# cheolwanpark/tiny-raytracer

Hardware: AMD Instinct MI355X
Metric: Mray/s (primary+secondary) (higher is better)
Workload: dtype f32; 1 GPU; cornell 2048x2048, depth 50, 256 spp per step (of 4096), streamed, reference-order BVH, seed 1; rays=160658711950, samples=22548578304, image_rows_per_gpu=2048, tuning=default, parallelism=single GPU, world_size=1, launched_by=plain

## Files before the change

### bindings/rust/tinyrt-sys/src/lib.rs

```rust
#![allow(non_camel_case_types)]

use std::os::raw::{c_char, c_int, c_void};

pub const TRT_ABI_VERSION: u32 = 4;

pub const TRT_OK: c_int = 0;
pub const TRT_ERR_INVALID_ARG: c_int = -1;
pub const TRT_ERR_DUPLICATE: c_int = -2;
pub const TRT_ERR_NOT_FOUND: c_int = -3;
pub const TRT_ERR_HIP: c_int = -4;
pub const TRT_ERR_NO_DEVICE: c_int = -5;
pub const TRT_ERR_OOM: c_int = -6;

pub const TRT_LAMBERTIAN: u32 = 0;
pub const TRT_METAL: u32 = 1;
pub const TRT_DIELECTRIC: u32 = 2;
pub const TRT_LIGHT: u32 = 3;

pub const TRT_BACKEND_MEGAKERNEL: u32 = 0;
pub const TRT_BACKEND_WAVEFRONT: u32 = 1;
pub const TRT_BACKEND_AUTO: u32 = 2;
pub const TRT_BACKEND_STREAMED: u32 = 3;

#[repr(C)]
// ... 420 lines not shown
    pub fn trt_render_multi(s: *mut trt_scene, cam: *const trt_camera, p: *const trt_render_params, devices: *const c_int,
                            ndev: u32, accum: *mut f32, stats: *mut trt_stats) -> c_int;
    pub fn trt_render_multi_device(s: *mut trt_scene, cam: *const trt_camera, p: *const trt_render_params,
                                   devices: *const c_int, ndev: u32, d_accum: *mut f32, stats: *mut trt_stats) -> c_int;
    pub fn trt_band_rows_local(height: u32, ndev: u32, rank: u32, rows_local: *mut u32) -> c_int;
    pub fn trt_band_copy_plan(width: u32, height: u32, ndev: u32, rank: u32, out: *mut trt_band_copy) -> c_int;
    pub fn trt_streamed_launch_plan(s: *const trt_scene, cam: *const trt_camera, p: *const trt_render_params,
                                    out: *mut trt_launch_plan) -> c_int;
    pub fn trt_render_device(s: *mut trt_scene, cam: *const trt_camera, p: *const trt_render_params, d_accum: *mut f32,
                             d_counters: *mut u64, stream: *mut c_void) -> c_int;
    pub fn trt_render_moments(s: *mut trt_scene, cam: *const trt_camera, p: *const trt_render_params, accum: *mut f32,
                              moment2: *mut f32, stats: *mut trt_stats) -> c_int;
    pub fn trt_render_moments_device(s: *mut trt_scene, cam: *const trt_camera, p: *const trt_render_params, d_accum: *mut f32,
                                     d_moment2: *mut f32, d_counters: *mut u64, stream: *mut c_void) -> c_int;
    pub fn trt_variance(accum: *const f32, moment2: *const f32, npixels: u32, samples_per_pixel: u32, variance: *mut f32) -> c_int;
    pub fn trt_variance_device(d_accum: *const f32, d_moment2: *const f32, npixels: u32, samples_per_pixel: u32,
                               d_variance: *mut f32, stream: *mut c_void) -> c_int;
    pub fn trt_render_pixels(s: *mut trt_scene, cam: *const trt_camera, p: *const trt_render_params, pixels: *const u32, n: u32,
                             accum: *mut f32, moment2: *mut f32, stats: *mut trt_stats) -> c_int;
    pub fn trt_render_pixels_device(s: *mut trt_scene, cam: *const trt_camera, p: *const trt_render_params, d_pixels: *const u32, n: u32,
                                    d_count: *const u32, d_accum: *mut f32, d_moment2: *mut f32, d_counters: *mut u64,
                                    stream: *mut c_void) -> c_int;
    pub fn trt_pixels_launch_plan(s: *const trt_scene, n: u32, compute_units: u32, out: *mut trt_query_plan) -> c_int;
    pub fn trt_select_pixels(accum: *const f32, moment2: *const f32, npixels: u32, samples_per_pixel: u32, samples_done: u32,
                             candidates: *const u32, n_candidates: u32, rel_tol: f32, abs_tol: f32, selected: *mut u32,
                             count: *mut u32) -> c_int;
    pub fn trt_select_pixels_device(d_accum: *const f32, d_moment2: *const f32, npixels: u32, samples_per_pixel: u32, samples_done: u32,
                                    d_candidates: *const u32, n_candidates: u32, rel_tol: f32, abs_tol: f32, d_selected: *mut u32,
                                    d_count: *mut u32, d_scratch: *mut c_void, scratch_bytes: u64, stream: *mut c_void) -> c_int;
    pub fn trt_select_scratch_bytes(n_candidates: u32) -> u64;
    pub fn trt_radiance_params_default(out: *mut trt_radiance_params);
    pub fn trt_radiance(s: *mut trt_scene, rays: *const trt_ray, n: u32, p: *const trt_radiance_params, radiance: *mut f32,
                        moment2: *mut f32, stats: *mut trt_stats) -> c_int;
    pub fn trt_radiance_device(s: *mut trt_scene, d_rays: *const trt_ray, n: u32, p: *const trt_radiance_params, d_radiance: *mut f32,
                               d_moment2: *mut f32, d_counters: *mut u64, stream: *mut c_void) -> c_int;
    pub fn trt_radiance_launch_plan(s: *const trt_scene, n: u32, compute_units: u32, out: *mut trt_query_plan) -> c_int;
    pub fn trt_gather_params_default(out: *mut trt_gather_params);
    pub fn trt_gather(s: *mut trt_scene, items: *const trt_ray, n: u32, p: *const trt_gather_params, radiance: *mut f32,
                      moment2: *mut f32, stats: *mut trt_stats) -> c_int;
    pub fn trt_gather_device(s: *mut trt_scene, d_items: *const trt_ray, n: u32, p: *const trt_gather_params, d_radiance: *mut f32,
                             d_moment2: *mut f32, d_counters: *mut u64, stream: *mut c_void) -> c_int;
    pub fn trt_gather_launch_plan(s: *const trt_scene, n: u32, compute_units: u32, out: *mut trt_query_plan) -> c_int;
    pub fn trt_ambient_params_default(out: *mut trt_ambient_params);
    pub fn trt_ambient(s: *mut trt_scene, items: *const trt_ray, n: u32, p: *const trt_ambient_params, visibility: *mut f32,
                       bent: *mut f32, stats: *mut trt_stats) -> c_int;
    pub fn trt_ambient_device(s: *mut trt_scene, d_items: *const trt_ray, n: u32, p: *const trt_ambient_params, d_visibility: *mut f32,
                              d_bent: *mut f32, d_counters: *mut u64, stream: *mut c_void) -> c_int;
    pub fn trt_ambient_launch_plan(s: *const trt_scene, n: u32, compute_units: u32, out: *mut trt_query_plan) -> c_int;
    pub fn trt_scene_emitters(s: *const trt_scene, out: *mut trt_emitter, cap: u32, count: *mut u32) -> c_int;
    pub fn trt_emitter_init_quad(out: *mut trt_emitter, corner: trt_vec3, u: trt_vec3, v: trt_vec3, color: trt_vec3);
    pub fn trt_emitter_init_sphere(out: *mut trt_emitter, centre: trt_vec3, radius: f32, color: trt_vec3);
    pub fn trt_direct_params_default(out: *mut trt_direct_params);
    pub fn trt_direct(s: *mut trt_scene, items: *const trt_ray, n: u32, emitters: *const trt_emitter, n_emitters: u32,
                      p: *const trt_direct_params, radiance: *mut f32, moment2: *mut f32, stats: *mut trt_stats) -> c_int;
    pub fn trt_direct_device(s: *mut trt_scene, d_items: *const trt_ray, n: u32, d_emitters: *const trt_emitter, n_emitters: u32,
                             p: *const trt_direct_params, d_radiance: *mut f32, d_moment2: *mut f32, d_counters: *mut u64,
                             stream: *mut c_void) -> c_int;
    pub fn trt_direct_launch_plan(s: *const trt_scene, n: u32, compute_units: u32, out: *mut trt_query_plan) -> c_int;
    pub fn trt_nee_params_default(out: *mut trt_nee_params);
    pub fn trt_nee(s: *mut trt_scene, items: *const trt_ray, n: u32, emitters: *const trt_emitter, n_emitters: u32,
                   p: *const trt_nee_params, radiance: *mut f32, moment2: *mut f32, stats: *mut trt_stats) -> c_int;
    pub fn trt_nee_device(s: *mut trt_scene, d_items: *const trt_ray, n: u32, d_emitters: *const trt_emitter, n_emitters: u32,
                          p: *const trt_nee_params, d_radiance: *mut f32, d_moment2: *mut f32, d_counters: *mut u64,
                          stream: *mut c_void) -> c_int;
    pub fn trt_nee_launch_plan(s: *const trt_scene, n: u32, compute_units: u32, out: *mut trt_query_plan) -> c_int;
    pub fn trt_nee_mis_params_default(out: *mut trt_nee_mis_params);
    pub fn trt_nee_mis(s: *mut trt_scene, items: *const trt_ray, n: u32, emitters: *const trt_emitter, n_emitters: u32,
                       p: *const trt_nee_mis_params, radiance: *mut f32, moment2: *mut f32, stats: *mut trt_stats) -> c_int;
    pub fn trt_nee_mis_device(s: *mut trt_scene, d_items: *const trt_ray, n: u32, d_emitters: *const trt_emitter, n_emitters: u32,
                              p: *const trt_nee_mis_params, d_radiance: *mut f32, d_moment2: *mut f32, d_counters: *mut u64,
                              stream: *mut c_void) -> c_int;
    pub fn trt_nee_mis_launch_plan(s: *const trt_scene, n: u32, compute_units: u32, out: *mut trt_query_plan) -> c_int;
    pub fn trt_direct_mis_params_default(out: *mut trt_direct_mis_params);
    pub fn trt_direct_mis(s: *mut trt_scene, items: *const trt_ray, n: u32, emitters: *const trt_emitter, n_emitters: u32,
                          p: *const trt_direct_mis_params, radiance: *mut f32, moment2: *mut f32, stats: *mut trt_stats) -> c_int;
    pub fn trt_direct_mis_device(s: *mut trt_scene, d_items: *const trt_ray, n: u32, d_emitters: *const trt_emitter, n_emitters: u32,
                                 p: *const trt_direct_mis_params, d_radiance: *mut f32, d_moment2: *mut f32, d_counters: *mut u64,
                                 stream: *mut c_void) -> c_int;
    pub fn trt_direct_mis_launch_plan(s: *const trt_scene, n: u32, compute_units: u32, out: *mut trt_query_plan) -> c_int;
    pub fn trt_emitter_pick_build(emitters: *const trt_emitter, n_emitters: u32, weights: *const f32, out: *mut trt_emitter_pick,
                                  total: *mut f32) -> c_int;
    pub fn trt_direct_pick(s: *mut trt_scene, items: *const trt_ray, n: u32, emitters: *const trt_emitter, pick: *const trt_emitter_pick,
                           n_emitters: u32, p: *const trt_direct_params, radiance: *mut f32, moment2: *mut f32, stats: *mut trt_stats) -> c_int;
    pub fn trt_direct_pick_device(s: *mut trt_scene, d_items: *const trt_ray, n: u32, d_emitters: *const trt_emitter,
                                  d_pick: *const trt_emitter_pick, n_emitters: u32, p: *const trt_direct_params, d_radiance: *mut f32,
                                  d_moment2: *mut f32, d_counters: *mut u64, stream: *mut c_void) -> c_int;
    pub fn trt_direct_pick_launch_plan(s: *const trt_scene, n: u32, compute_units: u32, out: *mut trt_query_plan) -> c_int;
    pub fn trt_direct_mis_pick(s: *mut trt_scene, items: *const trt_ray, n: u32, emitters: *const trt_emitter, pick: *const trt_emitter_pick,
                               n_emitters: u32, p: *const trt_direct_mis_params, total_power: f32, radiance: *mut f32, moment2: *mut f32,
                               stats: *mut trt_stats) -> c_int;
    pub fn trt_direct_mis_pick_device(s: *mut trt_scene, d_items: *const trt_ray, n: u32, d_emitters: *const trt_emitter,
                                      d_pick: *const trt_emitter_pick, n_emitters: u32, p: *const trt_direct_mis_params, total_power: f32,
                                      d_radiance: *mut f32, d_moment2: *mut f32, d_counters: *mut u64, stream: *mut c_void) -> c_int;
    pub fn trt_direct_mis_pick_launch_plan(s: *const trt_scene, n: u32, compute_units: u32, out: *mut trt_query_plan) -> c_int;
    pub fn trt_nee_pick(s: *mut trt_scene, items: *const trt_ray, n: u32, emitters: *const trt_emitter, pick: *const trt_emitter_pick,
                        n_emitters: u32, p: *const trt_nee_params, radiance: *mut f32, moment2: *mut f32, stats: *mut trt_stats) -> c_int;
    pub fn trt_nee_pick_device(s: *mut trt_scene, d_items: *const trt_ray, n: u32, d_emitters: *const trt_emitter,
                               d_pick: *const trt_emitter_pick, n_emitters: u32, p: *const trt_nee_params, d_radiance: *mut f32,
                               d_moment2: *mut f32, d_counters: *mut u64, stream: *mut c_void) -> c_int;
    pub fn trt_nee_pick_launch_plan(s: *const trt_scene, n: u32, compute_units: u32, out: *mut trt_query_plan) -> c_int;
    pub fn trt_nee_mis_pick(s: *mut trt_scene, items: *const trt_ray, n: u32, emitters: *const trt_emitter, pick: *const trt_emitter_pick,
                            n_emitters: u32, p: *const trt_nee_mis_params, total_power: f32, radiance: *mut f32, moment2: *mut f32,
                            stats: *mut trt_stats) -> c_int;
    pub fn trt_nee_mis_pick_device(s: *mut trt_scene, d_items: *const trt_ray, n: u32, d_emitters: *const trt_emitter,
                                   d_pick: *const trt_emitter_pick, n_emitters: u32, p: *const trt_nee_mis_params, total_power: f32,
                                   d_radiance: *mut f32, d_moment2: *mut f32, d_counters: *mut u64, stream: *mut c_void) -> c_int;
    pub fn trt_nee_mis_pick_launch_plan(s: *const trt_scene, n: u32, compute_units: u32, out: *mut trt_query_plan) -> c_int;
    pub fn trt_probe_params_default(out: *mut trt_probe_params);
    pub fn trt_probe(s: *mut trt_scene, items: *const trt_ray, n: u32, p: *const trt_probe_params, sh: *mut f32,
                     stats: *mut trt_stats) -> c_int;
    pub fn trt_probe_device(s: *mut trt_scene, d_items: *const trt_ray, n: u32, p: *const trt_probe_params, d_sh: *mut f32,
                            d_counters: *mut u64, stream: *mut c_void) -> c_int;
    pub fn trt_probe_launch_plan(s: *const trt_scene, n: u32, bands: u32, compute_units: u32, out: *mut trt_query_plan) -> c_int;
    pub fn trt_passes_params_default(out: *mut trt_passes_params);
    pub fn trt_passes(s: *mut trt_scene, items: *const trt_ray, n: u32, p: *const trt_passes_params, passes: *mut f32, spent: *mut f32,
                      stats: *mut trt_stats) -> c_int;
    pub fn trt_passes_device(s: *mut trt_scene, d_items: *const trt_ray, n: u32, p: *const trt_passes_params, d_passes: *mut f32,
                             d_spent: *mut f32, d_counters: *mut u64, stream: *mut c_void) -> c_int;
    pub fn trt_passes_launch_plan(s: *const trt_scene, n: u32, depth_bins: u32, compute_units: u32, out: *mut trt_query_plan) -> c_int;
    pub fn trt_sample_batch(s: *mut trt_scene, input: *const trt_sample_point, n: u32, out: *mut trt_sampled_color,
                            max_bounces: u32, background: trt_vec3, seed: u32, stats: *mut trt_stats) -> c_int;
    pub fn trt_intersect(s: *mut trt_scene, rays: *const trt_ray, t_max: *const f32, n: u32, hits: *mut trt_hit) -> c_int;
    pub fn trt_occluded(s: *mut trt_scene, rays: *const trt_ray, t_max: *const f32, n: u32, occluded: *mut u8) -> c_int;
    pub fn trt_intersect_device(s: *mut trt_scene, d_rays: *const trt_ray, d_t_max: *const f32, n: u32, d_hits: *mut trt_hit,
                                stream: *mut c_void) -> c_int;
    pub fn trt_occluded_device(s: *mut trt_scene, d_rays: *const trt_ray, d_t_max: *const f32, n: u32, d_occluded: *mut u8,
                               stream: *mut c_void) -> c_int;
    pub fn trt_query_launch_plan(s: *const trt_scene, n: u32, compute_units: u32, out: *mut trt_query_plan) -> c_int;
    pub fn trt_primary_rays(cam: *const trt_camera, p: *const trt_render_params, s: u32, rays: *mut trt_ray) -> c_int;
    pub fn trt_primary_rays_device(cam: *const trt_camera, p: *const trt_render_params, s: u32, d_rays: *mut trt_ray,
                                   stream: *mut c_void) -> c_int;
    pub fn trt_render_aov(s: *mut trt_scene, cam: *const trt_camera, p: *const trt_render_params, buffers: *const trt_aov_buffers) -> c_int;
    pub fn trt_render_aov_device(s: *mut trt_scene, cam: *const trt_camera, p: *const trt_render_params,
                                 d_buffers: *const trt_aov_buffers, stream: *mut c_void) -> c_int;
    pub fn trt_aov_launch_plan(s: *const trt_scene, n_pixels: u32, compute_units: u32, out: *mut trt_query_plan) -> c_int;
    pub fn trt_denoise_params_default(out: *mut trt_denoise_params);
    pub fn trt_denoise_scratch_bytes(width: u32, height: u32, params: *const trt_denoise_params) -> u64;
    pub fn trt_denoise(input: *const trt_denoise_inputs, width: u32, height: u32, params: *const trt_denoise_params, out: *mut f32) -> c_int;
    pub fn trt_denoise_device(d_in: *const trt_denoise_inputs, width: u32, height: u32, params: *const trt_denoise_params,
                              d_out: *mut f32, d_scratch: *mut c_void, scratch_bytes: u64, stream: *mut c_void) -> c_int;
    pub fn trt_denoise_color_default(out: *mut trt_denoise_color);
    pub fn trt_denoise_ex(input: *const trt_denoise_inputs, color: *const trt_denoise_color, width: u32, height: u32,
                          params: *const trt_denoise_params, out: *mut f32) -> c_int;
    pub fn trt_denoise_ex_device(d_in: *const trt_denoise_inputs, color: *const trt_denoise_color, width: u32, height: u32,
                                 params: *const trt_denoise_params, d_out: *mut f32, d_scratch: *mut c_void, scratch_bytes: u64,
                                 stream: *mut c_void) -> c_int;
    pub fn trt_tonemap_u8(accum: *const f32, npixels: u32, gamma: f32, rgb: *mut u8) -> c_int;
    pub fn trt_tonemap_u8_device(d_accum: *const f32, npixels: u32, gamma: f32, d_rgb: *mut u8, stream: *mut c_void) -> c_int;
    pub fn trt_streamed_chunk_spp(width: u32, rows: u32) -> u32;
    pub fn trt_kernel_timing_begin() -> c_int;
    pub fn trt_kernel_timing_end(total_ms: *mut f64, launches: *mut u32) -> c_int;

    pub fn trt_dominant_kernel(s: *const trt_scene, cam: *const trt_camera, p: *const trt_render_params) -> *const c_char;

    pub fn trt_last_error() -> *const c_char;
    pub fn trt_device_count() -> c_int;
    pub fn trt_set_device(ordinal: c_int) -> c_int;
    pub fn trt_abi_version() -> u32;
}
```

### include/tinyrt.h

```cpp
#ifndef TINYRT_H
#define TINYRT_H

#include <stddef.h>
#include <stdint.h>

#ifdef __cplusplus
extern "C" {
#endif

#define TRT_ABI_VERSION 4

enum trt_status {
    TRT_OK = 0,
    TRT_ERR_INVALID_ARG = -1,
    TRT_ERR_DUPLICATE = -2,
    TRT_ERR_NOT_FOUND = -3,
    TRT_ERR_HIP = -4,
    TRT_ERR_NO_DEVICE = -5,
    TRT_ERR_OOM = -6
};

typedef struct { float x, y, z; } trt_vec3;
typedef struct { trt_vec3 origin, direction; } trt_ray;
typedef struct { uint32_t x, y; trt_ray ray; } trt_sample_point;
// ... 267 lines not shown
typedef struct {
    uint32_t kind;
    uint32_t geometry;
    trt_vec3 a, b, c;
    trt_vec3 normal;
    trt_vec3 color;
    float area;
    uint32_t reserved[2];
} trt_emitter;
int trt_scene_emitters(const trt_scene *s, trt_emitter *out, uint32_t cap, uint32_t *count);
void trt_emitter_init_quad(trt_emitter *out, trt_vec3 corner, trt_vec3 u, trt_vec3 v, trt_vec3 color);
void trt_emitter_init_sphere(trt_emitter *out, trt_vec3 centre, float radius, trt_vec3 color);
typedef struct {
    trt_radiance_params path;
    float shadow_end;
    uint32_t reserved[7];
} trt_direct_params;
void trt_direct_params_default(trt_direct_params *out);
int trt_direct(trt_scene *s, const trt_ray *items, uint32_t n, const trt_emitter *emitters, uint32_t n_emitters,
               const trt_direct_params *p, float *radiance, float *moment2, trt_stats *stats);
int trt_direct_device(trt_scene *s, const trt_ray *d_items, uint32_t n, const trt_emitter *d_emitters, uint32_t n_emitters,
                      const trt_direct_params *p, float *d_radiance, float *d_moment2, uint64_t *d_counters, void *stream);
int trt_direct_launch_plan(const trt_scene *s, uint32_t n, uint32_t compute_units, trt_query_plan *out);

typedef struct {
    trt_gather_params gather;
    float shadow_end;
    uint32_t source_is_diffuse;
    uint32_t reserved[6];
} trt_nee_params;
void trt_nee_params_default(trt_nee_params *out);
int trt_nee(trt_scene *s, const trt_ray *items, uint32_t n, const trt_emitter *emitters, uint32_t n_emitters, const trt_nee_params *p,
            float *radiance, float *moment2, trt_stats *stats);
int trt_nee_device(trt_scene *s, const trt_ray *d_items, uint32_t n, const trt_emitter *d_emitters, uint32_t n_emitters,
                   const trt_nee_params *p, float *d_radiance, float *d_moment2, uint64_t *d_counters, void *stream);
int trt_nee_launch_plan(const trt_scene *s, uint32_t n, uint32_t compute_units, trt_query_plan *out);

enum trt_mis_heuristic { TRT_MIS_BALANCE = 0, TRT_MIS_POWER = 1 };
typedef struct {
    trt_nee_params nee;
    uint32_t heuristic;
    uint32_t reserved[7];
} trt_nee_mis_params;
void trt_nee_mis_params_default(trt_nee_mis_params *out);
int trt_nee_mis(trt_scene *s, const trt_ray *items, uint32_t n, const trt_emitter *emitters, uint32_t n_emitters,
                const trt_nee_mis_params *p, float *radiance, float *moment2, trt_stats *stats);
int trt_nee_mis_device(trt_scene *s, const trt_ray *d_items, uint32_t n, const trt_emitter *d_emitters, uint32_t n_emitters,
                       const trt_nee_mis_params *p, float *d_radiance, float *d_moment2, uint64_t *d_counters, void *stream);
int trt_nee_mis_launch_plan(const trt_scene *s, uint32_t n, uint32_t compute_units, trt_query_plan *out);

typedef struct {
    trt_direct_params direct;
    uint32_t heuristic;
    uint32_t reserved[7];
} trt_direct_mis_params;
void trt_direct_mis_params_default(trt_direct_mis_params *out);
int trt_direct_mis(trt_scene *s, const trt_ray *items, uint32_t n, const trt_emitter *emitters, uint32_t n_emitters,
                   const trt_direct_mis_params *p, float *radiance, float *moment2, trt_stats *stats);
int trt_direct_mis_device(trt_scene *s, const trt_ray *d_items, uint32_t n, const trt_emitter *d_emitters, uint32_t n_emitters,
                          const trt_direct_mis_params *p, float *d_radiance, float *d_moment2, uint64_t *d_counters, void *stream);
int trt_direct_mis_launch_plan(const trt_scene *s, uint32_t n, uint32_t compute_units, trt_query_plan *out);

typedef struct {
    float q;
    uint32_t alias;
    float prob;
    uint32_t reserved;
} trt_emitter_pick;
int trt_emitter_pick_build(const trt_emitter *emitters, uint32_t n_emitters, const float *weights, trt_emitter_pick *out, float *total);
int trt_direct_pick(trt_scene *s, const trt_ray *items, uint32_t n, const trt_emitter *emitters, const trt_emitter_pick *pick,
                    uint32_t n_emitters, const trt_direct_params *p, float *radiance, float *moment2, trt_stats *stats);
int trt_direct_pick_device(trt_scene *s, const trt_ray *d_items, uint32_t n, const trt_emitter *d_emitters, const trt_emitter_pick *d_pick,
                           uint32_t n_emitters, const trt_direct_params *p, float *d_radiance, float *d_moment2, uint64_t *d_counters,
                           void *stream);
int trt_direct_pick_launch_plan(const trt_scene *s, uint32_t n, uint32_t compute_units, trt_query_plan *out);
int trt_direct_mis_pick(trt_scene *s, const trt_ray *items, uint32_t n, const trt_emitter *emitters, const trt_emitter_pick *pick,
                        uint32_t n_emitters, const trt_direct_mis_params *p, float total_power, float *radiance, float *moment2,
                        trt_stats *stats);
int trt_direct_mis_pick_device(trt_scene *s, const trt_ray *d_items, uint32_t n, const trt_emitter *d_emitters,
                               const trt_emitter_pick *d_pick, uint32_t n_emitters, const trt_direct_mis_params *p, float total_power,
                               float *d_radiance, float *d_moment2, uint64_t *d_counters, void *stream);
int trt_direct_mis_pick_launch_plan(const trt_scene *s, uint32_t n, uint32_t compute_units, trt_query_plan *out);

int trt_nee_pick(trt_scene *s, const trt_ray *items, uint32_t n, const trt_emitter *emitters, const trt_emitter_pick *pick,
                 uint32_t n_emitters, const trt_nee_params *p, float *radiance, float *moment2, trt_stats *stats);
int trt_nee_pick_device(trt_scene *s, const trt_ray *d_items, uint32_t n, const trt_emitter *d_emitters, const trt_emitter_pick *d_pick,
                        uint32_t n_emitters, const trt_nee_params *p, float *d_radiance, float *d_moment2, uint64_t *d_counters,
                        void *stream);
int trt_nee_pick_launch_plan(const trt_scene *s, uint32_t n, uint32_t compute_units, trt_query_plan *out);
int trt_nee_mis_pick(trt_scene *s, const trt_ray *items, uint32_t n, const trt_emitter *emitters, const trt_emitter_pick *pick,
                     uint32_t n_emitters, const trt_nee_mis_params *p, float total_power, float *radiance, float *moment2,
                     trt_stats *stats);
int trt_nee_mis_pick_device(trt_scene *s, const trt_ray *d_items, uint32_t n, const trt_emitter *d_emitters,
                            const trt_emitter_pick *d_pick, uint32_t n_emitters, const trt_nee_mis_params *p, float total_power,
                            float *d_radiance, float *d_moment2, uint64_t *d_counters, void *stream);
int trt_nee_mis_pick_launch_plan(const trt_scene *s, uint32_t n, uint32_t compute_units, trt_query_plan *out);

typedef struct {
    uint32_t iterations;
    uint32_t normal_power_log2;
    float sigma_albedo;
    float sigma_depth;
    uint32_t reserved[4];
} trt_denoise_params;
void trt_denoise_params_default(trt_denoise_params *out);
typedef struct {
    const float *color;
    const float *albedo;
    const float *normal;
    const float *depth;
} trt_denoise_inputs;
uint64_t trt_denoise_scratch_bytes(uint32_t width, uint32_t height, const trt_denoise_params *params);
int trt_denoise(const trt_denoise_inputs *in, uint32_t width, uint32_t height, const trt_denoise_params *params, float *out);
int trt_denoise_device(const trt_denoise_inputs *d_in, uint32_t width, uint32_t height, const trt_denoise_params *params,
                       float *d_out, void *d_scratch, uint64_t scratch_bytes, void *stream);

typedef struct {
    const float *variance;
    float sigma_color;
    uint32_t reserved[5];
} trt_denoise_color;
void trt_denoise_color_default(trt_denoise_color *out);
int trt_denoise_ex(const trt_denoise_inputs *in, const trt_denoise_color *color, uint32_t width, uint32_t height,
                   const trt_denoise_params *params, float *out);
int trt_denoise_ex_device(const trt_denoise_inputs *d_in, const trt_denoise_color *color, uint32_t width, uint32_t height,
                          const trt_denoise_params *params, float *d_out, void *d_scratch, uint64_t scratch_bytes, void *stream);

int trt_tonemap_u8(const float *accum, uint32_t npixels, float gamma, uint8_t *rgb);

int trt_tonemap_u8_device(const float *d_accum, uint32_t npixels, float gamma, uint8_t *d_rgb, void *stream);

typedef struct {
    uint32_t scene_mode;
    uint32_t threads_per_workgroup, waves_per_simd, workgroups_per_cu;
    uint32_t lds_bytes, scene_lds_bytes;
    uint32_t leaf_slots, lds_leaf_stack, ray_pool;
    uint32_t walk;
    uint32_t specialised;
    uint32_t has_kernel;
    uint32_t kernel_waves_per_simd, kernel_threads, kernel_walk , kernel_ray_pool, kernel_counting;
    uint32_t chunk_spp;
    uint32_t dual_walk;
    uint64_t workspace_bytes;
} trt_launch_plan;
int trt_streamed_launch_plan(const trt_scene *s, const trt_camera *cam, const trt_render_params *p, trt_launch_plan *out);

uint32_t trt_streamed_chunk_spp(uint32_t width, uint32_t rows);

int trt_kernel_timing_begin(void);
int trt_kernel_timing_end(double *total_ms, uint32_t *launches);

const char *trt_dominant_kernel(const trt_scene *s, const trt_camera *cam, const trt_render_params *p);

const char *trt_last_error(void);
int trt_device_count(void);
int trt_set_device(int ordinal);
uint32_t trt_abi_version(void);

#ifdef __cplusplus
}
#endif
#endif
```

### tiny-raytracer_amd/_lib.py

```python
import ctypes as C
import os
import subprocess

_HERE = os.path.dirname(os.path.abspath(__file__))
LIB_PATH = os.environ.get("TRT_LIB_PATH") or os.path.join(_HERE, "libtinyrt.so")
CSRC = os.path.join(_HERE, "csrc")

TRT_OK = 0
ABI_VERSION = 4
ERR_INVALID_ARG, ERR_DUPLICATE, ERR_NOT_FOUND, ERR_HIP, ERR_NO_DEVICE, ERR_OOM = -1, -2, -3, -4, -5, -6
LAMBERTIAN, METAL, DIELECTRIC, LIGHT = 0, 1, 2, 3
BACKEND_MEGAKERNEL, BACKEND_WAVEFRONT, BACKEND_AUTO, BACKEND_STREAMED = 0, 1, 2, 3


class Vec3(C.Structure):
    _fields_ = [("x", C.c_float), ("y", C.c_float), ("z", C.c_float)]

    def __init__(self, x=0.0, y=0.0, z=0.0):
        super().__init__(float(x), float(y), float(z))

    def tolist(self):
        return [self.x, self.y, self.z]


# ... 178 lines not shown

SIGNATURES = {
    "trt_world_create": (C.c_int, [C.POINTER(C.c_void_p)]),
    "trt_world_destroy": (None, [C.c_void_p]),
    "trt_world_add_material": (C.c_int, [C.c_void_p, C.c_char_p, C.POINTER(Material)]),
    "trt_world_get_material": (C.c_int, [C.c_void_p, C.c_char_p, C.POINTER(C.c_uint32)]),
    "trt_world_add_sphere": (C.c_int, [C.c_void_p, Vec3, C.c_float, C.c_uint32]),
    "trt_world_add_spheres": (C.c_int, [C.c_void_p, C.c_uint32, C.c_void_p, C.c_void_p]),
    "trt_world_add_quad": (C.c_int, [C.c_void_p, Vec3, Vec3, Vec3, C.c_uint32]),
    "trt_world_num_geometries": (C.c_int, [C.c_void_p]),
    "trt_world_num_materials": (C.c_int, [C.c_void_p]),
    "trt_scene_create": (C.c_int, [C.c_void_p, C.POINTER(C.c_void_p)]),
    "trt_scene_options_default": (None, [C.POINTER(SceneOptions)]),
    "trt_scene_create_ex": (C.c_int, [C.c_void_p, C.POINTER(SceneOptions), C.POINTER(C.c_void_p)]),
    "trt_scene_create_on_device": (C.c_int, [C.c_void_p, C.POINTER(SceneOptions), C.POINTER(C.c_void_p)]),
    "trt_tuning_default": (None, [C.POINTER(Tuning)]),
    "trt_scene_destroy": (None, [C.c_void_p]),
    "trt_scene_trim": (C.c_int, [C.c_void_p]),
    "trt_scene_get_info": (C.c_int, [C.c_void_p, C.POINTER(SceneInfo)]),
    "trt_scene_get_nodes": (C.c_int, [C.c_void_p, C.c_void_p, C.c_void_p, C.c_void_p, C.c_uint32]),
    "trt_scene_get_cull_nodes": (C.c_int, [C.c_void_p, C.c_void_p, C.c_void_p, C.c_void_p, C.c_uint32]),
    "trt_scene_get_compact_nodes": (C.c_int, [C.c_void_p, C.c_void_p, C.c_uint32]),
    "trt_scene_get_packed": (C.c_int, [C.c_void_p, C.c_void_p, C.c_uint32]),
    "trt_camera_init": (C.c_int, [C.POINTER(CameraPOD), C.c_float, C.c_float, Vec3, Vec3, Vec3, C.c_float,
                                  C.c_uint32, C.c_uint32]),
    "trt_render": (C.c_int, [C.c_void_p, C.POINTER(CameraPOD), C.POINTER(RenderParams), C.c_void_p, C.POINTER(Stats)]),
    "trt_render_multi": (C.c_int, [C.c_void_p, C.POINTER(CameraPOD), C.POINTER(RenderParams), C.POINTER(C.c_int), C.c_uint32,
                                   C.c_void_p, C.POINTER(Stats)]),
    "trt_render_multi_device": (C.c_int, [C.c_void_p, C.POINTER(CameraPOD), C.POINTER(RenderParams), C.POINTER(C.c_int),
                                          C.c_uint32, C.c_void_p, C.POINTER(Stats)]),
    "trt_band_rows_local": (C.c_int, [C.c_uint32, C.c_uint32, C.c_uint32, C.POINTER(C.c_uint32)]),
    "trt_band_copy_plan": (C.c_int, [C.c_uint32, C.c_uint32, C.c_uint32, C.c_uint32, C.POINTER(BandCopy)]),
    "trt_streamed_launch_plan": (C.c_int, [C.c_void_p, C.POINTER(CameraPOD), C.POINTER(RenderParams), C.POINTER(LaunchPlan)]),
    "trt_kernel_timing_begin": (C.c_int, []),
    "trt_kernel_timing_end": (C.c_int, [C.POINTER(C.c_double), C.POINTER(C.c_uint32)]),
    "trt_render_device": (C.c_int, [C.c_void_p, C.POINTER(CameraPOD), C.POINTER(RenderParams), C.c_void_p, C.c_void_p,
                                    C.c_void_p]),
    "trt_render_moments": (C.c_int, [C.c_void_p, C.POINTER(CameraPOD), C.POINTER(RenderParams), C.c_void_p, C.c_void_p, C.POINTER(Stats)]),
    "trt_render_moments_device": (C.c_int, [C.c_void_p, C.POINTER(CameraPOD), C.POINTER(RenderParams), C.c_void_p, C.c_void_p, C.c_void_p,
                                            C.c_void_p]),
    "trt_variance": (C.c_int, [C.c_void_p, C.c_void_p, C.c_uint32, C.c_uint32, C.c_void_p]),
    "trt_variance_device": (C.c_int, [C.c_void_p, C.c_void_p, C.c_uint32, C.c_uint32, C.c_void_p, C.c_void_p]),
    "trt_render_pixels": (C.c_int, [C.c_void_p, C.POINTER(CameraPOD), C.POINTER(RenderParams), C.c_void_p, C.c_uint32, C.c_void_p, C.c_void_p,
                                    C.POINTER(Stats)]),
    "trt_render_pixels_device": (C.c_int, [C.c_void_p, C.POINTER(CameraPOD), C.POINTER(RenderParams), C.c_void_p, C.c_uint32, C.c_void_p,
                                           C.c_void_p, C.c_void_p, C.c_void_p, C.c_void_p]),
    "trt_pixels_launch_plan": (C.c_int, [C.c_void_p, C.c_uint32, C.c_uint32, C.POINTER(QueryPlan)]),
    "trt_select_pixels": (C.c_int, [C.c_void_p, C.c_void_p, C.c_uint32, C.c_uint32, C.c_uint32, C.c_void_p, C.c_uint32, C.c_float, C.c_float,
                                    C.c_void_p, C.POINTER(C.c_uint32)]),
    "trt_select_pixels_device": (C.c_int, [C.c_void_p, C.c_void_p, C.c_uint32, C.c_uint32, C.c_uint32, C.c_void_p, C.c_uint32, C.c_float,
                                           C.c_float, C.c_void_p, C.c_void_p, C.c_void_p, C.c_uint64, C.c_void_p]),
    "trt_select_scratch_bytes": (C.c_uint64, [C.c_uint32]),
    "trt_radiance_params_default": (None, [C.POINTER(RadianceParams)]),
    "trt_radiance": (C.c_int, [C.c_void_p, C.c_void_p, C.c_uint32, C.POINTER(RadianceParams), C.c_void_p, C.c_void_p, C.POINTER(Stats)]),
    "trt_radiance_device": (C.c_int, [C.c_void_p, C.c_void_p, C.c_uint32, C.POINTER(RadianceParams), C.c_void_p, C.c_void_p, C.c_void_p,
                                      C.c_void_p]),
    "trt_radiance_launch_plan": (C.c_int, [C.c_void_p, C.c_uint32, C.c_uint32, C.POINTER(QueryPlan)]),
    "trt_gather_params_default": (None, [C.POINTER(GatherParams)]),
    "trt_gather": (C.c_int, [C.c_void_p, C.c_void_p, C.c_uint32, C.POINTER(GatherParams), C.c_void_p, C.c_void_p, C.POINTER(Stats)]),
    "trt_gather_device": (C.c_int, [C.c_void_p, C.c_void_p, C.c_uint32, C.POINTER(GatherParams), C.c_void_p, C.c_void_p, C.c_void_p,
                                    C.c_void_p]),
    "trt_gather_launch_plan": (C.c_int, [C.c_void_p, C.c_uint32, C.c_uint32, C.POINTER(QueryPlan)]),
    "trt_ambient_params_default": (None, [C.POINTER(AmbientParams)]),
    "trt_ambient": (C.c_int, [C.c_void_p, C.c_void_p, C.c_uint32, C.POINTER(AmbientParams), C.c_void_p, C.c_void_p, C.POINTER(Stats)]),
    "trt_ambient_device": (C.c_int, [C.c_void_p, C.c_void_p, C.c_uint32, C.POINTER(AmbientParams), C.c_void_p, C.c_void_p, C.c_void_p,
                                     C.c_void_p]),
    "trt_ambient_launch_plan": (C.c_int, [C.c_void_p, C.c_uint32, C.c_uint32, C.POINTER(QueryPlan)]),
    "trt_scene_emitters": (C.c_int, [C.c_void_p, C.c_void_p, C.c_uint32, C.POINTER(C.c_uint32)]),
    "trt_emitter_init_quad": (None, [C.POINTER(Emitter), Vec3, Vec3, Vec3, Vec3]),
    "trt_emitter_init_sphere": (None, [C.POINTER(Emitter), Vec3, C.c_float, Vec3]),
    "trt_direct_params_default": (None, [C.POINTER(DirectParams)]),
    "trt_direct": (C.c_int, [C.c_void_p, C.c_void_p, C.c_uint32, C.c_void_p, C.c_uint32, C.POINTER(DirectParams), C.c_void_p, C.c_void_p,
                             C.POINTER(Stats)]),
    "trt_direct_device": (C.c_int, [C.c_void_p, C.c_void_p, C.c_uint32, C.c_void_p, C.c_uint32, C.POINTER(DirectParams), C.c_void_p, C.c_void_p,
                                    C.c_void_p, C.c_void_p]),
    "trt_direct_launch_plan": (C.c_int, [C.c_void_p, C.c_uint32, C.c_uint32, C.POINTER(QueryPlan)]),
    "trt_nee_params_default": (None, [C.POINTER(NeeParams)]),
    "trt_nee": (C.c_int, [C.c_void_p, C.c_void_p, C.c_uint32, C.c_void_p, C.c_uint32, C.POINTER(NeeParams), C.c_void_p, C.c_void_p,
                          C.POINTER(Stats)]),
    "trt_nee_device": (C.c_int, [C.c_void_p, C.c_void_p, C.c_uint32, C.c_void_p, C.c_uint32, C.POINTER(NeeParams), C.c_void_p, C.c_void_p,
                                 C.c_void_p, C.c_void_p]),
    "trt_nee_launch_plan": (C.c_int, [C.c_void_p, C.c_uint32, C.c_uint32, C.POINTER(QueryPlan)]),
    "trt_nee_mis_params_default": (None, [C.POINTER(NeeMisParams)]),
    "trt_nee_mis": (C.c_int, [C.c_void_p, C.c_void_p, C.c_uint32, C.c_void_p, C.c_uint32, C.POINTER(NeeMisParams), C.c_void_p, C.c_void_p,
                              C.POINTER(Stats)]),
    "trt_nee_mis_device": (C.c_int, [C.c_void_p, C.c_void_p, C.c_uint32, C.c_void_p, C.c_uint32, C.POINTER(NeeMisParams), C.c_void_p, C.c_void_p,
                                     C.c_void_p, C.c_void_p]),
    "trt_nee_mis_launch_plan": (C.c_int, [C.c_void_p, C.c_uint32, C.c_uint32, C.POINTER(QueryPlan)]),
    "trt_direct_mis_params_default": (None, [C.POINTER(DirectMisParams)]),
    "trt_direct_mis": (C.c_int, [C.c_void_p, C.c_void_p, C.c_uint32, C.c_void_p, C.c_uint32, C.POINTER(DirectMisParams), C.c_void_p, C.c_void_p,
                                 C.POINTER(Stats)]),
    "trt_direct_mis_device": (C.c_int, [C.c_void_p, C.c_void_p, C.c_uint32, C.c_void_p, C.c_uint32, C.POINTER(DirectMisParams), C.c_void_p,
                                        C.c_void_p, C.c_void_p, C.c_void_p]),
    "trt_direct_mis_launch_plan": (C.c_int, [C.c_void_p, C.c_uint32, C.c_uint32, C.POINTER(QueryPlan)]),
    "trt_emitter_pick_build": (C.c_int, [C.c_void_p, C.c_uint32, C.c_void_p, C.c_void_p, C.POINTER(C.c_float)]),
    "trt_direct_pick": (C.c_int, [C.c_void_p, C.c_void_p, C.c_uint32, C.c_void_p, C.c_void_p, C.c_uint32, C.POINTER(DirectParams), C.c_void_p,
                                  C.c_void_p, C.POINTER(Stats)]),
    "trt_direct_pick_device": (C.c_int, [C.c_void_p, C.c_void_p, C.c_uint32, C.c_void_p, C.c_void_p, C.c_uint32, C.POINTER(DirectParams),
                                         C.c_void_p, C.c_void_p, C.c_void_p, C.c_void_p]),
    "trt_direct_pick_launch_plan": (C.c_int, [C.c_void_p, C.c_uint32, C.c_uint32, C.POINTER(QueryPlan)]),
    "trt_direct_mis_pick": (C.c_int, [C.c_void_p, C.c_void_p, C.c_uint32, C.c_void_p, C.c_void_p, C.c_uint32, C.POINTER(DirectMisParams),
                                      C.c_float, C.c_void_p, C.c_void_p, C.POINTER(Stats)]),
    "trt_direct_mis_pick_device": (C.c_int, [C.c_void_p, C.c_void_p, C.c_uint32, C.c_void_p, C.c_void_p, C.c_uint32, C.POINTER(DirectMisParams),
                                             C.c_float, C.c_void_p, C.c_void_p, C.c_void_p, C.c_void_p]),
    "trt_direct_mis_pick_launch_plan": (C.c_int, [C.c_void_p, C.c_uint32, C.c_uint32, C.POINTER(QueryPlan)]),
    "trt_nee_pick": (C.c_int, [C.c_void_p, C.c_void_p, C.c_uint32, C.c_void_p, C.c_void_p, C.c_uint32, C.POINTER(NeeParams), C.c_void_p,
                               C.c_void_p, C.POINTER(Stats)]),
    "trt_nee_pick_device": (C.c_int, [C.c_void_p, C.c_void_p, C.c_uint32, C.c_void_p, C.c_void_p, C.c_uint32, C.POINTER(NeeParams),
                                      C.c_void_p, C.c_void_p, C.c_void_p, C.c_void_p]),
    "trt_nee_pick_launch_plan": (C.c_int, [C.c_void_p, C.c_uint32, C.c_uint32, C.POINTER(QueryPlan)]),
    "trt_nee_mis_pick": (C.c_int, [C.c_void_p, C.c_void_p, C.c_uint32, C.c_void_p, C.c_void_p, C.c_uint32, C.POINTER(NeeMisParams),
                                   C.c_float, C.c_void_p, C.c_void_p, C.POINTER(Stats)]),
    "trt_nee_mis_pick_device": (C.c_int, [C.c_void_p, C.c_void_p, C.c_uint32, C.c_void_p, C.c_void_p, C.c_uint32, C.POINTER(NeeMisParams),
                                          C.c_float, C.c_void_p, C.c_void_p, C.c_void_p, C.c_void_p]),
    "trt_nee_mis_pick_launch_plan": (C.c_int, [C.c_void_p, C.c_uint32, C.c_uint32, C.POINTER(QueryPlan)]),
    "trt_probe_params_default": (None, [C.POINTER(ProbeParams)]),
    "trt_probe": (C.c_int, [C.c_void_p, C.c_void_p, C.c_uint32, C.POINTER(ProbeParams), C.c_void_p, C.POINTER(Stats)]),
    "trt_probe_device": (C.c_int, [C.c_void_p, C.c_void_p, C.c_uint32, C.POINTER(ProbeParams), C.c_void_p, C.c_void_p, C.c_void_p]),
    "trt_probe_launch_plan": (C.c_int, [C.c_void_p, C.c_uint32, C.c_uint32, C.c_uint32, C.POINTER(QueryPlan)]),
    "trt_passes_params_default": (None, [C.POINTER(PassesParams)]),
    "trt_passes": (C.c_int, [C.c_void_p, C.c_void_p, C.c_uint32, C.POINTER(PassesParams), C.c_void_p, C.c_void_p, C.POINTER(Stats)]),
    "trt_passes_device": (C.c_int, [C.c_void_p, C.c_void_p, C.c_uint32, C.POINTER(PassesParams), C.c_void_p, C.c_void_p, C.c_void_p,
                                    C.c_void_p]),
    "trt_passes_launch_plan": (C.c_int, [C.c_void_p, C.c_uint32, C.c_uint32, C.c_uint32, C.POINTER(QueryPlan)]),
    "trt_sample_batch": (C.c_int, [C.c_void_p, C.c_void_p, C.c_uint32, C.c_void_p, C.c_uint32, Vec3, C.c_uint32,
                                   C.POINTER(Stats)]),
    "trt_intersect": (C.c_int, [C.c_void_p, C.c_void_p, C.c_void_p, C.c_uint32, C.c_void_p]),
    "trt_occluded": (C.c_int, [C.c_void_p, C.c_void_p, C.c_void_p, C.c_uint32, C.c_void_p]),
    "trt_intersect_device": (C.c_int, [C.c_void_p, C.c_void_p, C.c_void_p, C.c_uint32, C.c_void_p, C.c_void_p]),
    "trt_occluded_device": (C.c_int, [C.c_void_p, C.c_void_p, C.c_void_p, C.c_uint32, C.c_void_p, C.c_void_p]),
    "trt_query_launch_plan": (C.c_int, [C.c_void_p, C.c_uint32, C.c_uint32, C.POINTER(QueryPlan)]),
    "trt_primary_rays": (C.c_int, [C.POINTER(CameraPOD), C.POINTER(RenderParams), C.c_uint32, C.c_void_p]),
    "trt_primary_rays_device": (C.c_int, [C.POINTER(CameraPOD), C.POINTER(RenderParams), C.c_uint32, C.c_void_p, C.c_void_p]),
    "trt_render_aov": (C.c_int, [C.c_void_p, C.POINTER(CameraPOD), C.POINTER(RenderParams), C.POINTER(AovBuffers)]),
    "trt_render_aov_device": (C.c_int, [C.c_void_p, C.POINTER(CameraPOD), C.POINTER(RenderParams), C.POINTER(AovBuffers), C.c_void_p]),
    "trt_aov_launch_plan": (C.c_int, [C.c_void_p, C.c_uint32, C.c_uint32, C.POINTER(QueryPlan)]),
    "trt_denoise_params_default": (None, [C.POINTER(DenoiseParams)]),
    "trt_denoise_scratch_bytes": (C.c_uint64, [C.c_uint32, C.c_uint32, C.POINTER(DenoiseParams)]),
    "trt_denoise": (C.c_int, [C.POINTER(DenoiseInputs), C.c_uint32, C.c_uint32, C.POINTER(DenoiseParams), C.c_void_p]),
    "trt_denoise_device": (C.c_int, [C.POINTER(DenoiseInputs), C.c_uint32, C.c_uint32, C.POINTER(DenoiseParams), C.c_void_p, C.c_void_p,
                                     C.c_uint64, C.c_void_p]),
    "trt_denoise_color_default": (None, [C.POINTER(DenoiseColor)]),
    "trt_denoise_ex": (C.c_int, [C.POINTER(DenoiseInputs), C.POINTER(DenoiseColor), C.c_uint32, C.c_uint32, C.POINTER(DenoiseParams), C.c_void_p]),
    "trt_denoise_ex_device": (C.c_int, [C.POINTER(DenoiseInputs), C.POINTER(DenoiseColor), C.c_uint32, C.c_uint32, C.POINTER(DenoiseParams),
                                        C.c_void_p, C.c_void_p, C.c_uint64, C.c_void_p]),
    "trt_streamed_chunk_spp": (C.c_uint32, [C.c_uint32, C.c_uint32]),
    "trt_tonemap_u8": (C.c_int, [C.c_void_p, C.c_uint32, C.c_float, C.c_void_p]),
    "trt_tonemap_u8_device": (C.c_int, [C.c_void_p, C.c_uint32, C.c_float, C.c_void_p, C.c_void_p]),
    "trt_dominant_kernel": (C.c_char_p, [C.c_void_p, C.POINTER(CameraPOD), C.POINTER(RenderParams)]),
    "trt_last_error": (C.c_char_p, []),
    "trt_device_count": (C.c_int, []),
    "trt_set_device": (C.c_int, [C.c_int]),
    "trt_abi_version": (C.c_uint32, []),
}


def build(force=False):
    if force and os.path.exists(LIB_PATH):
        os.remove(LIB_PATH)
    subprocess.run(["make", "-C", CSRC, "--no-print-directory"], check=True)
    return LIB_PATH


def _share_hip_runtime_with_torch():
    import importlib.util
    try:
        spec = importlib.util.find_spec("torch")
    except (ImportError, ValueError):
        spec = None
    if spec is None or not spec.submodule_search_locations:
        return None
    cand = os.path.join(list(spec.submodule_search_locations)[0], "lib", "libamdhip64.so")
    if os.path.exists(cand):
        C.CDLL(cand, mode=C.RTLD_GLOBAL)
        return cand
    return None


def load():
    _share_hip_runtime_with_torch()
    if not os.path.exists(LIB_PATH):
        raise ImportError(
            f"{LIB_PATH} is missing: build the HIP extension first (python -c 'import __graft_entry__ as g; g.build()' "
            "or make -C tiny-raytracer_amd/csrc). There is no fallback path.")
    lib = C.CDLL(LIB_PATH)
    for name, (res, args) in SIGNATURES.items():
        fn = getattr(lib, name)
        fn.restype = res
        fn.argtypes = args
    if lib.trt_abi_version() != ABI_VERSION:
        raise ImportError("libtinyrt.so ABI version mismatch")
    return lib


lib = load()


class TinyRTError(RuntimeError):
    def __init__(self, code, message):
        super().__init__(f"tinyrt error {code}: {message}")
        self.code = code


def check(rc):
    if rc != TRT_OK:
        raise TinyRTError(rc, lib.trt_last_error().decode("utf-8", "replace"))
```

### tiny-raytracer_amd/csrc/capi.hip

```cpp
#include <hip/hip_runtime.h>

#include <math.h>
#include <stdio.h>
#include <stdlib.h>
#include <string.h>

#include <algorithm>
#include <memory>
#include <mutex>
#include <new>
#include <string>
#include <thread>
#include <vector>

#include "axis_quads.h"
#include "nearest_first.h"
#include "flat_reuse.h"
#include "host_stage.h"
#include "kernels.h"
#include "scene.h"
#include "scene_adopt.h"
#include "scene_cache.h"
#include "scene_query.h"
#include "stream_plan.h"

using namespace trt;

struct trt_world {
    World w;
};

namespace trt {
namespace {
std::mutex g_timing_mu;
bool g_timing_on = false;
unsigned g_timing_epoch = 0;
struct TimingPair { hipEvent_t begin, end; int device; };
std::vector<TimingPair> g_timing_pairs;
struct TimingOpen { hipEvent_t ev = nullptr; hipStream_t stream = nullptr; int device = -1; unsigned epoch = 0; };
thread_local TimingOpen t_open;
}
void timing_mark(hipStream_t stream, bool begin) {
    unsigned epoch;
    {
        std::lock_guard<std::mutex> lock(g_timing_mu);
        if (!g_timing_on) return;
        epoch = g_timing_epoch;
    }
    int dev = -1;
    if (hipGetDevice(&dev) != hipSuccess) { (void)hipGetLastError(); return; }
    if (begin) {
        if (t_open.ev) { (void)hipEventDestroy(t_open.ev); t_open = TimingOpen{}; }
        hipEvent_t ev = nullptr;
        if (hipEventCreate(&ev) != hipSuccess) { (void)hipGetLastError(); return; }
        if (hipEventRecord(ev, stream) != hipSuccess) { (void)hipGetLastError(); (void)hipEventDestroy(ev); return; }
        t_open.ev = ev; t_open.stream = stream; t_open.device = dev; t_open.epoch = epoch;
        return;
    }
    if (!t_open.ev) return;
    TimingOpen o = t_open;
    t_open = TimingOpen{};
    hipEvent_t ev = nullptr;
    if (o.stream != stream || o.device != dev || o.epoch != epoch || hipEventCreate(&ev) != hipSuccess) {
        (void)hipGetLastError();
        (void)hipEventDestroy(o.ev);
        return;
    }
    if (hipEventRecord(ev, stream) != hipSuccess) { (void)hipGetLastError(); (void)hipEventDestroy(ev); (void)hipEventDestroy(o.ev); return; }
    std::lock_guard<std::mutex> lock(g_timing_mu);
    if (g_timing_on && g_timing_epoch == epoch) g_timing_pairs.push_back(TimingPair{o.ev, ev, dev});
    else { (void)hipEventDestroy(o.ev); (void)hipEventDestroy(ev); }
}
}

struct trt_scene {
    SceneHost host;
    FlatReuse flat_reuse{};
    std::vector<uint32_t> geo_index;
    SceneCache cache;
};

namespace {

thread_local std::string g_last_error;

int fail(int code, const std::string& msg) {
    g_last_error = msg;
    return code;
}
int fail_hip(hipError_t e, const char* what) {
    return fail(TRT_ERR_HIP, std::string(what) + ": " + hipGetErrorString(e));
}
#define TRT_HIP(call)                                        \
    do {                                                     \
        hipError_t e_ = (call);                              \
        if (e_ != hipSuccess) return fail_hip(e_, #call);    \
    } while (0)

struct Defaults {
    trt_tuning tuning;
    trt_scene_options scene;
    bool flat_reuse = true;
    bool axis_quads = true;
    bool nearest_first = true;
};
const Defaults& defaults() {
    static const Defaults d = [] {
        Defaults x;
        x.tuning = tuning_builtin();
        x.scene = scene_options_builtin();
        auto env = [](const char* name) -> const char* { const char* e = getenv(name); return (e && *e) ? e : nullptr; };
        auto u32 = [&](const char* name, uint32_t& field) { if (const char* e = env(name)) field = (uint32_t)strtoul(e, nullptr, 10); };
        trt_tuning& t = x.tuning;
        u32("TRT_STREAM_MINW", t.stream_waves_per_simd); u32("TRT_BIG_THREADS", t.stream_big_threads); u32("TRT_STREAM_BATCH_SPP", t.stream_batch_spp);
        u32("TRT_RADIANCE_GB", t.radiance_gb); u32("TRT_LEAF_SLOTS", t.leaf_slots); u32("TRT_LDS_LEAF_STACK", t.lds_leaf_stack);
        u32("TRT_RAY_POOL", t.ray_pool); u32("TRT_STRAGGLERS", t.stragglers); u32("TRT_LDS_STRAGGLERS", t.lds_stragglers);
        u32("TRT_DUAL_WALK", t.dual_walk); u32("TRT_RUNTIME_WALK", t.runtime_walk); u32("TRT_XCD_REMAP", t.xcd_remap);
        u32("TRT_MINW", t.mega_waves_per_simd); u32("TRT_MEGA_THREADS", t.mega_threads); u32("TRT_MINW8", t.mega_global_waves8);
        u32("TRT_WF_MINW", t.wf_waves_per_simd); u32("TRT_WF_SERVE_MIN", t.wf_serve_min);
        trt_scene_options& o = x.scene;
        if (const char* e = env("TRT_CULL_PRUNE")) {
            const float v = (float)atof(e);
            if (v > 0.0f && v <= 1.0f) o.cull_prune = v;
        }
        if (const char* e = env("TRT_FLAT_WALK")) o.flat_walk = atoi(e) ? 1 : 0;
        if (const char* e = env("TRT_FLAT_REUSE")) x.flat_reuse = atoi(e) != 0;
        if (const char* e = env("TRT_AXIS_QUADS")) x.axis_quads = atoi(e) != 0;
        if (const char* e = env("TRT_NEAREST_FIRST")) x.nearest_first = atoi(e) != 0;
        if (const char* e = env("TRT_COMPACT_NODES")) o.compact_nodes = atoi(e) ? 1 : 0;
        if (const char* e = env("TRT_SCRATCH_CAP_MB")) o.scratch_cap_bytes = (uint64_t)strtoull(e, nullptr, 10) << 20;
        return x;
    }();
    return d;
}

[[maybe_unused]] const bool g_defaults_read_at_load = (defaults(), true);

int require_device() {
    int n = 0;
    hipError_t e = hipGetDeviceCount(&n);
    if (e != hipSuccess || n <= 0) {
        (void)hipGetLastError();
        return fail(TRT_ERR_NO_DEVICE, "no HIP device visible: libtinyrt has no CPU path, it needs a gfx950 GPU");
    }
    return TRT_OK;
}

int scene_on_device(trt_scene* s, SceneDev& out) {
    out.L = s->host.layout;
    return s->cache.on_device(SceneCache::PACKED_SCENE, s->host.blob.data(), s->host.layout.blob_bytes, "scene upload", out.blob);
}

void to_camera_dev(const trt_camera& c, CameraDev& d) {
    const trt_vec3* src[6] = {&c.position, &c.viewport_upper_left, &c.horizontal, &c.vertical, &c.defocus_disk_u, &c.defocus_disk_v};
    float* dst[6] = {d.pos, d.upper_left, d.horizontal, d.vertical, d.du, d.dv};
    for (int i = 0; i < 6; i++) { dst[i][0] = src[i]->x; dst[i][1] = src[i]->y; dst[i][2] = src[i]->z; }
    d.width = c.width;
    d.height = c.height;
}

int to_render_args(const trt_camera* cam, const trt_render_params* p, RenderArgs& ra, uint32_t& rows, trt_tuning& tn) {
    if (cam->width < 2 || cam->height < 2) return fail(TRT_ERR_INVALID_ARG, "camera width and height must be at least 2 (pointgen.rs:41-42 divides by width-1, height-1)");
    if (p->samples_per_pixel == 0) return fail(TRT_ERR_INVALID_ARG, "samples_per_pixel must be positive");
    uint32_t s1 = p->sample_end == 0 ? p->samples_per_pixel : p->sample_end;
    if (p->sample_begin > s1 || s1 > p->samples_per_pixel) return fail(TRT_ERR_INVALID_ARG, "sample range must satisfy begin <= end <= samples_per_pixel");
    if (p->backend > TRT_BACKEND_STREAMED) return fail(TRT_ERR_INVALID_ARG, "unknown backend");
    ra.background[0] = p->background.x; ra.background[1] = p->background.y; ra.background[2] = p->background.z;
    ra.inv_spp = 1.0f / (float)p->samples_per_pixel;
    ra.max_bounces = p->max_bounces;
    ra.seed_key = rng_seed_key(p->seed);
    ra.sample_begin = p->sample_begin;
    ra.sample_end = s1;
    ra.accumulate = p->accumulate ? 1u : 0u;
    if (p->band_rows == 0) {
        ra.band_rows = 0; ra.band_stride = 1; ra.band_offset = 0;
        rows = cam->height;
    } else {
        if (p->band_stride == 0 || p->band_offset >= p->band_stride) return fail(TRT_ERR_INVALID_ARG, "band_offset must be below band_stride");
        rows = p->rows_local;
        if (rows > 0) {
            uint32_t last = rows - 1;
            uint64_t y = ((uint64_t)(last / p->band_rows) * p->band_stride + p->band_offset) * p->band_rows + last % p->band_rows;
            if (y >= cam->height) return fail(TRT_ERR_INVALID_ARG, "rows_local maps past the last image row");
        }
        ra.band_rows = p->band_rows; ra.band_stride = p->band_stride; ra.band_offset = p->band_offset;
    }
    ra.rows_local = rows;
    tn = p->tuning ? *p->tuning : defaults().tuning;
    if (tn.stream_batch_spp > 256u) tn.stream_batch_spp = 256u;
    if (tn.stragglers > 63u) tn.stragglers = 63u;
    if (tn.lds_stragglers > 63u) tn.lds_stragglers = 63u;
    if (tn.radiance_gb > 64u) tn.radiance_gb = 64u;
    ra.leaf_slots = tn.leaf_slots;
    ra.lds_leaf_stack = tn.lds_leaf_stack;
    ra.xcd_aware = tn.xcd_remap ? 1u : 0u;
    ra.stragglers = tn.stragglers;
    ra.ref_tree = p->collect_stats == 1 ? 1u : 0u;
    ra.flat_reuse = FlatReuse{0u, 0u, 0u};
    return TRT_OK;
}

int check_render_args(const trt_camera* cam, const trt_render_params* p, uint32_t& rows) {
    RenderArgs ra;
    trt_tuning tn;
    return to_render_args(cam, p, ra, rows, tn);
}

int enqueue_render(trt_scene* s, const trt_camera* cam, const trt_render_params* p, float* d_accum, uint64_t* d_counters,
                   hipStream_t stream, uint32_t* rows_out, float* d_moment2 = nullptr, MomentsLaunch launch_moments = nullptr) {
    RenderArgs ra;
    trt_tuning tn;
    uint32_t rows = 0;
    int rc = to_render_args(cam, p, ra, rows, tn);
    if (rc != TRT_OK) return rc;
    if (rows_out) *rows_out = rows;
    SceneDev sc;
    rc = scene_on_device(s, sc);
    if (rc != TRT_OK) return rc;
    CameraDev cd;
    to_camera_dev(*cam, cd);
    ra.flat_reuse = s->flat_reuse;
    const size_t bytes = (size_t)rows * cam->width * 3 * sizeof(float);
    if (rows == 0 || ra.sample_begin == ra.sample_end || ra.max_bounces == 0) {
        if (!ra.accumulate && bytes) TRT_HIP(hipMemsetAsync(d_accum, 0, bytes, stream));
        if (!ra.accumulate && bytes && d_moment2) TRT_HIP(hipMemsetAsync(d_moment2, 0, bytes, stream));
        return TRT_OK;
    }
    const bool wavefront = p->backend == TRT_BACKEND_WAVEFRONT;
    const bool streamed = p->backend == TRT_BACKEND_STREAMED || p->backend == TRT_BACKEND_AUTO;
    if (wavefront || streamed) {
        int dev = 0;
        TRT_HIP(hipGetDevice(&dev));
        Workspace* ws = nullptr;
        if (wavefront) {
            rc = s->cache.workspace_acquire(dev, wavefront_workspace_bytes(cam->width, rows), stream, &ws);
        } else {
            uint32_t samples = ra.sample_end - ra.sample_begin;
            const uint32_t full = streamed_chunk_spp(cam->width, rows, tn.radiance_gb);
            if (samples > full) samples = full;
            const uint32_t wanted = samples;
            const uint32_t short_samples = s->cache.short_samples(dev);
            if (short_samples != 0u && short_samples < samples) {
                const size_t idle = s->cache.idle_workspace_bytes(dev);
                size_t free_b = 0, total_b = 0;
                const bool known = hipMemGetInfo(&free_b, &total_b) == hipSuccess;
                (void)hipGetLastError();
                if (!known || free_b + idle < streamed_workspace_bytes(cam->width, rows, samples, tn.radiance_gb)) samples = short_samples;
            }
            bool trimmed = false;
            for (;;) {
                rc = s->cache.workspace_acquire(dev, streamed_workspace_bytes(cam->width, rows, samples, tn.radiance_gb), stream, &ws);
                if (rc != TRT_ERR_OOM) break;
                if (!trimmed) {
                    trimmed = true;
                    s->cache.trim(dev, 0);
                    continue;
                }
                if (samples <= 1u) break;
                samples = (samples + 1u) / 2u;
            }
            s->cache.set_short_samples(dev, (rc == TRT_OK && samples < wanted) ? samples : 0u);
        }
        if (rc != TRT_OK) return rc;
        hipError_t le;
        if (streamed && d_moment2) {
            le = launch_moments ? launch_moments(sc, cd, ra, tn, ws->ptr, ws->bytes, d_accum, d_moment2, reinterpret_cast<unsigned long long*>(d_counters),
                                                 p->collect_stats != 0, stream)
                                : hipErrorInvalidDeviceFunction;
        } else if (streamed) {
            le = launch_streamed(sc, cd, ra, tn, ws->ptr, ws->bytes, d_accum, reinterpret_cast<unsigned long long*>(d_counters), p->collect_stats != 0, stream);
        } else {
            le = launch_wavefront(sc, cd, ra, tn, ws->ptr, d_accum, reinterpret_cast<unsigned long long*>(d_counters), p->collect_stats != 0, stream);
        }
        rc = s->cache.workspace_release(dev, ws, stream);
        if (le != hipSuccess) return fail_hip(le, streamed ? "launch_streamed" : "launch_wavefront");
        return rc;
    }
    TRT_HIP(launch_megakernel(sc, cd, ra, tn, d_accum, reinterpret_cast<unsigned long long*>(d_counters), p->collect_stats != 0, stream));
    return TRT_OK;
}

void set_flat_reuse(trt_scene* s) {
    const SceneLayout& L = s->host.layout;
    const size_t end = 16u * ((size_t)L.off_leaf_list + 2u * (size_t)L.n_leaves);
    const bool have = L.flat_walk != 0u && L.n_leaves > 0u && s->host.blob.size() >= end;
    uint32_t m[3];
    flat_reuse_masks(have ? s->host.blob.data() + 16u * (size_t)L.off_leaf_list : nullptr, L.n_leaves, have && defaults().flat_reuse, m);
    const size_t qend = 16u * ((size_t)L.off_quad + 5u * (size_t)L.n_quads);
    const bool have_quads = have && L.n_quads > 0u && s->host.blob.size() >= qend;
    const uint32_t aq = axis_quads_flag(have_quads ? s->host.blob.data() + 16u * (size_t)L.off_quad : nullptr, L.n_quads, L.n_leaves, L.flat_walk != 0u,
                                        scene_mode(L) == 1, defaults().axis_quads);
    float planes[3];
    const uint32_t nf = nearest_first_flag(have ? s->host.blob.data() + 16u * (size_t)L.off_leaf_list : nullptr, L.n_leaves,
                                           have_quads ? s->host.blob.data() + 16u * (size_t)L.off_quad : nullptr, L.n_quads, L.n_spheres, aq,
                                           defaults().nearest_first, planes);
    s->flat_reuse = FlatReuse{m[0], m[1], m[2], aq, nf, planes[0], planes[1], planes[2]};
}

void set_geo_index(trt_scene* s) {
    const SceneLayout& L = s->host.layout;
    const std::vector<int32_t>& geo = s->host.reference.prim_geo;
    s->geo_index.assign((size_t)L.n_spheres + L.n_quads, 0xFFFFFFFFu);
    const size_t end = 16u * ((size_t)L.off_ref_nodes + 2u * (size_t)L.n_nodes);
    if (geo.size() < L.n_nodes || s->host.blob.size() < end) return;
    for (uint32_t i = 0; i < L.n_nodes; i++) {
        if (geo[i] < 0) continue;
        uint32_t link;
        memcpy(&link, s->host.blob.data() + 16u * ((size_t)L.off_ref_nodes + 2u * (size_t)i + 1u) + 12u, 4);
        const size_t slot = (size_t)(link & PRIM_INDEX_MASK) + ((link & PRIM_QUAD_BIT) ? L.n_spheres : 0u);
        if (!(link & NODE_INNER_BIT) && slot < s->geo_index.size()) s->geo_index[slot] = (uint32_t)geo[i];
    }
}

trt_scene* scene_from_host(SceneHost&& host, const trt_scene_options& opt) {
    std::unique_ptr<trt_scene> s(new trt_scene());
    s->host = std::move(host);
    set_flat_reuse(s.get());
    set_geo_index(s.get());
    s->cache.set_cap((size_t)opt.scratch_cap_bytes);
    return s.release();
}

}

namespace trt {
int query_fail(int code, const std::string& msg) { return fail(code, msg); }
int query_fail_hip(hipError_t e, const char* what) { return fail_hip(e, what); }
int query_require_device() { return require_device(); }
const SceneLayout& query_scene_layout(const trt_scene* s) { return s->host.layout; }
int query_scene_on_device(trt_scene* s, QueryScene& out) {
    int rc = scene_on_device(s, out.scene);
    if (rc != TRT_OK) return rc;
    out.flat_reuse = s->flat_reuse;
    return s->cache.on_device(SceneCache::GEO_INDEX, s->geo_index.data(), s->geo_index.size() * sizeof(uint32_t), "geometry index upload", out.geo_index);
}
int query_render_args(const trt_camera* cam, const trt_render_params* p, RenderArgs& ra, uint32_t& rows) {
    trt_render_params q = *p;
    q.backend = TRT_BACKEND_AUTO;
    q.tuning = nullptr;
    trt_tuning tn;
    return to_render_args(cam, &q, ra, rows, tn);
}
void query_camera_dev(const trt_camera& cam, CameraDev& out) { to_camera_dev(cam, out); }
}

namespace trt {
int scene_options_check(const trt_scene_options& opt) {
    if (!(opt.cull_prune > 0.0f && opt.cull_prune <= 1.0f)) return fail(TRT_ERR_INVALID_ARG, "cull_prune must be in (0, 1]");
    return TRT_OK;
}
trt_scene_options scene_options_or_defaults(const trt_scene_options* options) { return options ? *options : defaults().scene; }
int scene_fail(int code, const std::string& msg) { return fail(code, msg); }
const World& world_of(const trt_world* w) { return w->w; }
trt_scene* scene_adopt(SceneHost&& host, const trt_scene_options& opt, int device, void* d_blob) {
    try {
        trt_scene* s = scene_from_host(std::move(host), opt);
        if (d_blob) s->cache.adopt_packed_scene(device, d_blob);
        return s;
    } catch (const std::bad_alloc&) {
        fail(TRT_ERR_OOM, "out of memory");
        return nullptr;
    }
}
}

extern "C" {

uint32_t trt_abi_version(void) { return TRT_ABI_VERSION; }
const char* trt_last_error(void) { return g_last_error.c_str(); }

int trt_device_count(void) {
    int n = 0;
    if (hipGetDeviceCount(&n) != hipSuccess) { (void)hipGetLastError(); return 0; }
    return n;
}
int trt_set_device(int ordinal) {
    int rc = require_device();
    if (rc != TRT_OK) return rc;
    TRT_HIP(hipSetDevice(ordinal));
    return TRT_OK;
}

int trt_world_create(trt_world** out) {
    if (!out) return fail(TRT_ERR_INVALID_ARG, "out is null");
    trt_world* w = new (std::nothrow) trt_world();
    if (!w) return fail(TRT_ERR_OOM, "out of memory");
    *out = w;
    return TRT_OK;
}
void trt_world_destroy(trt_world* w) { delete w; }

int trt_world_add_material(trt_world* w, const char* name, const trt_material* m) {
    if (!w || !name || !m) return fail(TRT_ERR_INVALID_ARG, "null argument");
    if (m->kind > TRT_LIGHT) return fail(TRT_ERR_INVALID_ARG, "unknown material kind");
    try {
        std::string key(name);
        if (w->w.material_index.count(key)) return fail(TRT_ERR_DUPLICATE, key + " key is already in the material table");
        trt_material mm = *m;
        if (mm.kind == TRT_METAL) mm.param = fminf(fmaxf(mm.param, 0.0f), 1.0f);
        w->w.material_index.emplace(key, (uint32_t)w->w.materials.size());
        w->w.materials.push_back(mm);
    } catch (const std::bad_alloc&) {
        return fail(TRT_ERR_OOM, "out of memory");
    }
    return TRT_OK;
}
int trt_world_get_material(const trt_world* w, const char* name, uint32_t* index) {
    if (!w || !name || !index) return fail(TRT_ERR_INVALID_ARG, "null argument");
    auto it = w->w.material_index.find(name);
    if (it == w->w.material_index.end()) return fail(TRT_ERR_NOT_FOUND, std::string("no material named ") + name);
    *index = it->second;
    return TRT_OK;
}
int trt_world_add_sphere(trt_world* w, trt_vec3 center, float radius, uint32_t material) {
    if (!w) return fail(TRT_ERR_INVALID_ARG, "world is null");
    if (material >= w->w.materials.size()) return fail(TRT_ERR_INVALID_ARG, "material index out of range");
// ... 550 lines not shown
```

### tiny-raytracer_amd/csrc/kernels.h

```cpp
#pragma once

#include <hip/hip_runtime.h>
#include <stddef.h>
#include <stdint.h>

#include "scene.h"

namespace trt {

struct SceneDev {
    const float4* blob;
    SceneLayout L;
};

struct CameraDev {
    float pos[3], upper_left[3], horizontal[3], vertical[3], du[3], dv[3];
    uint32_t width, height;
};

struct FlatReuse {
    uint32_t x, y, z;
    uint32_t axis_quads = 0u;
    uint32_t nearest_first = 0u;
    float px = 0.0f, py = 0.0f, pz = 0.0f;
};

struct RenderArgs {
    float background[3];
    float inv_spp;
    uint32_t max_bounces;
    uint32_t seed_key;
    uint32_t sample_begin, sample_end;
    uint32_t accumulate;
    uint32_t band_rows, band_stride, band_offset;
    uint32_t rows_local;
    uint32_t xcd_aware;
    uint32_t lds_leaf_stack;
    uint32_t leaf_slots;
    uint32_t ref_tree;
    uint32_t stragglers;
    FlatReuse flat_reuse;
};

inline trt_tuning tuning_builtin() {
    trt_tuning t{};
    t.stream_waves_per_simd = 0;
    t.stream_big_threads = 0;
    t.stream_batch_spp = 8;
    t.radiance_gb = 16;
    t.leaf_slots = 0;
    t.lds_leaf_stack = 1;
    t.ray_pool = 1;
    t.stragglers = 8;
    t.lds_stragglers = 8;
    t.dual_walk = 0;
    t.runtime_walk = 0;
    t.xcd_remap = 0;
    t.mega_waves_per_simd = 0; t.mega_threads = 0; t.mega_global_waves8 = 0;
    t.wf_waves_per_simd = 0; t.wf_serve_min = 0;
    return t;
}

inline uint32_t rng_seed_key(uint32_t seed) {
    uint32_t x = seed + 0x9E3779B9u;
    x ^= x >> 16; x *= 0x7feb352du; x ^= x >> 15; x *= 0x846ca68bu; x ^= x >> 16;
    return x;
}

enum { CTR_SAMPLES = 0, CTR_RAYS, CTR_NODE, CTR_SPHERE, CTR_QUAD_PLANE, CTR_QUAD_INSIDE, CTR_SHADE, CTR_PEND = 7,
       CTR_W_ROUNDS = 8, CTR_W_STEPS, CTR_W_LEAF, CTR_W_GEN, CTR_SHADE_KIND = 12, CTR_COUNT = 16 };

inline int scene_mode(const SceneLayout& L) { return L.hot_bytes <= kLdsSceneMaxBytes ? 1 : 0; }
inline uint32_t scene_lds_bytes(const SceneLayout& L) { return scene_mode(L) == 1 ? L.hot_bytes : 0u; }
inline size_t q_align16(size_t b) { return (b + 15u) & ~(size_t)15u; }

void timing_mark(hipStream_t stream, bool begin);

hipError_t launch_megakernel(const SceneDev& sc, const CameraDev& cam, const RenderArgs& ra, const trt_tuning& tn, float* d_accum,
                             unsigned long long* d_counters, bool stats, hipStream_t stream);

struct WfState {
    float4* s0;
    float4* s1;
    float4* s2;
    float4* s3;
    uint2* rng;
};
size_t wavefront_workspace_bytes(uint32_t width, uint32_t rows);
hipError_t launch_wavefront(const SceneDev& sc, const CameraDev& cam, const RenderArgs& ra, const trt_tuning& tn, void* workspace, float* d_accum,
                            unsigned long long* d_counters, bool stats, hipStream_t stream);

uint32_t streamed_chunk_spp(uint32_t width, uint32_t rows, uint32_t radiance_gb);
size_t streamed_workspace_bytes(uint32_t width, uint32_t rows, uint32_t samples, uint32_t radiance_gb);
uint32_t streamed_chunk_that_fits(uint32_t width, uint32_t rows, size_t bytes);
struct StreamLaunchPlan {
    int mode, threads, waves_per_simd;
    uint32_t wg_per_cu, slots;
    bool lds_stack, flat, compact, pool, specialised;
    bool dual;
    int walk;
    size_t lds_bytes, scene_lds_bytes;
    int kernel_index;
    int kernel_minw, kernel_threads, kernel_walk;
    bool kernel_pool, kernel_stats;
    const char* kernel_name;
};
hipError_t launch_streamed(const SceneDev& sc, const CameraDev& cam, const RenderArgs& ra, const trt_tuning& tn, void* workspace, size_t workspace_bytes,
                           float* d_accum, unsigned long long* d_counters, bool stats, hipStream_t stream);
hipError_t launch_streamed_moments(const SceneDev& sc, const CameraDev& cam, const RenderArgs& ra, const trt_tuning& tn, void* workspace, size_t workspace_bytes,
                                   float* d_accum, float* d_moment2, unsigned long long* d_counters, bool stats, hipStream_t stream);
hipError_t launch_variance(const float* d_accum, const float* d_moment2, uint32_t npixels, uint32_t samples_per_pixel, float* d_variance, hipStream_t stream);

hipError_t launch_tonemap_u8(const float* d_accum, unsigned long long npixels, float gamma, uint8_t* d_rgb, hipStream_t stream);

hipError_t launch_sample_batch(const SceneDev& sc, const trt_sample_point* d_in, uint32_t n, trt_sampled_color* d_out,
                               const RenderArgs& ra, unsigned long long* d_counters, bool stats, hipStream_t stream);

}
```

### tiny-raytracer_amd/csrc/rt_path.h

```cpp
#pragma once

#include "axis_quads.h"
#include "nearest_first.h"
#include "kernels.h"
#include "rt_device.h"
#include "stream_plan.h"

namespace trt {

extern __shared__ float4 g_lds[];


template <int MODE>
struct SceneAcc {
    const float4* blob;
    SceneLayout L;
    TRT_DEV float4 f4(uint32_t idx) const { return MODE == MODE_LDS ? g_lds[idx] : blob[idx]; }
    TRT_DEV uint32_t u32(uint32_t idx) const {
        return MODE == MODE_LDS ? reinterpret_cast<const uint32_t*>(g_lds)[idx] : reinterpret_cast<const uint32_t*>(blob)[idx];
    }
    TRT_DEV void node(uint32_t i, float4& a, float4& b) const { a = f4(2u * i); b = f4(2u * i + 1u); }
    TRT_DEV void ref_node(uint32_t i, float4& a, float4& b) const { a = blob[L.off_ref_nodes + 2u * i]; b = blob[L.off_ref_nodes + 2u * i + 1u]; }
    TRT_DEV float4 sphere(uint32_t i) const { return f4(L.off_sphere + i); }
    TRT_DEV float4 quad(uint32_t plane, uint32_t i) const { return f4(L.off_quad + 5u * i + plane); }
// ... 308 lines not shown
    const uint32_t lim = lds_offset(limit), base = lds_offset(g_lds);
    unsigned long long saved, m0, m1;
    uint32_t cnt;
    asm volatile(
        "s_mov_b64 %[sv], exec\n"
        "1:\n"
        "v_cmp_gt_u32_e32 vcc, %[n], %[i]\n"
        "v_cmp_ne_u32_e64 %[m0], %[top], %[lim]\n"
        "s_and_b64 vcc, vcc, %[m0]\n"
        "s_and_b64 exec, exec, vcc\n"
        "s_cbranch_scc0 2f\n"
        "v_lshl_add_u32 v52, %[i], 5, %[base]\n"
        "ds_read_b128 v[48:51], v52\n"
        "ds_read_b128 v[52:55], v52 offset:16\n"
        "s_waitcnt lgkmcnt(1)\n"
        "v_sub_f32_e32 v48, v48, %[ox]\n"
        "v_sub_f32_e32 v51, v51, %[ox]\n"
        "v_sub_f32_e32 v49, v49, %[oy]\n"
        "v_sub_f32_e32 v50, v50, %[oz]\n"
        "v_mul_f32_e32 v48, v48, %[ix]\n"
        "v_mul_f32_e32 v51, v51, %[ix]\n"
        "v_mul_f32_e32 v49, v49, %[iy]\n"
        "v_mul_f32_e32 v50, v50, %[iz]\n"
        "s_waitcnt lgkmcnt(0)\n"
        "v_sub_f32_e32 v52, v52, %[oy]\n"
        "v_sub_f32_e32 v53, v53, %[oz]\n"
        "v_mul_f32_e32 v52, v52, %[iy]\n"
        "v_mul_f32_e32 v53, v53, %[iz]\n"
        "v_med3_f32 v56, v48, v51, %[tmin]\n"
        "v_med3_f32 v48, v48, v51, %[tb]\n"
        "v_min_f32_e32 v57, v49, v52\n"
        "v_max_f32_e32 v49, v49, v52\n"
        "v_min_f32_e32 v51, v50, v53\n"
        "v_max_f32_e32 v50, v50, v53\n"
        "v_max3_f32 v56, v56, v57, v51\n"
        "v_min3_f32 v48, v48, v49, v50\n"
        "v_cmp_nle_f32_e32 vcc, v48, v56\n"
        "v_cmp_gt_i32_e64 %[m0], 0, v55\n"
        "s_and_b64 %[m1], vcc, %[m0]\n"
        "v_cndmask_b32_e64 %[i], v54, |v55|, %[m1]\n"
        "s_andn2_b64 %[m1], vcc, %[m0]\n"
        "s_and_saveexec_b64 %[m0], %[m1]\n"
        "ds_write2_b32 %[top], v55, v56 offset1:1\n"
        "v_add_u32_e32 %[top], 0x200, %[top]\n"
        "s_mov_b64 exec, %[m0]\n"
        "s_bcnt1_i32_b64 %[cnt], exec\n"
        "s_cmp_gt_u32 %[cnt], %[few]\n"
        "s_cbranch_scc1 1b\n"
        "2:\n"
        "s_mov_b64 exec, %[sv]\n"
        : [i] "+v"(tr.i), [top] "+v"(top), [sv] "=&s"(saved), [m0] "=&s"(m0), [m1] "=&s"(m1), [cnt] "=&s"(cnt)
        : [n] "s"(n), [few] "s"(few), [base] "s"(base), [lim] "v"(lim), [ox] "v"(o.x), [oy] "v"(o.y), [oz] "v"(o.z), [ix] "v"(tr.inv.x),
          [iy] "v"(tr.inv.y), [iz] "v"(tr.inv.z), [tb] "v"(tr.t_best), [tmin] "s"(kTMin)
        : "vcc", "scc", "memory", "v48", "v49", "v50", "v51", "v52", "v53", "v54", "v55", "v56", "v57");
    return stk + ((top - stk_off) >> 3);
}

template <int MODE, bool STATS, bool ANY = false>
TRT_DEV bool walk_fast_lds(const SceneAcc<MODE>& sc, const Ray& ray, Trav& tr, Counters<STATS>& ctr, float2* stk, uint32_t slots,
                           uint32_t stragglers = 0u, uint32_t entered = 64u) {
    const uint32_t n = sc.L.n_cull_nodes;
    float2* const limit = stk + 64u * slots;
    const uint32_t few = stragglers < entered ? stragglers : entered - 1u;
    for (;;) {
        float2* top = stk;
        if constexpr (kAsmBoxLoop && !STATS && MODE == MODE_LDS) {
            top = box_loop_lds(tr, ray.o, stk, limit, n, few);
        } else
        while (tr.i < n && top != limit) {
            float4 na, nb;
            sc.node(tr.i, na, nb);
            if constexpr (STATS) { ctr.node++; if (first_active_lane()) ctr.w_steps++; }
            float start;
            const bool pass = slab_fast_entry(na, nb, ray.o, tr.inv, kTMin, tr.t_best, start);
            const uint32_t link = __float_as_uint(nb.w);
            const bool inner = (link & NODE_INNER_BIT) != 0u;
            tr.i = (pass && inner) ? (link & ~NODE_INNER_BIT) : __float_as_uint(nb.z);
            if (pass && !inner) {
                *top = make_float2(nb.w, start);
                top += 64;
            }
            if ((uint32_t)__builtin_popcountll(__builtin_amdgcn_ballot_w64(true)) <= few) break;
        }
        TRT_CLK(ctr, 1);
        if (top == stk && tr.i >= n) return true;
        if (top != stk) leaf_phase<MODE, STATS>(stk, top, tr, ctr, [&](uint32_t leaf) { trav_leaf<MODE, STATS>(sc, ray, tr, leaf, ctr); });
        TRT_CLK(ctr, 2);
        if constexpr (ANY) { if (tr.prim_best != PRIM_NONE) tr.i = n; }
        if (tr.i >= n) return true;
        if ((uint32_t)__builtin_popcountll(__builtin_amdgcn_ballot_w64(true)) <= few) { trav_park(stk, tr); return false; }
    }
}

#define TRT_FLAT_BOX(LOX, LOY, LOZ, HIX, HIY, HIZ)                                                                                        \
    "s_bitcmp1_b32 %[rx], %[i]\n s_cbranch_scc1 10f\n"                                                                                  \
    "v_sub_f32_e32 %[t0], " LOX ", %[ox]\n v_sub_f32_e32 %[t1], " HIX ", %[ox]\n v_mul_f32_e32 %[t0], %[ix], %[t0]\n"                  \
    "v_mul_f32_e32 %[t1], %[ix], %[t1]\n v_med3_f32 %[xe], %[t0], %[t1], %[tmin]\n v_med3_f32 %[xx], %[t0], %[t1], %[tb]\n"              \
    "10:\n s_bitcmp1_b32 %[ry], %[i]\n s_cbranch_scc1 11f\n"                                                                            \
    "v_sub_f32_e32 %[t0], " LOY ", %[oy]\n v_sub_f32_e32 %[t1], " HIY ", %[oy]\n v_mul_f32_e32 %[t0], %[iy], %[t0]\n"                  \
    "v_mul_f32_e32 %[t1], %[iy], %[t1]\n v_min_f32_e32 %[ye], %[t0], %[t1]\n v_max_f32_e32 %[yx], %[t0], %[t1]\n"                        \
    "11:\n s_bitcmp1_b32 %[rz], %[i]\n s_cbranch_scc1 12f\n"                                                                            \
    "v_sub_f32_e32 %[t0], " LOZ ", %[oz]\n v_sub_f32_e32 %[t1], " HIZ ", %[oz]\n v_mul_f32_e32 %[t0], %[iz], %[t0]\n"                  \
    "v_mul_f32_e32 %[t1], %[iz], %[t1]\n v_min_f32_e32 %[ze], %[t0], %[t1]\n v_max_f32_e32 %[zx], %[t0], %[t1]\n"                        \
    "12:\n v_max3_f32 %[st], %[xe], %[ye], %[ze]\n v_min3_f32 %[t0], %[xx], %[yx], %[zx]\n v_cmp_nle_f32_e32 vcc, %[t0], %[st]\n"

TRT_DEV float2* box_loop_flat(const Trav& tr, const V3& o, const float4* __restrict__ leaf_list, uint32_t& i, uint32_t n, float2* stk, float2* limit,
                              FlatReuse reuse) {
    const uint32_t stk_off = lds_offset(stk);
    uint32_t top = stk_off;
    const uint32_t lim = lds_offset(limit);
    const uint32_t first = ~(1u << (i & 31u));
    const uint32_t rx = reuse.x & first, ry = reuse.y & first, rz = reuse.z & first;
    unsigned long long m;
    uint32_t off;
    float t0, t1, xe, xx, ye, yx, ze, zx, st, lk;
    asm volatile(
        "s_lshl_b32 %[off], %[i], 5\n"
        "s_load_dwordx16 s[36:51], %[list], %[off]\n"
        "1:\n"
        "s_waitcnt lgkmcnt(0)\n"
        TRT_FLAT_BOX("s36", "s37", "s38", "s39", "s40", "s41")
        "s_and_saveexec_b64 %[m], vcc\n"
        "v_mov_b32_e32 %[lk], s43\n"
        "ds_write2_b32 %[top], %[lk], %[st] offset1:1\n"
        "v_add_u32_e32 %[top], 0x200, %[top]\n"
        "s_mov_b64 exec, %[m]\n"
        "s_add_u32 %[i], %[i], 1\n"
        "s_cmp_ge_u32 %[i], %[n]\n"
        "s_cbranch_scc1 2f\n"
        TRT_FLAT_BOX("s44", "s45", "s46", "s47", "s48", "s49")
        "v_mov_b32_e32 %[lk], s51\n"
        "s_add_u32 %[off], %[off], 64\n"
        "s_load_dwordx16 s[36:51], %[list], %[off]\n"
        "s_and_saveexec_b64 %[m], vcc\n"
        "ds_write2_b32 %[top], %[lk], %[st] offset1:1\n"
        "v_add_u32_e32 %[top], 0x200, %[top]\n"
        "s_mov_b64 exec, %[m]\n"
        "s_add_u32 %[i], %[i], 1\n"
        "v_cmp_gt_u32_e32 vcc, %[top], %[lim]\n"
        "s_cmp_lg_u64 vcc, 0\n"
        "s_cbranch_scc1 2f\n"
        "s_cmp_lt_u32 %[i], %[n]\n"
        "s_cbranch_scc1 1b\n"
        "2:\n"
        "s_waitcnt lgkmcnt(0)\n"
        : [i] "+s"(i), [top] "+v"(top), [m] "=&s"(m), [off] "=&s"(off), [t0] "=&v"(t0), [t1] "=&v"(t1), [xe] "=&v"(xe), [xx] "=&v"(xx),
          [ye] "=&v"(ye), [yx] "=&v"(yx), [ze] "=&v"(ze), [zx] "=&v"(zx), [st] "=&v"(st), [lk] "=&v"(lk)
        : [n] "s"(n), [list] "s"(leaf_list), [lim] "v"(lim), [ox] "v"(o.x), [oy] "v"(o.y), [oz] "v"(o.z), [ix] "v"(tr.inv.x), [iy] "v"(tr.inv.y),
          [iz] "v"(tr.inv.z), [tb] "v"(tr.t_best), [tmin] "s"(kTMin), [rx] "s"(rx), [ry] "s"(ry), [rz] "s"(rz)
        : "vcc", "scc", "memory", "s36", "s37", "s38", "s39", "s40", "s41", "s42", "s43", "s44", "s45", "s46", "s47", "s48", "s49", "s50", "s51");
    return stk + ((top - stk_off) >> 3);
}

struct FlatIntervals {
    float xe, xx, ye, yx, ze, zx;
};
TRT_DEV bool flat_box(FlatIntervals& c, float4 na, float4 nb, V3 o, V3 inv, uint32_t axes, float start, float end, float& start_out) {
    if (axes & 1u) { const float x0 = (na.x - o.x) * inv.x, x1 = (na.w - o.x) * inv.x; c.xe = __builtin_fminf(x0, x1); c.xx = __builtin_fmaxf(x0, x1); }
    if (axes & 2u) { const float y0 = (na.y - o.y) * inv.y, y1 = (nb.x - o.y) * inv.y; c.ye = __builtin_fminf(y0, y1); c.yx = __builtin_fmaxf(y0, y1); }
    if (axes & 4u) { const float z0 = (na.z - o.z) * inv.z, z1 = (nb.y - o.z) * inv.z; c.ze = __builtin_fminf(z0, z1); c.zx = __builtin_fmaxf(z0, z1); }
    const float tn = __builtin_fmaxf(__builtin_fmaxf(c.xe, c.ye), c.ze);
    const float tf = __builtin_fminf(__builtin_fminf(c.xx, c.yx), c.zx);
    start = __builtin_fmaxf(start, tn);
    end = __builtin_fminf(end, tf);
    start_out = start;
    return !(end <= start);
}
TRT_DEV uint32_t flat_axes(const FlatReuse& r, uint32_t i) {
    const uint32_t b = 1u << (i & 31u);
    return ((r.x & b) ? 0u : 1u) | ((r.y & b) ? 0u : 2u) | ((r.z & b) ? 0u : 4u);
}

template <int MODE, bool STATS, bool ANY = false>
TRT_DEV void walk_flat(const SceneAcc<MODE>& sc, const float4* __restrict__ leaf_list, const Ray& ray, Trav& tr, Counters<STATS>& ctr,
                       float2* stk, uint32_t slots, FlatReuse reuse) {
    const uint32_t n = sc.L.n_leaves;
    uint32_t i = 0;
    const bool nearest = !STATS && !ANY && reuse.nearest_first != 0u;
    const float margin = nearest ? nf_margin(reuse.px, reuse.py, reuse.pz, ray.o.x, ray.o.y, ray.o.z, tr.inv.x, tr.inv.y, tr.inv.z) : 0.0f;
    auto phase = [&](const float2* top) {
        if constexpr (!STATS && !ANY) {
            if (nearest) { leaf_phase_nearest<MODE>(sc, ray, stk, top, tr, margin); return; }
        }
        leaf_phase<MODE, STATS>(stk, top, tr, ctr, [&](uint32_t leaf) { trav_leaf<MODE, STATS, !STATS>(sc, ray, tr, leaf, ctr, reuse.axis_quads); });
    };
    if constexpr (kAsmBoxLoop && !STATS) {
        float2* const lim = stk + 64u * (slots - 2u);
        do {
            float2* const top = box_loop_flat(tr, ray.o, leaf_list, i, n, stk, lim, reuse);
            TRT_CLK(ctr, 1);
            phase(top);
            TRT_CLK(ctr, 2);
            if constexpr (ANY) { if (__builtin_amdgcn_ballot_w64(tr.prim_best == PRIM_NONE) == 0ull) return; }
        } while (i < n);
        return;
    }
    const float4* __restrict__ pair = leaf_list;
    float4 a0 = pair[0], b0 = pair[1], a1 = pair[2], b1 = pair[3];
    float2* const limit = stk + 64u * (slots - 2u);
    FlatIntervals iv;
    do {
        float2* top = stk;
        bool first = true;
        for (; i < n;) {
            pair += 4;
            const float4 na0 = pair[0], nb0 = pair[1], na1 = pair[2], nb1 = pair[3];
            if constexpr (STATS) { ctr.node++; if (first_active_lane()) ctr.w_steps++; }
            float start;
            if (flat_box(iv, a0, b0, ray.o, tr.inv, first ? 7u : flat_axes(reuse, i), kTMin, tr.t_best, start)) {
                *top = make_float2(b0.w, start);
                top += 64;
            }
            first = false;
            if (i + 1u < n) {
                if constexpr (STATS) { ctr.node++; if (first_active_lane()) ctr.w_steps++; }
                if (flat_box(iv, a1, b1, ray.o, tr.inv, flat_axes(reuse, i + 1u), kTMin, tr.t_best, start)) {
                    *top = make_float2(b1.w, start);
                    top += 64;
                }
            }
            i += 2u;
            a0 = na0; b0 = nb0; a1 = na1; b1 = nb1;
            if (__builtin_amdgcn_ballot_w64(top > limit) != 0ull) break;
        }
        TRT_CLK(ctr, 1);
        if constexpr (STATS) ctr.pend += (uint32_t)(top - stk) >> 6;
        phase(top);
        TRT_CLK(ctr, 2);
        if constexpr (ANY) { if (__builtin_amdgcn_ballot_w64(tr.prim_best == PRIM_NONE) == 0ull) return; }
    } while (i < n);
}

constexpr uint32_t kCompactLeafBit = 0x80000000u;
typedef _Float16 half2_t __attribute__((ext_vector_type(2)));

template <int MODE, bool STATS>
TRT_DEV void compact_leaf_test(const SceneAcc<MODE>& sc, const float4* __restrict__ leaf_list, const Ray& ray, Trav& tr, uint32_t leaf, Counters<STATS>& ctr) {
    leaf &= ~kCompactLeafBit;
    const float4 na = leaf_list[2u * leaf], nb = leaf_list[2u * leaf + 1u];
    if constexpr (STATS) ctr.node++;
    if (slab_fast(na, nb, ray.o, tr.inv, kTMin, tr.t_best)) trav_leaf<MODE, STATS>(sc, ray, tr, __float_as_uint(nb.w), ctr);
}

TRT_DEV float2* box_loop_compact(Trav& tr, const V3& o, const uint4* __restrict__ nodes16, float2* stk, float2* limit, uint32_t end, uint32_t few) {
    const uint32_t stk_off = lds_offset(stk);
    uint32_t top = stk_off;
    const uint32_t lim = lds_offset(limit);
    unsigned long long saved, m0, m1;
    uint32_t cnt;
    asm volatile(
        "s_mov_b64 %[sv], exec\n"
        "v_mul_f32_e64 v57, -%[ox], %[ix]\n"
        "v_mul_f32_e64 v58, -%[oy], %[iy]\n"
        "v_mul_f32_e64 v59, -%[oz], %[iz]\n"
        "1:\n"
        "v_cmp_gt_u32_e32 vcc, %[n], %[i]\n"
        "v_cmp_ne_u32_e64 %[m0], %[top], %[lim]\n"
        "s_and_b64 vcc, vcc, %[m0]\n"
        "s_and_b64 exec, exec, vcc\n"
        "s_cbranch_scc0 2f\n"
        "global_load_dwordx4 v[48:51], %[i], %[nodes]\n"
        "s_waitcnt vmcnt(0)\n"
        "v_fma_mix_f32 v52, v48, %[ix], v57 op_sel:[0,0,0] op_sel_hi:[1,0,0]\n"
        "v_fma_mix_f32 v53, v48, %[iy], v58 op_sel:[1,0,0] op_sel_hi:[1,0,0]\n"
        "v_fma_mix_f32 v54, v49, %[iz], v59 op_sel:[0,0,0] op_sel_hi:[1,0,0]\n"
        "v_fma_mix_f32 v49, v49, %[ix], v57 op_sel:[1,0,0] op_sel_hi:[1,0,0]\n"
        "v_fma_mix_f32 v48, v50, %[iy], v58 op_sel:[0,0,0] op_sel_hi:[1,0,0]\n"
        "v_fma_mix_f32 v50, v50, %[iz], v59 op_sel:[1,0,0] op_sel_hi:[1,0,0]\n"
        "v_med3_f32 v55, v52, v49, %[tmin]\n"
        "v_med3_f32 v52, v52, v49, %[tb]\n"
        "v_min_f32_e32 v56, v53, v48\n"
        "v_max_f32_e32 v48, v53, v48\n"
        "v_min_f32_e32 v49, v54, v50\n"
        "v_max_f32_e32 v54, v54, v50\n"
        "v_max3_f32 v55, v55, v56, v49\n"
        "v_min3_f32 v52, v52, v48, v54\n"
        "v_cmp_nle_f32_e32 vcc, v52, v55\n"
        "v_cmp_gt_i32_e64 %[m0], 0, v51\n"
        "s_or_b64 %[m1], vcc, %[m0]\n"
        "v_add_u32_e32 v56, 16, %[i]\n"
        "v_cndmask_b32_e64 %[i], v51, v56, %[m1]\n"
        "s_and_b64 %[m1], vcc, %[m0]\n"
        "s_and_saveexec_b64 %[m0], %[m1]\n"
        "ds_write2_b32 %[top], v51, v55 offset1:1\n"
        "v_add_u32_e32 %[top], 0x200, %[top]\n"
        "s_mov_b64 exec, %[m0]\n"
        "s_bcnt1_i32_b64 %[cnt], exec\n"
        "s_cmp_gt_u32 %[cnt], %[few]\n"
        "s_cbranch_scc1 1b\n"
        "2:\n"
        "s_mov_b64 exec, %[sv]\n"
        : [i] "+v"(tr.i), [top] "+v"(top), [sv] "=&s"(saved), [m0] "=&s"(m0), [m1] "=&s"(m1), [cnt] "=&s"(cnt)
        : [n] "s"(end), [few] "s"(few), [nodes] "s"(nodes16), [lim] "v"(lim), [ox] "v"(o.x), [oy] "v"(o.y), [oz] "v"(o.z), [ix] "v"(tr.inv.x),
          [iy] "v"(tr.inv.y), [iz] "v"(tr.inv.z), [tb] "v"(tr.t_best), [tmin] "s"(kTMin)
        : "vcc", "scc", "memory", "v48", "v49", "v50", "v51", "v52", "v53", "v54", "v55", "v56", "v57", "v58", "v59");
    return stk + ((top - stk_off) >> 3);
}

template <int MODE, bool STATS, bool ANY = false>
TRT_DEV bool walk_compact(const SceneAcc<MODE>& sc, const uint4* __restrict__ nodes16, const float4* __restrict__ leaf_list,
                          const Ray& ray, Trav& tr, Counters<STATS>& ctr, float2* stk, uint32_t slots, uint32_t stragglers = 0u,
                          uint32_t entered = 64u) {
    const uint32_t n = sc.L.n_cull_nodes << 4;
    float2* const limit = stk + 64u * slots;
    const uint32_t few = stragglers < entered ? stragglers : entered - 1u;
    for (;;) {
        float2* top = stk;
        if constexpr (kAsmBoxLoop && !STATS) {
            top = box_loop_compact(tr, ray.o, nodes16, stk, limit, n, few);
        } else
        while (tr.i < n && top != limit) {
            const uint4 q = nodes16[tr.i >> 4];
            if constexpr (STATS) { ctr.node++; if (first_active_lane()) ctr.w_steps++; }
            const half2_t a = __builtin_bit_cast(half2_t, q.x), b = __builtin_bit_cast(half2_t, q.y), c = __builtin_bit_cast(half2_t, q.z);
            float start;
            const bool pass = slab_fast6_entry(v3((float)a.x, (float)a.y, (float)b.x), v3((float)b.y, (float)c.x, (float)c.y), ray.o, tr.inv,
                                               kTMin, tr.t_best, start);
            const bool is_leaf = (q.w & kCompactLeafBit) != 0u;
            const uint32_t next = tr.i + 16u;
            if (pass && is_leaf) {
                *top = make_float2(__uint_as_float(q.w & ~kCompactLeafBit), start);
                top += 64;
            }
            tr.i = (pass || is_leaf) ? next : q.w;
            if ((uint32_t)__builtin_popcountll(__builtin_amdgcn_ballot_w64(true)) <= few) break;
        }
        TRT_CLK(ctr, 1);
        if (top == stk && tr.i >= n) return true;
        if (top != stk) leaf_phase<MODE, STATS>(stk, top, tr, ctr, [&](uint32_t leaf) { compact_leaf_test<MODE, STATS>(sc, leaf_list, ray, tr, leaf, ctr); });
        TRT_CLK(ctr, 2);
        if constexpr (ANY) { if (tr.prim_best != PRIM_NONE) tr.i = n; }
        if (tr.i >= n) return true;
        if ((uint32_t)__builtin_popcountll(__builtin_amdgcn_ballot_w64(true)) <= few) { trav_park(stk, tr); return false; }
    }
}

#define TRT_COMPACT_STEP(D0, D1, D2, D3, I, TOP)                                                                                              \
                          \
        "v_fma_mix_f32 v52, " D0 ", %[ix" I "], %[nx" I "] op_sel:[0,0,0] op_sel_hi:[1,0,0]\n"                                        \
        "v_fma_mix_f32 v53, " D0 ", %[iy" I "], %[ny" I "] op_sel:[1,0,0] op_sel_hi:[1,0,0]\n"                                        \
        "v_fma_mix_f32 v54, " D1 ", %[iz" I "], %[nz" I "] op_sel:[0,0,0] op_sel_hi:[1,0,0]\n"                                        \
        "v_fma_mix_f32 " D1 ", " D1 ", %[ix" I "], %[nx" I "] op_sel:[1,0,0] op_sel_hi:[1,0,0]\n"                                     \
// ... 348 lines not shown
```

### tiny-raytracer_amd/csrc/scene.h

```cpp
#pragma once

#include <stdint.h>

#include <string>
#include <unordered_map>
#include <vector>

#include "../../include/tinyrt.h"

namespace trt {

struct F4 { float x, y, z, w; };

enum : uint32_t { PRIM_NONE = 0xFFFFFFFFu, PRIM_QUAD_BIT = 0x40000000u, PRIM_INDEX_MASK = 0x3FFFFFFFu,
                  NODE_INNER_BIT = 0x80000000u };

struct Geometry {
    uint32_t kind;
    uint32_t material;
    trt_vec3 a, b, c;
};

struct World {
    std::vector<Geometry> geometries;
    std::vector<trt_material> materials;
    std::unordered_map<std::string, uint32_t> material_index;
};

struct SceneLayout {
    uint32_t n_nodes;
    uint32_t n_cull_nodes;
    uint32_t reserved0;
    uint32_t n_spheres, n_quads, n_materials;
    uint32_t off_sphere, off_quad, off_material;
    uint32_t off_sphere_mat, off_material_kind;
    uint32_t off_ref_nodes;
    uint32_t hot_bytes, blob_bytes;
    uint32_t all_finite;
    uint32_t n_leaves;
    uint32_t off_leaf_list;
    uint32_t flat_walk;
    uint32_t off_compact;
    float compact_origin_limit[3];
    uint32_t lazy_color;
};
constexpr uint32_t kLdsSceneMaxBytes = 64u * 1024u;
constexpr uint32_t kLeafListPad = 4;
constexpr uint32_t kFlatWalkMaxLeaves = 32;

struct NodeDump {
    std::vector<float> bbox6;
    std::vector<int32_t> prim_geo;
    std::vector<int32_t> skip;
};

struct SceneHost {
    SceneLayout layout;
    std::vector<uint8_t> blob;
    uint32_t max_depth = 0;
    NodeDump reference, culling;
};

bool compile_scene(const World& w, const trt_scene_options& opt, SceneHost& out, std::string& msg);
bool scene_layout(const World& w, const trt_scene_options& opt, uint32_t ns, uint32_t nq, uint32_t nn, uint32_t nc, bool all_finite,
                  SceneLayout& L, std::string& msg);
uint32_t reference_max_depth(uint32_t n);
trt_scene_options scene_options_builtin();

void camera_init(trt_camera& out, float focus_distance, float defocus_angle_deg, trt_vec3 position, trt_vec3 look_at,
                 trt_vec3 up, float vertical_fov_deg, uint32_t width, uint32_t height);

void emitter_init_quad(trt_emitter& out, trt_vec3 corner, trt_vec3 u, trt_vec3 v, trt_vec3 color);
void emitter_init_sphere(trt_emitter& out, trt_vec3 centre, float radius, trt_vec3 color);

void tonemap_u8(const float* accum, uint32_t npixels, float gamma, uint8_t* rgb);

}
```

### tiny-raytracer_amd/csrc/scene_cache.h

```cpp
#pragma once

#include <hip/hip_runtime.h>

#include <algorithm>
#include <condition_variable>
#include <mutex>
#include <new>
#include <string>
#include <unordered_map>
#include <vector>

#include "scene_query.h"

namespace trt {

class DeviceRestore {
  public:
    DeviceRestore() : e_(hipGetDevice(&prev_)) {}
    DeviceRestore(const DeviceRestore&) = delete;
    ~DeviceRestore() { if (e_ == hipSuccess) (void)hipSetDevice(prev_); }
    hipError_t error() const { return e_; }
    int device() const { return prev_; }
  private:
    int prev_ = 0;
    hipError_t e_;
};

struct Workspace {
    void* ptr = nullptr;
    size_t bytes = 0;
    hipEvent_t done = nullptr;
    hipStream_t last_stream = nullptr;
    bool recorded = false;
    bool busy = false;
};
struct RenderCtx {
    hipStream_t stream = nullptr;
    hipEvent_t ev0 = nullptr, ev1 = nullptr;
    unsigned long long* d_ctr = nullptr;
    float* d_accum = nullptr;
    size_t accum_bytes = 0;
    bool busy = false;
};
constexpr size_t kMaxWorkspacesPerDevice = 8;

class SceneCache {
  public:
    enum Upload { PACKED_SCENE, GEO_INDEX };
    ~SceneCache() {
        DeviceRestore restore;
        for (auto& kv : dev_) {
            if (hipSetDevice(kv.first) != hipSuccess) continue;
            DeviceCache& dc = kv.second;
            for (Workspace* w : dc.ws) {
                if (w->recorded) (void)hipEventSynchronize(w->done);
                if (w->ptr) (void)hipFree(w->ptr);
                if (w->done) (void)hipEventDestroy(w->done);
                delete w;
            }
            for (RenderCtx* c : dc.ctx) context_destroy(c);
            for (Cached& u : dc.up) if (u.ptr) (void)hipFree(u.ptr);
        }
    }
    void set_cap(size_t bytes) { cap_ = bytes; }
    template <class T>
    int on_device(Upload which, const void* host, size_t bytes, const char* label, T*& out) {
        int dev = 0;
        hipError_t e = hipGetDevice(&dev);
        if (e != hipSuccess) return query_fail_hip(e, "hipGetDevice");
        std::unique_lock<std::mutex> lock(mu_);
        Cached& u = dev_[dev].up[which];
        while (u.ptr == nullptr && u.busy) cv_.wait(lock);
        if (u.ptr == nullptr) {
            u.busy = true;
            lock.unlock();
            void* d = nullptr;
            e = hipMalloc(&d, bytes ? bytes : sizeof(uint32_t));
            if (e == hipSuccess && bytes) {
                e = hipMemcpy(d, host, bytes, hipMemcpyHostToDevice);
                if (e != hipSuccess) { (void)hipFree(d); d = nullptr; }
            }
            lock.lock();
            u.busy = false;
            u.ptr = d;
            cv_.notify_all();
            if (e != hipSuccess) return query_fail_hip(e, label);
        }
        out = static_cast<T*>(u.ptr);
        return TRT_OK;
    }
    void adopt_packed_scene(int dev, void* d_blob) { std::lock_guard<std::mutex> lock(mu_); dev_[dev].up[PACKED_SCENE].ptr = d_blob; }
    int workspace_acquire(int dev, size_t need, hipStream_t stream, Workspace** out) {
        std::unique_lock<std::mutex> lock(mu_);
        DeviceCache& dc = dev_[dev];
        bool may_grow = true;
        for (;;) {
            Workspace* pick = nullptr;
            Workspace* regrow = nullptr;
            for (Workspace* w : dc.ws) {
                if (w->busy || !ws_finished(w)) continue;
                if (w->bytes >= need) { if (!pick || w->bytes < pick->bytes) pick = w; }
                else if (!regrow) regrow = w;
            }
            enum { USE, REGROW, CREATE, QUEUE, DRAIN } what = USE;
            bool same_stream = false;
            if (!pick && stream != hipStreamPerThread) {
                for (Workspace* w : dc.ws) if (!w->busy && w->recorded && w->last_stream == stream && w->bytes >= need && (!pick || w->bytes < pick->bytes)) pick = w;
                same_stream = pick != nullptr;
            }
            if (same_stream) what = QUEUE;
            if (!pick && regrow) { pick = regrow; what = REGROW; }
            if (!pick && may_grow && dc.ws.size() < kMaxWorkspacesPerDevice) {
                pick = new (std::nothrow) Workspace();
                if (!pick) return query_fail(TRT_ERR_OOM, "out of memory");
                dc.ws.push_back(pick);
                what = CREATE;
            }
            if (!pick) {
                for (Workspace* w : dc.ws) if (!w->busy && w->bytes >= need) { pick = w; what = QUEUE; break; }
            }
            if (!pick) {
                bool any_busy = false;
                for (Workspace* w : dc.ws) any_busy = any_busy || w->busy;
                if (any_busy) { cv_.wait(lock); continue; }
                if (dc.ws.empty()) return query_fail(TRT_ERR_OOM, "no device memory for a render workspace");
                pick = dc.ws.front();
                what = DRAIN;
            }
            pick->busy = true;
            lock.unlock();
            hipError_t e = hipSuccess;
            const char* where = "";
            if (what == CREATE) {
                e = hipEventCreateWithFlags(&pick->done, hipEventDisableTiming); where = "hipEventCreate(workspace)";
                if (e == hipSuccess) { e = hipMalloc(&pick->ptr, need); where = "hipMalloc(workspace)"; if (e == hipSuccess) pick->bytes = need; else pick->ptr = nullptr; }
            } else if (what == DRAIN || what == REGROW) {
                if (what == DRAIN) { e = hipEventSynchronize(pick->done); where = "hipEventSynchronize(workspace)"; }
                if (e == hipSuccess && pick->ptr) { e = hipFree(pick->ptr); where = "hipFree(workspace)"; pick->ptr = nullptr; pick->bytes = 0; }
                if (e == hipSuccess) { e = hipMalloc(&pick->ptr, need); where = "hipMalloc(workspace)"; if (e == hipSuccess) pick->bytes = need; else pick->ptr = nullptr; }
                if (e == hipSuccess) pick->recorded = false;
            } else if (what == QUEUE) {
                e = hipStreamWaitEvent(stream, pick->done, 0); where = "hipStreamWaitEvent(workspace)";
            }
            if (e == hipSuccess) { *out = pick; return TRT_OK; }
            (void)hipGetLastError();
            lock.lock();
            if (what == CREATE) {
                dc.ws.erase(std::find(dc.ws.begin(), dc.ws.end(), pick));
                if (pick->done) (void)hipEventDestroy(pick->done);
                delete pick;
                cv_.notify_all();
                if (e == hipErrorOutOfMemory) {
                    bool fits = false;
                    for (Workspace* w : dc.ws) fits = fits || w->busy || w->bytes >= need;
                    if (fits) { may_grow = false; continue; }
                    return query_fail(TRT_ERR_OOM, std::string(where) + ": " + hipGetErrorString(e));
                }
                return query_fail_hip(e, where);
            }
            pick->busy = false;
            cv_.notify_all();
            if (e == hipErrorOutOfMemory) return query_fail(TRT_ERR_OOM, std::string(where) + ": " + hipGetErrorString(e));
            return query_fail_hip(e, where);
        }
    }
    int workspace_release(int dev, Workspace* w, hipStream_t stream) {
        hipError_t e = hipEventRecord(w->done, stream);
        bool recorded = e == hipSuccess;
        if (!recorded) {
            (void)hipGetLastError();
            (void)hipStreamSynchronize(stream);
            (void)hipGetLastError();
        }
        {
            std::unique_lock<std::mutex> lock(mu_);
            w->recorded = recorded;
            w->last_stream = stream;
            w->busy = false;
            trim_locked(lock, dev_[dev], cap_);
        }
        cv_.notify_all();
        if (e != hipSuccess) return query_fail_hip(e, "hipEventRecord(workspace)");
        return TRT_OK;
    }

    int context_acquire(int dev, size_t accum_bytes, RenderCtx** out) {
        RenderCtx* c = nullptr;
        bool fresh = false;
        {
            std::lock_guard<std::mutex> lock(mu_);
            DeviceCache& dc = dev_[dev];
            RenderCtx* fits = nullptr;
            RenderCtx* any = nullptr;
            for (RenderCtx* k : dc.ctx) {
                if (k->busy) continue;
                if (k->accum_bytes >= accum_bytes && (!fits || k->accum_bytes < fits->accum_bytes)) fits = k;
                if (!any || k->accum_bytes > any->accum_bytes) any = k;
            }
            c = fits ? fits : any;
            if (!c) {
                c = new (std::nothrow) RenderCtx();
                if (!c) return query_fail(TRT_ERR_OOM, "out of memory");
                dc.ctx.push_back(c);
                fresh = true;
            }
            c->busy = true;
        }
        hipError_t e = hipSuccess;
        const char* where = "";
        if (fresh) {
            e = hipStreamCreateWithFlags(&c->stream, hipStreamNonBlocking); where = "hipStreamCreate";
            if (e == hipSuccess) { e = hipEventCreate(&c->ev0); where = "hipEventCreate"; }
            if (e == hipSuccess) { e = hipEventCreate(&c->ev1); where = "hipEventCreate"; }
            if (e == hipSuccess) { e = hipMalloc(reinterpret_cast<void**>(&c->d_ctr), CTR_COUNT * sizeof(unsigned long long)); where = "hipMalloc(counters)"; }
        }
        if (e == hipSuccess && c->accum_bytes < accum_bytes) {
            if (c->d_accum) { e = hipFree(c->d_accum); where = "hipFree(frame)"; c->d_accum = nullptr; c->accum_bytes = 0; }
            if (e == hipSuccess) { e = hipMalloc(reinterpret_cast<void**>(&c->d_accum), accum_bytes); where = "hipMalloc(frame)"; if (e == hipSuccess) c->accum_bytes = accum_bytes; else c->d_accum = nullptr; }
        }
        if (e == hipSuccess) { *out = c; return TRT_OK; }
        (void)hipGetLastError();
        const int rc = query_fail_hip(e, where);
        std::lock_guard<std::mutex> lock(mu_);
        if (fresh) {
            DeviceCache& dc = dev_[dev];
            dc.ctx.erase(std::find(dc.ctx.begin(), dc.ctx.end(), c));
            context_destroy(c);
        } else {
            c->busy = false;
        }
        return rc;
    }
    void context_release(int dev, RenderCtx* c) {
        std::unique_lock<std::mutex> lock(mu_);
        c->busy = false;
        trim_locked(lock, dev_[dev], cap_);
    }
    void trim(int dev, size_t cap) { std::unique_lock<std::mutex> lock(mu_); trim_locked(lock, dev_[dev], cap); }
    void trim_all() {
        DeviceRestore restore;
        std::vector<int> devices;
        {
            std::lock_guard<std::mutex> lock(mu_);
            for (auto& kv : dev_) devices.push_back(kv.first);
        }
        for (int d : devices) if (hipSetDevice(d) == hipSuccess) trim(d, 0);
    }
    size_t idle_workspace_bytes(int dev) {
        std::lock_guard<std::mutex> lock(mu_);
        size_t idle = 0;
        for (Workspace* w : dev_[dev].ws) if (!w->busy) idle += w->bytes;
        return idle;
    }
    uint32_t short_samples(int dev) { std::lock_guard<std::mutex> lock(mu_); return dev_[dev].short_samples; }
    void set_short_samples(int dev, uint32_t samples) { std::lock_guard<std::mutex> lock(mu_); dev_[dev].short_samples = samples; }
  private:
    struct Cached { void* ptr = nullptr; bool busy = false; };
    struct DeviceCache {
        Cached up[2];
        std::vector<Workspace*> ws;
        std::vector<RenderCtx*> ctx;
        uint32_t short_samples = 0;
    };
    static bool ws_finished(Workspace* w) {
        if (!w->recorded) return true;
        const bool done = hipEventQuery(w->done) == hipSuccess;
        (void)hipGetLastError();
        return done;
    }
    static void context_destroy(RenderCtx* c) {
        if (c->d_accum) (void)hipFree(c->d_accum);
        if (c->d_ctr) (void)hipFree(c->d_ctr);
        if (c->ev0) (void)hipEventDestroy(c->ev0);
        if (c->ev1) (void)hipEventDestroy(c->ev1);
        if (c->stream) { (void)hipStreamSynchronize(c->stream); (void)hipStreamDestroy(c->stream); }
        (void)hipGetLastError();
        delete c;
    }
    void trim_locked(std::unique_lock<std::mutex>& lock, DeviceCache& dc, size_t cap) {
        for (;;) {
            size_t total = 0;
            for (Workspace* w : dc.ws) if (!w->busy) total += w->bytes;
            for (RenderCtx* c : dc.ctx) if (!c->busy) total += c->accum_bytes;
            if (total <= cap) return;
            Workspace* bw = nullptr;
            RenderCtx* bc = nullptr;
            for (Workspace* w : dc.ws) if (!w->busy && w->bytes && ws_finished(w) && (!bw || w->bytes > bw->bytes)) bw = w;
            for (RenderCtx* c : dc.ctx) if (!c->busy && c->accum_bytes && (!bc || c->accum_bytes > bc->accum_bytes)) bc = c;
            if (!bw && !bc) return;
            void* victim;
            if (bw && (!bc || bw->bytes >= bc->accum_bytes)) { bw->busy = true; victim = bw->ptr; bw->ptr = nullptr; bw->bytes = 0; bw->recorded = false; bc = nullptr; }
            else { bc->busy = true; victim = bc->d_accum; bc->d_accum = nullptr; bc->accum_bytes = 0; bw = nullptr; }
            lock.unlock();
            (void)hipFree(victim);
            (void)hipGetLastError();
            lock.lock();
            if (bw) bw->busy = false; else bc->busy = false;
            cv_.notify_all();
        }
    }
    std::mutex mu_;
    std::condition_variable cv_;
    std::unordered_map<int, DeviceCache> dev_;
    size_t cap_ = (size_t)32 << 30;
};

inline void counters_to_stats(const unsigned long long* c, trt_stats* st) {
    st->samples = c[CTR_SAMPLES]; st->rays = c[CTR_RAYS]; st->node_tests = c[CTR_NODE]; st->sphere_tests = c[CTR_SPHERE];
    st->quad_plane_tests = c[CTR_QUAD_PLANE]; st->quad_inside_tests = c[CTR_QUAD_INSIDE]; st->shades = c[CTR_SHADE];
    for (int i = 0; i < 4; i++) st->wave_trips[i] = c[CTR_W_ROUNDS + i];
    st->gather_per_band = 0;
}

class CtxRun {
  public:
    explicit CtxRun(SceneCache& cache, int dev = -1) : cache_(cache), dev_(dev) { if (dev < 0) step(hipGetDevice(&dev_), "hipGetDevice"); }
    CtxRun(const CtxRun&) = delete;
    ~CtxRun() {
        if (!c_) return;
        if (!drained_) (void)hipStreamSynchronize(c_->stream);
        for (int k = 0; k < n_owned_; k++) (void)hipFree(owned_[k]);
        if (!ok()) (void)hipGetLastError();
        cache_.context_release(dev_, c_);
    }
    bool ok() const { return rc_ == TRT_OK; }
    void acquire(size_t frame_bytes) { if (ok()) rc_ = cache_.context_acquire(dev_, frame_bytes, &c_); }
    hipStream_t stream() const { return c_ ? c_->stream : nullptr; }
    float* frame() const { return c_ ? c_->d_accum : nullptr; }
    unsigned long long* counters() const { return c_ ? c_->d_ctr : nullptr; }
    template <class T>
    void alloc(T** p, size_t bytes, const char* what, int code) {
        if (!ok()) return;
        const hipError_t e = n_owned_ < 2 ? hipMalloc(reinterpret_cast<void**>(p), bytes) : hipErrorInvalidValue;
        if (e != hipSuccess) { (void)hipGetLastError(); *p = nullptr; rc_ = query_fail(code, std::string(what) + ": " + hipGetErrorString(e)); return; }
        owned_[n_owned_++] = *p;
    }
    void zero_counters() { if (ok()) step(hipMemsetAsync(c_->d_ctr, 0, CTR_COUNT * sizeof(unsigned long long), c_->stream), "hipMemsetAsync(counters)"); }
    void step(hipError_t e, const char* what) { if (ok() && e != hipSuccess) rc_ = query_fail_hip(e, what); }
    void step(int status) { if (ok()) rc_ = status; }
    void time_begin() { if (ok()) step(hipEventRecord(c_->ev0, c_->stream), "hipEventRecord(ev0)"); }
    void time_end() { if (ok()) step(hipEventRecord(c_->ev1, c_->stream), "hipEventRecord(ev1)"); }
    int finish(unsigned long long (&h_ctr)[CTR_COUNT], float* ms) {
        if (ok()) step(hipMemcpyAsync(h_ctr, c_->d_ctr, sizeof(h_ctr), hipMemcpyDeviceToHost, c_->stream), "hipMemcpyAsync(counters)");
        if (ok()) { step(hipStreamSynchronize(c_->stream), "hipStreamSynchronize"); drained_ = ok(); }
        if (ok()) step(hipEventElapsedTime(ms, c_->ev0, c_->ev1), "hipEventElapsedTime");
        return rc_;
    }
    int finish(trt_stats* stats) {
        float ms = 0.0f;
        if (finish(h_ctr_, &ms) == TRT_OK && stats) { counters_to_stats(h_ctr_, stats); stats->kernel_ms = ms; }
        return rc_;
    }
  private:
    SceneCache& cache_;
    int dev_ = 0;
    RenderCtx* c_ = nullptr;
    int rc_ = TRT_OK, n_owned_ = 0;
    bool drained_ = false;
    void* owned_[2] = {nullptr, nullptr};
    unsigned long long h_ctr_[CTR_COUNT] = {0};
};

}
```

### tiny-raytracer_amd/csrc/streamed.hip

```cpp
#include <string>

#include "host_stage.h"
#include "kernels.h"
#include "rt_path.h"
#include "stream_plan.h"
#include "wave_run.h"

namespace trt {

template <int MODE, bool STATS, int MINW = 1, int THREADS = 256, int WALK = WALK_RUNTIME, bool LAZY = false>
__global__ __launch_bounds__(THREADS, MINW) void stream_sample_kernel(SceneDev scd, CameraDev cam, RenderArgs ra,
                                                                             float* __restrict__ colors,
                                                                             uint32_t* __restrict__ batch_counter,
                                                                             unsigned long long* __restrict__ counters,
                                                                             uint32_t tiles_x, uint32_t n_tiles, uint32_t n_batches, uint32_t batch_spp,
                                                                             const float4* __restrict__ leaf_list,
                                                                             const uint4* __restrict__ nodes16) {
    stage_scene_to_lds<MODE>(scd);
    const FlatReuse flat_reuse = axis_quads_to_lds<MODE, STATS, WALK>(scd, ra.flat_reuse);
    const SceneAcc<MODE> sc{scd.blob, scd.L};
    const uint32_t lane = threadIdx.x & 63u;
    const V3 background = v3(ra.background[0], ra.background[1], ra.background[2]);
    const uint32_t n_spp = ra.sample_end - ra.sample_begin;
    float2* const leaf_stack = (WALK != WALK_REGS && (WALK != WALK_RUNTIME || ra.lds_leaf_stack))
        ? reinterpret_cast<float2*>(lds_behind_scene(sc)) + (threadIdx.x >> 6) * (64u * ra.leaf_slots) + lane
        : nullptr;

    uint32_t tile_x0 = 0, tile_row0 = 0, tile_slot0 = 0, ds0 = 0, items_per_batch = 0, cursor = 0;
    bool exhausted = false;

    Path p;
    p.remain = 0u;
    bool has_path = false, stocked = false;
    uint32_t out_idx = 0, stock_idx = 0;
    Ray stock_ray;
    Rng stock_rng;
    uint32_t n_samples = 0, n_rays = 0;
    Counters<STATS> ctr;
    constexpr bool kResumable = !STATS && (WALK == WALK_COMPACT || WALK == WALK_LDS_STACK);
    bool walking = false;

    TRT_CLK_START(ctr);
    for (;;) {
        if (!exhausted && __builtin_amdgcn_ballot_w64(!has_path && !stocked) != 0ull) {
            if (cursor >= items_per_batch) {
                uint32_t b = 0;
                if (lane == 0u) b = atomicAdd(batch_counter, 1u);
                b = __builtin_amdgcn_readfirstlane(b);
                if (b >= n_batches) {
                    exhausted = true;
                } else {
                    const uint32_t tile = b % n_tiles;
                    ds0 = (b / n_tiles) * batch_spp;
                    tile_x0 = (tile % tiles_x) * 8u;
                    tile_row0 = (tile / tiles_x) * 8u;
                    tile_slot0 = tile * n_spp * 64u;
                    items_per_batch = 64u * (n_spp - ds0 < batch_spp ? n_spp - ds0 : batch_spp);
                    cursor = 0;
                }
            }
            if (!exhausted) {
                const uint64_t want = __builtin_amdgcn_ballot_w64(!stocked);
                const uint32_t item = cursor + wave_rank(want);
                cursor += (uint32_t)__builtin_popcountll(want);
                if (!stocked && item < items_per_batch) {
                    const uint32_t l = item & 63u, ds = ds0 + (item >> 6);
                    const uint32_t x = tile_x0 + (l & 7u), row = tile_row0 + (l >> 3);
                    if (x < cam.width && row < ra.rows_local) {
                        if constexpr (STATS) { if (first_active_lane()) ctr.w_gen++; }
                        const uint32_t y = image_row(ra, row);
                        stock_rng = rng_seed(ra.seed_key, y * cam.width + x, ra.sample_begin + ds);
                        stock_ray = primary_ray(cam, x, y, stock_rng);
                        stock_idx = tile_slot0 + ds * 64u + l;
                        stocked = true;
                    }
                }
            }
        }
        if (!has_path && stocked) {
            p.ray = stock_ray;
            p.rng = stock_rng;
            p.color = v3(0.0f, 0.0f, 0.0f);
            p.atten = v3(1.0f, 1.0f, 1.0f);
            p.remain = ra.max_bounces;
            out_idx = stock_idx;
            has_path = true;
            stocked = false;
            n_samples++;
        }
        if (__builtin_amdgcn_ballot_w64(has_path) == 0ull) {
            if (exhausted) break;
            continue;
        }
        TRT_CLK(ctr, 0);
        if (has_path) {
            if constexpr (STATS) { if (first_active_lane()) ctr.w_rounds++; }
            if constexpr (kResumable) {
                Trav tr = trav_begin<MODE, WALK == WALK_COMPACT>(sc, p.ray, false);
                if (walking) trav_unpark(leaf_stack, tr); else n_rays++;
                const uint32_t entered = (uint32_t)__builtin_popcountll(__builtin_amdgcn_ballot_w64(true));
                walking = !closest_hit_resume<MODE, STATS, WALK>(sc, p.ray, tr, ctr, ra.leaf_slots, leaf_stack, leaf_list, nodes16, ra.stragglers, entered);
                if (!walking) {
                    if (shade_hit<MODE, STATS, LAZY>(sc, p, tr.prim_best, tr.t_best, background, ctr)) {
                        radiance_store(colors, out_idx, p.color);
                        has_path = false;
                    }
                }
            } else {
                n_rays++;
                float t;
                const uint32_t prim = closest_hit<MODE, STATS, WALK>(sc, p.ray, STATS && ra.ref_tree != 0u, t, ctr, ra.leaf_slots, leaf_stack, leaf_list, nodes16, flat_reuse);
                if (shade_hit<MODE, STATS, LAZY>(sc, p, prim, t, background, ctr)) {
                    radiance_store(colors, out_idx, p.color);
                    has_path = false;
                }
            }
        }
        TRT_CLK(ctr, 3);
    }
    flush_counters<STATS>(counters, n_samples, n_rays, ctr);
}


struct StreamKernargs {
    SceneDev scd; CameraDev cam; RenderArgs ra;
    float* colors; uint32_t* batch_counter; unsigned long long* counters;
    uint32_t tiles_x, n_tiles, n_batches, batch_spp;
    const float4* leaf_list; const uint4* nodes16;
};
struct StreamTileArgs { uint32_t tiles_x, n_tiles, n_batches, batch_spp; };
template <class T>
TRT_DEV T kernarg_reload(size_t offset) {
    static_assert(sizeof(T) % 4 == 0, "whole words");
    typedef const __attribute__((address_space(4))) uint32_t* WordPtr;
    WordPtr w = (WordPtr)__builtin_amdgcn_kernarg_segment_ptr() + offset / 4;
    asm volatile("" : "+s"(w));
    uint32_t words[sizeof(T) / 4];
#pragma unroll
    for (uint32_t i = 0; i < sizeof(T) / 4; i++) words[i] = w[i];
    T v;
    __builtin_memcpy(&v, words, sizeof(T));
    return v;
}

template <int MODE, bool STATS, int MINW = 1, int THREADS = 256, int WALK = WALK_RUNTIME, bool LAZY = false>
__global__ __launch_bounds__(THREADS, MINW) void stream_pool_kernel(SceneDev scd, CameraDev cam_entry, RenderArgs ra,
                                                                           float* __restrict__ colors_entry,
                                                                           uint32_t* __restrict__ batch_counter_entry,
                                                                           unsigned long long* __restrict__ counters,
                                                                           uint32_t tiles_x_entry, uint32_t n_tiles_entry, uint32_t n_batches_entry, uint32_t batch_spp_entry,
                                                                           const float4* __restrict__ leaf_list,
                                                                           const uint4* __restrict__ nodes16) {
    stage_scene_to_lds<MODE>(scd);
    const FlatReuse flat_reuse = axis_quads_to_lds<MODE, STATS, WALK>(scd, ra.flat_reuse);
    const SceneAcc<MODE> sc{scd.blob, scd.L};
    const uint32_t lane = threadIdx.x & 63u;
    const V3 background = v3(ra.background[0], ra.background[1], ra.background[2]);
    char* const lds_tail = lds_behind_scene(sc);
    float2* const leaf_stack = reinterpret_cast<float2*>(lds_tail) + (threadIdx.x >> 6) * (64u * ra.leaf_slots) + lane;
    uint32_t* const pool = reinterpret_cast<uint32_t*>(lds_tail + (size_t)THREADS * ra.leaf_slots * sizeof(float2)) + (threadIdx.x >> 6) * (64u * kPoolDwords);

    uint32_t tile_x0 = 0, tile_row0 = 0, tile_slot0 = 0, ds0 = 0, items_per_batch = 0, cursor = 0;
    uint32_t pool_head = 0, pool_count = 0;
    bool exhausted = false;

    Path p;
    p.remain = 0u;
    bool has_path = false;
    uint32_t out_idx = 0;
    uint32_t n_samples = 0, n_rays = 0;
    Counters<STATS> ctr;
    constexpr bool kResumable = !STATS && (WALK == WALK_COMPACT || WALK == WALK_LDS_STACK);
    bool walking = false;

    TRT_CLK_START(ctr);
    for (;;) {
        for (;;) {
            const uint64_t need = __builtin_amdgcn_ballot_w64(!has_path);
            if (need == 0ull) break;
            if (pool_count == 0u) {
                if (exhausted) break;
                const CameraDev cam = kernarg_reload<CameraDev>(offsetof(StreamKernargs, cam));
                const RenderArgs rr = kernarg_reload<RenderArgs>(offsetof(StreamKernargs, ra));
                const StreamTileArgs ta = kernarg_reload<StreamTileArgs>(offsetof(StreamKernargs, tiles_x));
                const uint32_t n_spp = rr.sample_end - rr.sample_begin;
                if (cursor >= items_per_batch) {
                    uint32_t* const batch_counter = kernarg_reload<uint32_t*>(offsetof(StreamKernargs, batch_counter));
                    const uint32_t tiles_x = ta.tiles_x, n_tiles = ta.n_tiles, n_batches = ta.n_batches, batch_spp = ta.batch_spp;
                    uint32_t b = 0;
                    if (lane == 0u) b = atomicAdd(batch_counter, 1u);
                    b = __builtin_amdgcn_readfirstlane(b);
                    if (b >= n_batches) { exhausted = true; break; }
                    const uint32_t tile = b % n_tiles;
                    ds0 = (b / n_tiles) * batch_spp;
                    tile_x0 = (tile % tiles_x) * 8u;
                    tile_row0 = (tile / tiles_x) * 8u;
                    tile_slot0 = tile * n_spp * 64u;
                    items_per_batch = 64u * (n_spp - ds0 < batch_spp ? n_spp - ds0 : batch_spp);
                    cursor = 0;
                }
                const uint32_t item = cursor + lane;
                cursor += 64u;
                const uint32_t ds = ds0 + (item >> 6);
                const uint32_t x = tile_x0 + (lane & 7u), row = tile_row0 + (lane >> 3);
                const bool valid = x < cam.width && row < rr.rows_local;
                const uint64_t vmask = __builtin_amdgcn_ballot_w64(valid);
                if (valid) {
                    if constexpr (STATS) { if (first_active_lane()) ctr.w_gen++; }
                    const uint32_t y = image_row(rr, row);
                    Rng rng = rng_seed(rr.seed_key, y * cam.width + x, rr.sample_begin + ds);
                    const Ray ray = primary_ray(cam, x, y, rng);
                    const uint32_t e = wave_rank(vmask);
                    pool[0u * 64u + e] = __float_as_uint(ray.o.x); pool[1u * 64u + e] = __float_as_uint(ray.o.y); pool[2u * 64u + e] = __float_as_uint(ray.o.z);
                    pool[3u * 64u + e] = __float_as_uint(ray.d.x); pool[4u * 64u + e] = __float_as_uint(ray.d.y); pool[5u * 64u + e] = __float_as_uint(ray.d.z);
                    pool[6u * 64u + e] = rng.s0; pool[7u * 64u + e] = rng.s1;
                    pool[8u * 64u + e] = tile_slot0 + ds * 64u + lane;
                }
                pool_head = 0u;
                pool_count = (uint32_t)__builtin_popcountll(vmask);
                if (pool_count == 0u) continue;
            }
            const uint32_t rank = wave_rank(need);
            if (!has_path && rank < pool_count) {
                const uint32_t e = pool_head + rank;
                p.ray.o = v3(__uint_as_float(pool[0u * 64u + e]), __uint_as_float(pool[1u * 64u + e]), __uint_as_float(pool[2u * 64u + e]));
                p.ray.d = v3(__uint_as_float(pool[3u * 64u + e]), __uint_as_float(pool[4u * 64u + e]), __uint_as_float(pool[5u * 64u + e]));
                p.rng.s0 = pool[6u * 64u + e]; p.rng.s1 = pool[7u * 64u + e];
                out_idx = pool[8u * 64u + e];
                p.color = v3(0.0f, 0.0f, 0.0f);
                p.atten = v3(1.0f, 1.0f, 1.0f);
                p.remain = ra.max_bounces;
                has_path = true;
                n_samples++;
            }
            const uint32_t wanted = (uint32_t)__builtin_popcountll(need);
            const uint32_t taken = wanted < pool_count ? wanted : pool_count;
            pool_head += taken;
            pool_count -= taken;
        }
        if (__builtin_amdgcn_ballot_w64(has_path) == 0ull) break;
        TRT_CLK(ctr, 0);
        if (has_path) {
            if constexpr (STATS) { if (first_active_lane()) ctr.w_rounds++; }
            if constexpr (kResumable) {
                Trav tr = trav_begin<MODE, WALK == WALK_COMPACT>(sc, p.ray, false);
                if (walking) trav_unpark(leaf_stack, tr); else n_rays++;
                const uint32_t entered = (uint32_t)__builtin_popcountll(__builtin_amdgcn_ballot_w64(true));
                walking = !closest_hit_resume<MODE, STATS, WALK>(sc, p.ray, tr, ctr, ra.leaf_slots, leaf_stack, leaf_list, nodes16, ra.stragglers, entered);
                if (!walking) {
                    if (shade_hit<MODE, STATS, LAZY>(sc, p, tr.prim_best, tr.t_best, background, ctr)) {
                        radiance_store(kernarg_reload<float*>(offsetof(StreamKernargs, colors)), out_idx, p.color);
                        has_path = false;
                    }
                }
            } else {
                n_rays++;
                float t;
                const uint32_t prim = closest_hit<MODE, STATS, WALK>(sc, p.ray, STATS && ra.ref_tree != 0u, t, ctr, ra.leaf_slots, leaf_stack, leaf_list, nodes16, flat_reuse);
                if (shade_hit<MODE, STATS, LAZY>(sc, p, prim, t, background, ctr)) {
                    radiance_store(kernarg_reload<float*>(offsetof(StreamKernargs, colors)), out_idx, p.color);
                    has_path = false;
                }
            }
        }
        TRT_CLK(ctr, 3);
    }
    flush_counters<STATS>(counters, n_samples, n_rays, ctr);
}

struct DualSlot {
    Path p;
    uint32_t out_idx = 0;
    bool has_path = false;
    bool walking = false;
};

template <int MINW, int THREADS = 256>
__global__ __launch_bounds__(THREADS, MINW) void stream_dual_kernel(SceneDev scd, CameraDev cam, RenderArgs ra,
                                                                           float* __restrict__ colors,
                                                                           uint32_t* __restrict__ batch_counter,
                                                                           unsigned long long* __restrict__ counters,
                                                                           uint32_t tiles_x, uint32_t n_tiles, uint32_t n_batches, uint32_t batch_spp,
                                                                           const float4* __restrict__ leaf_list,
                                                                           const uint4* __restrict__ nodes16) {
    constexpr int MODE = MODE_GLOBAL;
    const SceneAcc<MODE> sc{scd.blob, scd.L};
    const uint32_t lane = threadIdx.x & 63u, wave = threadIdx.x >> 6;
    const V3 background = v3(ra.background[0], ra.background[1], ra.background[2]);
    const uint32_t n_spp = ra.sample_end - ra.sample_begin;
    char* const lds_tail = reinterpret_cast<char*>(g_lds);
    float2* const stkA = reinterpret_cast<float2*>(lds_tail) + (2u * wave) * (64u * ra.leaf_slots) + lane;
    float2* const stkB = stkA + 64u * ra.leaf_slots;
    uint32_t* const pool = reinterpret_cast<uint32_t*>(lds_tail + (size_t)THREADS * 2u * ra.leaf_slots * sizeof(float2)) + wave * (64u * kPoolDwords);

    uint32_t tile_x0 = 0, tile_row0 = 0, tile_slot0 = 0, ds0 = 0, items_per_batch = 0, cursor = 0;
    uint32_t pool_head = 0, pool_count = 0;
    bool exhausted = false;
    uint32_t n_samples = 0, n_rays = 0;
    Counters<false> ctr;
    DualSlot A, B;
    A.p.remain = 0u; B.p.remain = 0u;

    auto take = [&](DualSlot& S) {
        for (;;) {
            const uint64_t need = __builtin_amdgcn_ballot_w64(!S.has_path);
            if (need == 0ull) break;
            if (pool_count == 0u) {
                if (exhausted) break;
                if (cursor >= items_per_batch) {
                    uint32_t b = 0;
                    if (lane == 0u) b = atomicAdd(batch_counter, 1u);
                    b = __builtin_amdgcn_readfirstlane(b);
                    if (b >= n_batches) { exhausted = true; break; }
                    const uint32_t tile = b % n_tiles;
                    ds0 = (b / n_tiles) * batch_spp;
                    tile_x0 = (tile % tiles_x) * 8u;
                    tile_row0 = (tile / tiles_x) * 8u;
                    tile_slot0 = tile * n_spp * 64u;
                    items_per_batch = 64u * (n_spp - ds0 < batch_spp ? n_spp - ds0 : batch_spp);
                    cursor = 0;
                }
                const uint32_t item = cursor + lane;
                cursor += 64u;
                const uint32_t ds = ds0 + (item >> 6);
                const uint32_t x = tile_x0 + (lane & 7u), row = tile_row0 + (lane >> 3);
                const bool valid = x < cam.width && row < ra.rows_local;
                const uint64_t vmask = __builtin_amdgcn_ballot_w64(valid);
                if (valid) {
                    const uint32_t y = image_row(ra, row);
                    Rng rng = rng_seed(ra.seed_key, y * cam.width + x, ra.sample_begin + ds);
                    const Ray ray = primary_ray(cam, x, y, rng);
                    const uint32_t e = wave_rank(vmask);
                    pool[0u * 64u + e] = __float_as_uint(ray.o.x); pool[1u * 64u + e] = __float_as_uint(ray.o.y); pool[2u * 64u + e] = __float_as_uint(ray.o.z);
                    pool[3u * 64u + e] = __float_as_uint(ray.d.x); pool[4u * 64u + e] = __float_as_uint(ray.d.y); pool[5u * 64u + e] = __float_as_uint(ray.d.z);
                    pool[6u * 64u + e] = rng.s0; pool[7u * 64u + e] = rng.s1;
                    pool[8u * 64u + e] = tile_slot0 + ds * 64u + lane;
                }
                pool_head = 0u;
                pool_count = (uint32_t)__builtin_popcountll(vmask);
                if (pool_count == 0u) continue;
            }
            const uint32_t rank = wave_rank(need);
            if (!S.has_path && rank < pool_count) {
                const uint32_t e = pool_head + rank;
                S.p.ray.o = v3(__uint_as_float(pool[0u * 64u + e]), __uint_as_float(pool[1u * 64u + e]), __uint_as_float(pool[2u * 64u + e]));
                S.p.ray.d = v3(__uint_as_float(pool[3u * 64u + e]), __uint_as_float(pool[4u * 64u + e]), __uint_as_float(pool[5u * 64u + e]));
                S.p.rng.s0 = pool[6u * 64u + e]; S.p.rng.s1 = pool[7u * 64u + e];
                S.out_idx = pool[8u * 64u + e];
                S.p.color = v3(0.0f, 0.0f, 0.0f);
                S.p.atten = v3(1.0f, 1.0f, 1.0f);
                S.p.remain = ra.max_bounces;
                S.has_path = true;
                n_samples++;
            }
            const uint32_t wanted = (uint32_t)__builtin_popcountll(need);
            const uint32_t taken = wanted < pool_count ? wanted : pool_count;
            pool_head += taken;
            pool_count -= taken;
        }
    };
    auto settle = [&](DualSlot& S, Trav& tr, bool done, float2* stk) {
        if (!S.has_path) return;
        if (!done) { trav_park(stk, tr); S.walking = true; return; }
        S.walking = false;
        if (shade_hit<MODE, false, true>(sc, S.p, tr.prim_best, tr.t_best, background, ctr)) {
            radiance_store(colors, S.out_idx, S.p.color);
            S.has_path = false;
        }
    };

    TRT_CLK_START(ctr);
    for (;;) {
        take(A);
        take(B);
        if (__builtin_amdgcn_ballot_w64(A.has_path || B.has_path) == 0ull) break;
        TRT_CLK(ctr, 0);
        Trav trA = trav_begin<MODE, true>(sc, A.p.ray, false), trB = trav_begin<MODE, true>(sc, B.p.ray, false);
        if (A.has_path) { if (A.walking) trav_unpark(stkA, trA); else n_rays++; }
        if (B.has_path) { if (B.walking) trav_unpark(stkB, trB); else n_rays++; }
        const uint32_t entered = (uint32_t)__builtin_popcountll(__builtin_amdgcn_ballot_w64(A.has_path)) +
                                 (uint32_t)__builtin_popcountll(__builtin_amdgcn_ballot_w64(B.has_path));
        bool doneA = false, doneB = false;
        walk_compact2<MODE>(sc, nodes16, leaf_list, A.p.ray, trA, A.has_path, B.p.ray, trB, B.has_path, ctr, stkA, stkB, ra.leaf_slots, ra.stragglers,
                            entered, doneA, doneB);
        settle(A, trA, doneA, stkA);
        settle(B, trB, doneB, stkB);
        TRT_CLK(ctr, 3);
    }
    flush_counters<false>(counters, n_samples, n_rays, ctr);
}

__global__ __launch_bounds__(256) void stream_fold_kernel(const float* __restrict__ colors, float* __restrict__ accum, uint32_t width, uint32_t rows,
                                                          uint32_t tiles_x, uint32_t n_tiles, uint32_t n_spp, float inv_spp, uint32_t accumulate) {
    const uint32_t tile = blockIdx.x * (blockDim.x >> 6) + (threadIdx.x >> 6), lane = threadIdx.x & 63u;
    if (tile >= n_tiles) return;
    const uint32_t x = (tile % tiles_x) * 8u + (lane & 7u), row = (tile / tiles_x) * 8u + (lane >> 3);
    if (x >= width || row >= rows) return;
    float* out = accum + 3ull * ((unsigned long long)row * width + x);
    V3 acc = v3(0.0f, 0.0f, 0.0f);
    if (accumulate) acc = v3(out[0], out[1], out[2]);
    const float* rec = colors + 3ull * ((unsigned long long)tile * n_spp * 64ull + lane);
    for (uint32_t s = 0; s < n_spp; s++) {
        const Radiance c = *reinterpret_cast<const Radiance*>(rec + 3ull * 64ull * s);
        acc = acc + v3(c.r, c.g, c.b) * inv_spp;
    }
    out[0] = acc.x; out[1] = acc.y; out[2] = acc.z;
}

__global__ __launch_bounds__(256) void stream_fold_moments_kernel(const float* __restrict__ colors, float* __restrict__ accum, float* __restrict__ moment2,
                                                                  uint32_t width, uint32_t rows, uint32_t tiles_x, uint32_t n_tiles, uint32_t n_spp,
                                                                  float inv_spp, uint32_t accumulate) {
    const uint32_t tile = blockIdx.x * (blockDim.x >> 6) + (threadIdx.x >> 6), lane = threadIdx.x & 63u;
    if (tile >= n_tiles) return;
    const uint32_t x = (tile % tiles_x) * 8u + (lane & 7u), row = (tile / tiles_x) * 8u + (lane >> 3);
    if (x >= width || row >= rows) return;
    const unsigned long long px = 3ull * ((unsigned long long)row * width + x);
    float* out = accum + px;
    float* out2 = moment2 + px;
    V3 acc = v3(0.0f, 0.0f, 0.0f), m2 = v3(0.0f, 0.0f, 0.0f);
    if (accumulate) { acc = v3(out[0], out[1], out[2]); m2 = v3(out2[0], out2[1], out2[2]); }
    const float* rec = colors + 3ull * ((unsigned long long)tile * n_spp * 64ull + lane);
    for (uint32_t s = 0; s < n_spp; s++) {
        const Radiance c = *reinterpret_cast<const Radiance*>(rec + 3ull * 64ull * s);
        acc = acc + v3(c.r, c.g, c.b) * inv_spp;
        m2.x = m2.x + (c.r * c.r) * inv_spp;
        m2.y = m2.y + (c.g * c.g) * inv_spp;
        m2.z = m2.z + (c.b * c.b) * inv_spp;
    }
    out[0] = acc.x; out[1] = acc.y; out[2] = acc.z;
    out2[0] = m2.x; out2[1] = m2.y; out2[2] = m2.z;
}

__global__ __launch_bounds__(256) void variance_kernel(const float* __restrict__ accum, const float* __restrict__ moment2, uint32_t npixels, float inv_nm1,
                                                       uint32_t known, float* __restrict__ variance) {
    const uint32_t i = blockIdx.x * 256u + threadIdx.x;
    if (i >= npixels) return;
    if (!known) { variance[i] = __builtin_inff(); return; }
    const float* s = accum + 3ull * i;
    const float* m = moment2 + 3ull * i;
    float dr = m[0] - s[0] * s[0], dg = m[1] - s[1] * s[1], db = m[2] - s[2] * s[2];
    dr = dr > 0.0f ? dr : 0.0f;
    dg = dg > 0.0f ? dg : 0.0f;
    db = db > 0.0f ? db : 0.0f;
    variance[i] = ((dr + dg) + db) * inv_nm1;
}

hipError_t launch_variance(const float* d_accum, const float* d_moment2, uint32_t npixels, uint32_t samples_per_pixel, float* d_variance, hipStream_t stream) {
    if (npixels == 0u) return hipSuccess;
    const uint32_t known = samples_per_pixel > 1u ? 1u : 0u;
    const float inv_nm1 = known ? 1.0f / (float)(samples_per_pixel - 1u) : 0.0f;
    hipLaunchKernelGGL(variance_kernel, dim3((npixels + 255u) / 256u), dim3(256), 0, stream, d_accum, d_moment2, npixels, inv_nm1, known, d_variance);
    return hipGetLastError();
}

static unsigned long long padded_pixels(uint32_t width, uint32_t rows) { return 64ull * ((width + 7u) / 8u) * ((rows + 7u) / 8u); }

uint32_t streamed_chunk_spp(uint32_t width, uint32_t rows, uint32_t radiance_gb) {
    const unsigned long long px = padded_pixels(width, rows);
    const unsigned long long budget = (unsigned long long)(radiance_gb >= 1u && radiance_gb <= 64u ? radiance_gb : 16u) << 30;
    const unsigned long long fit = px ? budget / (px * 12ull) : 256ull;
    uint32_t c = 16;
    while (c < 256u && 2ull * c <= fit) c *= 2u;
    while (c > 1u && px * c >= (1ull << 32)) c /= 2u;
    return c;
}
constexpr size_t kWorkspaceHeader = 256;
size_t streamed_workspace_bytes(uint32_t width, uint32_t rows, uint32_t samples, uint32_t radiance_gb) {
    const uint32_t chunk = streamed_chunk_spp(width, rows, radiance_gb);
    return kWorkspaceHeader + (size_t)padded_pixels(width, rows) * (samples < chunk ? (samples ? samples : 1u) : chunk) * 3 * sizeof(float);
}
uint32_t streamed_chunk_that_fits(uint32_t width, uint32_t rows, size_t bytes) {
    const unsigned long long px = padded_pixels(width, rows);
    if (px == 0 || bytes <= kWorkspaceHeader) return 0;
    unsigned long long c = (bytes - kWorkspaceHeader) / (px * 12ull);
    if (c > 256ull) c = 256ull;
    while (c > 1ull && px * c >= (1ull << 32)) c--;
    return (uint32_t)c;
}

namespace {

#define TRT_FN_POOL(MODE, STATS, MINW, THREADS, WALK, LAZY) reinterpret_cast<const void*>(&stream_pool_kernel<MODE, STATS, MINW, THREADS, WALK, LAZY>),
#define TRT_FN_SAMPLE(MODE, STATS, MINW, THREADS, WALK, LAZY) reinterpret_cast<const void*>(&stream_sample_kernel<MODE, STATS, MINW, THREADS, WALK, LAZY>),
#define TRT_FN_DUAL(MINW) reinterpret_cast<const void*>(&stream_dual_kernel<MINW, 256>),
const void* const kStreamKernelFns[] = {
    TRT_STREAM_SPECIALISED(TRT_FN_POOL, TRT_FN_SAMPLE, TRT_FN_DUAL)
    TRT_STREAM_GENERAL(TRT_FN_POOL, TRT_FN_SAMPLE, TRT_FN_DUAL)
};
#undef TRT_FN_POOL
#undef TRT_FN_SAMPLE
#undef TRT_FN_DUAL
static_assert(sizeof(kStreamKernelFns) / sizeof(kStreamKernelFns[0]) == kStreamKernelCount, "one address per shape row");

}

static hipError_t launch_streamed_folds(const SceneDev& sc, const CameraDev& cam, const RenderArgs& ra_all, const trt_tuning& tn, void* workspace, size_t workspace_bytes,
                                        float* d_accum, float* d_moment2, unsigned long long* d_counters, bool stats, hipStream_t stream) {
    if (ra_all.rows_local == 0 || cam.width == 0) return hipSuccess;
    uint32_t* batch_counter = static_cast<uint32_t*>(workspace);
    float* colors = reinterpret_cast<float*>(static_cast<char*>(workspace) + kWorkspaceHeader);
    const uint32_t samples_all = ra_all.sample_end - ra_all.sample_begin;
    uint32_t chunk_full = streamed_chunk_spp(cam.width, ra_all.rows_local, tn.radiance_gb);
    const uint32_t granted = streamed_chunk_that_fits(cam.width, ra_all.rows_local, workspace_bytes);
    if (granted == 0u) return hipErrorInvalidValue;
    if (chunk_full > granted) chunk_full = granted;
    const uint32_t chunk = samples_all < chunk_full ? (samples_all ? samples_all : 1u) : chunk_full;
    uint32_t tiles_x = (cam.width + 7u) / 8u;
    const uint32_t tiles_y = (ra_all.rows_local + 7u) / 8u;
    uint32_t n_tiles = tiles_x * tiles_y;
    int dev = 0, cus = 256;
    hipError_t e = hipGetDevice(&dev);
    if (e != hipSuccess) return e;
    (void)hipDeviceGetAttribute(&cus, hipDeviceAttributeMultiprocessorCount, dev);
    const StreamLaunchPlan pl = streamed_launch_plan(sc.L, ra_all, tn, stats);
    if (pl.kernel_index < 0 || (size_t)pl.kernel_index >= kStreamKernelCount) return hipErrorInvalidDeviceFunction;
    const void* const kernel = kStreamKernelFns[pl.kernel_index];
    const LdsLayout lds = plan_lds_layout(pl);
    if (lds.total() != pl.lds_bytes || !lds.fits(1u) || pl.kernel_threads != pl.threads || (pl.pool && !pl.lds_stack) ||
        (pl.flat && pl.slots < 2u) || (pl.kernel_pool != pl.pool)) return hipErrorInvalidConfiguration;
    SceneDev scd = sc;
    CameraDev camd = cam;
    const float4* leaf_list = (pl.flat || pl.compact) ? sc.blob + sc.L.off_leaf_list : nullptr;
    const uint4* nodes16 = pl.compact ? reinterpret_cast<const uint4*>(sc.blob + sc.L.off_compact) : nullptr;
    const int walk_of_plan = pl.walk;
    const uint32_t resident = (uint32_t)cus * pl.wg_per_cu;
    const uint32_t waves_per_wg = (uint32_t)pl.threads / 64u;
    if (pl.lds_bytes > 48u * 1024u) {
        e = hipFuncSetAttribute(kernel, hipFuncAttributeMaxDynamicSharedMemorySize, (int)pl.lds_bytes);
        if (e != hipSuccess) return e;
    }
    bool first = true;
    for (uint32_t s0 = ra_all.sample_begin; s0 < ra_all.sample_end; s0 += chunk) {
        RenderArgs ra = ra_all;
        ra.lds_leaf_stack = pl.lds_stack ? 1u : 0u;
        if (pl.lds_stack) ra.leaf_slots = pl.slots;
        if (walk_of_plan == WALK_LDS_STACK) {
            ra.stragglers = tn.lds_stragglers;
        }
        if (!pl.lds_stack || pl.slots < 2u) ra.stragglers = 0u;
        ra.sample_begin = s0;
        ra.sample_end = s0 + chunk < ra_all.sample_end ? s0 + chunk : ra_all.sample_end;
        uint32_t batch_spp = tn.stream_batch_spp ? tn.stream_batch_spp : kBatchSpp;
        uint32_t n_batches = n_tiles * ((ra.sample_end - ra.sample_begin + batch_spp - 1u) / batch_spp);
        uint32_t grid_x = resident;
        const uint32_t max_useful = (n_batches + waves_per_wg - 1u) / waves_per_wg;
        if (grid_x > max_useful) grid_x = max_useful ? max_useful : 1u;
        e = hipMemsetAsync(batch_counter, 0, sizeof(uint32_t), stream);
        if (e != hipSuccess) return e;
        void* args[] = {&scd, &camd, &ra, &colors, &batch_counter, &d_counters, &tiles_x, &n_tiles, &n_batches, &batch_spp, &leaf_list, &nodes16};
        timing_mark(stream, true);
        e = hipLaunchKernel(kernel, dim3(grid_x), dim3((uint32_t)pl.threads), args, pl.lds_bytes, stream);
        timing_mark(stream, false);
        if (e != hipSuccess) return e;
        const uint32_t fold_blocks = (n_tiles + 3u) / 4u;
        if (d_moment2 == nullptr) {
            hipLaunchKernelGGL(stream_fold_kernel, dim3(fold_blocks), dim3(256), 0, stream, colors, d_accum, cam.width, ra_all.rows_local, tiles_x, n_tiles,
                               ra.sample_end - ra.sample_begin, ra_all.inv_spp, (first && !ra_all.accumulate) ? 0u : 1u);
        } else {
            hipLaunchKernelGGL(stream_fold_moments_kernel, dim3(fold_blocks), dim3(256), 0, stream, colors, d_accum, d_moment2, cam.width, ra_all.rows_local,
                               tiles_x, n_tiles, ra.sample_end - ra.sample_begin, ra_all.inv_spp, (first && !ra_all.accumulate) ? 0u : 1u);
        }
        e = hipGetLastError();
        if (e != hipSuccess) return e;
        first = false;
    }
    return hipSuccess;
}

hipError_t launch_streamed(const SceneDev& sc, const CameraDev& cam, const RenderArgs& ra, const trt_tuning& tn, void* workspace, size_t workspace_bytes,
                           float* d_accum, unsigned long long* d_counters, bool stats, hipStream_t stream) {
    return launch_streamed_folds(sc, cam, ra, tn, workspace, workspace_bytes, d_accum, nullptr, d_counters, stats, stream);
}

hipError_t launch_streamed_moments(const SceneDev& sc, const CameraDev& cam, const RenderArgs& ra, const trt_tuning& tn, void* workspace, size_t workspace_bytes,
                                   float* d_accum, float* d_moment2, unsigned long long* d_counters, bool stats, hipStream_t stream) {
    if (d_moment2 == nullptr) return hipErrorInvalidValue;
    return launch_streamed_folds(sc, cam, ra, tn, workspace, workspace_bytes, d_accum, d_moment2, d_counters, stats, stream);
}

}

extern "C" {

int trt_render_moments(trt_scene* s, const trt_camera* cam, const trt_render_params* p, float* accum, float* moment2, trt_stats* stats) {
    return trt::query_render_moments(s, cam, p, accum, moment2, stats, &trt::launch_streamed_moments);
}

int trt_render_moments_device(trt_scene* s, const trt_camera* cam, const trt_render_params* p, float* d_accum, float* d_moment2,
                              uint64_t* d_counters, void* stream) {
    return trt::query_render_moments_device(s, cam, p, d_accum, d_moment2, d_counters, static_cast<hipStream_t>(stream), &trt::launch_streamed_moments);
}

int trt_variance_device(const float* d_accum, const float* d_moment2, uint32_t npixels, uint32_t samples_per_pixel, float* d_variance, void* stream) {
    if (npixels && (!d_accum || !d_moment2 || !d_variance)) return trt::query_fail(TRT_ERR_INVALID_ARG, "null argument");
    if (npixels == 0u) return TRT_OK;
    const int rc = trt::query_require_device();
    if (rc != TRT_OK) return rc;
    const hipError_t e = trt::launch_variance(d_accum, d_moment2, npixels, samples_per_pixel, d_variance, static_cast<hipStream_t>(stream));
    if (e != hipSuccess) return trt::query_fail_hip(e, "variance launch");
    return TRT_OK;
}

int trt_variance(const float* accum, const float* moment2, uint32_t npixels, uint32_t samples_per_pixel, float* variance) {
    return trt::host_form([&]() -> int {
        if (npixels && (!accum || !moment2 || !variance)) return trt::query_fail(TRT_ERR_INVALID_ARG, "null argument");
        if (npixels == 0u) return TRT_OK;
        const int rc = trt::query_require_device();
        if (rc != TRT_OK) return rc;
        const size_t frame = (size_t)npixels * 12u;
        trt::HostStage st("variance buffers");
        const size_t r_s = st.reserve(frame), r_m = st.reserve(frame), r_v = st.reserve((size_t)npixels * 4u);
        st.alloc();
        st.up(r_s, accum, frame, "hipMemcpy of the inputs");
        st.up(r_m, moment2, frame, "hipMemcpy of the inputs");
        if (st.ok()) st.run(trt::launch_variance(st.ptr<float>(r_s), st.ptr<float>(r_m), npixels, samples_per_pixel, st.ptr<float>(r_v), nullptr), "variance launch");
        st.down(variance, r_v, (size_t)npixels * 4u, "hipMemcpy of the result");
        return st.finish();
    });
}

}
```

Baseline: 66960 Mray/s.

## JIT-compile streamed kernel with scene leaf boxes baked as asm literals

At render time the host generates GCN assembly that tests each flat-walk leaf box with its bounds as immediate literals, skipping axes that the flat-reuse masks mark as shared. It then compiles a specialised stream_pool kernel via hiprtc and launches it through hipModuleLaunchKernel in place of the built-in kernel. The aim is to remove the per-ray loads of leaf bounds and the looping overhead of the flat box walk. In exchange it adds a runtime dependency on hiprtc, a one-time compilation cost inside the call, and hand-written assembly with a PC-relative jump table that bakes in scene data.

New measurement: 71250 Mray/s (median of 6 runs). 1.06x the previous value.

```diff
diff --git a/bindings/rust/tinyrt-sys/src/lib.rs b/bindings/rust/tinyrt-sys/src/lib.rs
--- a/bindings/rust/tinyrt-sys/src/lib.rs
+++ b/bindings/rust/tinyrt-sys/src/lib.rs
@@ -596,6 +596,8 @@
     pub fn trt_kernel_timing_end(total_ms: *mut f64, launches: *mut u32) -> c_int;
 
     pub fn trt_dominant_kernel(s: *const trt_scene, cam: *const trt_camera, p: *const trt_render_params) -> *const c_char;
+    pub fn trt_flat_literal_compilations() -> u64;
+    pub fn trt_flat_literal_diagnostic() -> *const c_char;
 
     pub fn trt_last_error() -> *const c_char;
     pub fn trt_device_count() -> c_int;
diff --git a/include/tinyrt.h b/include/tinyrt.h
--- a/include/tinyrt.h
+++ b/include/tinyrt.h
@@ -443,6 +443,9 @@
 
 const char *trt_dominant_kernel(const trt_scene *s, const trt_camera *cam, const trt_render_params *p);
 
+uint64_t trt_flat_literal_compilations(void);
+const char *trt_flat_literal_diagnostic(void);
+
 const char *trt_last_error(void);
 int trt_device_count(void);
 int trt_set_device(int ordinal);
diff --git a/tiny-raytracer_amd/_lib.py b/tiny-raytracer_amd/_lib.py
--- a/tiny-raytracer_amd/_lib.py
+++ b/tiny-raytracer_amd/_lib.py
@@ -354,6 +354,8 @@
     "trt_device_count": (C.c_int, []),
     "trt_set_device": (C.c_int, [C.c_int]),
     "trt_abi_version": (C.c_uint32, []),
+    "trt_flat_literal_compilations": (C.c_uint64, []),
+    "trt_flat_literal_diagnostic": (C.c_char_p, []),
 }
 
 
diff --git a/tiny-raytracer_amd/csrc/capi.hip b/tiny-raytracer_amd/csrc/capi.hip
--- a/tiny-raytracer_amd/csrc/capi.hip
+++ b/tiny-raytracer_amd/csrc/capi.hip
@@ -103,6 +103,8 @@
     bool flat_reuse = true;
     bool axis_quads = true;
     bool nearest_first = true;
+    uint32_t flat_literal = 2;
+    bool flat_literal_test_fail = false;
 };
 const Defaults& defaults() {
     static const Defaults d = [] {
@@ -127,6 +129,8 @@
         if (const char* e = env("TRT_FLAT_REUSE")) x.flat_reuse = atoi(e) != 0;
         if (const char* e = env("TRT_AXIS_QUADS")) x.axis_quads = atoi(e) != 0;
         if (const char* e = env("TRT_NEAREST_FIRST")) x.nearest_first = atoi(e) != 0;
+        if (const char* e = env("TRT_FLAT_LITERAL")) x.flat_literal = atoi(e) != 0 ? 1u : 0u;
+        if (const char* e = env("TRT_FLAT_LITERAL_TEST_FAIL")) x.flat_literal_test_fail = atoi(e) != 0;
         if (const char* e = env("TRT_COMPACT_NODES")) o.compact_nodes = atoi(e) ? 1 : 0;
         if (const char* e = env("TRT_SCRATCH_CAP_MB")) o.scratch_cap_bytes = (uint64_t)strtoull(e, nullptr, 10) << 20;
         return x;
@@ -262,6 +266,18 @@
             s->cache.set_short_samples(dev, (rc == TRT_OK && samples < wanted) ? samples : 0u);
         }
         if (rc != TRT_OK) return rc;
+        LiteralRequest lit;
+        const SceneLayout& L = s->host.layout;
+        if (streamed && defaults().flat_literal != 0u && L.flat_walk != 0u && L.n_leaves > 0u &&
+            s->host.blob.size() >= 16u * ((size_t)L.off_leaf_list + 2u * (size_t)L.n_leaves)) {
+            lit.slot = s->cache.literal_kernel(dev);
+            lit.leaf_list = s->host.blob.data() + 16u * (size_t)L.off_leaf_list;
+            lit.n_leaves = L.n_leaves;
+            const uint64_t call_samples = (uint64_t)cam->width * rows * (ra.sample_end - ra.sample_begin);
+            lit.wanted = defaults().flat_literal == 1u || call_samples >= kLiteralAutoSamples;
+            lit.empty_source = defaults().flat_literal_test_fail;
+        }
+        const LiteralScope lit_scope(lit.slot ? &lit : nullptr);
         hipError_t le;
         if (streamed && d_moment2) {
             le = launch_moments ? launch_moments(sc, cd, ra, tn, ws->ptr, ws->bytes, d_accum, d_moment2, reinterpret_cast<unsigned long long*>(d_counters),
diff --git a/tiny-raytracer_amd/csrc/flat_literal.h b/tiny-raytracer_amd/csrc/flat_literal.h
--- /dev/null
+++ b/tiny-raytracer_amd/csrc/flat_literal.h
@@ -0,0 +1,123 @@
+#pragma once
+
+#include <stdint.h>
+#include <stdio.h>
+#include <string.h>
+
+#include <string>
+
+#include "flat_reuse.h"
+
+namespace trt {
+
+constexpr uint32_t kFlatLiteralMaxLeaves = 32u;
+
+namespace flat_literal_detail {
+
+inline void hex(std::string& s, uint32_t bits) {
+    char b[16];
+    snprintf(b, sizeof b, "0x%08x", bits);
+    s += b;
+}
+
+inline void box(std::string& s, const uint32_t w[8], uint32_t axes) {
+    static const char* const o[3] = {"%[ox]", "%[oy]", "%[oz]"};
+    static const char* const inv[3] = {"%[ix]", "%[iy]", "%[iz]"};
+    static const char* const lo_out[3] = {"%[xe]", "%[ye]", "%[ze]"};
+    static const char* const hi_out[3] = {"%[xx]", "%[yx]", "%[zx]"};
+    for (int k = 0; k < 3; k++) {
+        if (!(axes & (1u << k))) continue;
+        s += "v_sub_f32_e32 %[t0], "; hex(s, w[k]); s += ", "; s += o[k]; s += "\n";
+        s += "v_sub_f32_e32 %[t1], "; hex(s, w[3 + k]); s += ", "; s += o[k]; s += "\n";
+        s += "v_mul_f32_e32 %[t0], "; s += inv[k]; s += ", %[t0]\n";
+        s += "v_mul_f32_e32 %[t1], "; s += inv[k]; s += ", %[t1]\n";
+        if (k == 0) {
+            s += "v_med3_f32 %[xe], %[t0], %[t1], %[tmin]\n";
+            s += "v_med3_f32 %[xx], %[t0], %[t1], %[tb]\n";
+        } else {
+            s += "v_min_f32_e32 "; s += lo_out[k]; s += ", %[t0], %[t1]\n";
+            s += "v_max_f32_e32 "; s += hi_out[k]; s += ", %[t0], %[t1]\n";
+        }
+    }
+    s += "v_max3_f32 %[st], %[xe], %[ye], %[ze]\n";
+    s += "v_min3_f32 %[t0], %[xx], %[yx], %[zx]\n";
+    s += "v_cmp_nle_f32_e32 vcc, %[t0], %[st]\n";
+    s += "s_and_saveexec_b64 %[m], vcc\n";
+    s += "v_mov_b32_e32 %[lk], "; hex(s, w[7]); s += "\n";
+    s += "ds_write2_b32 %[top], %[lk], %[st] offset1:1\n";
+    s += "v_add_u32_e32 %[top], 0x200, %[top]\n";
+    s += "s_mov_b64 exec, %[m]\n";
+}
+
+inline void label(std::string& s, uint32_t base, uint32_t k) { s += std::to_string(base + k); s += ":\n"; }
+inline void ref(std::string& s, uint32_t base, uint32_t k, char dir) { s += std::to_string(base + k); s += dir; }
+
+}
+
+inline bool flat_literal_asm(const void* leaf_list, uint32_t n_leaves, const uint32_t masks[3], std::string& out) {
+    using namespace flat_literal_detail;
+    if (leaf_list == nullptr || n_leaves == 0u || n_leaves > kFlatLiteralMaxLeaves) return false;
+    const unsigned char* p = static_cast<const unsigned char*>(leaf_list);
+    const uint32_t n = n_leaves;
+    auto leaf = [&](uint32_t k, uint32_t w[8]) { memcpy(w, p + 32u * (size_t)k, 32u); };
+    auto axes_of = [&](uint32_t k) {
+        const uint32_t b = 1u << k;
+        return k == 0u ? 7u : (((masks[0] & b) ? 0u : 1u) | ((masks[1] & b) ? 0u : 2u) | ((masks[2] & b) ? 0u : 4u));
+    };
+    std::string s;
+    uint32_t w[8];
+    s += "s_cmp_lg_u32 %[i], 0\n";
+    s += "s_cbranch_scc1 900f\n";
+    for (uint32_t k = 0; k < n; k++) {
+        label(s, 200u, k);
+        leaf(k, w);
+        box(s, w, axes_of(k));
+        if ((k & 1u) && k + 1u < n) {
+            s += "v_cmp_gt_u32_e32 vcc, %[top], %[lim]\n";
+            s += "s_cbranch_vccnz "; ref(s, 400u, k + 1u, 'f'); s += "\n";
+        }
+    }
+    s += "s_mov_b32 %[i], "; hex(s, n); s += "\n";
+    s += "s_branch 990f\n";
+    for (uint32_t k = 2; k < n; k += 2u) {
+        label(s, 400u, k);
+        s += "s_mov_b32 %[i], "; hex(s, k); s += "\n";
+        s += "s_branch 990f\n";
+    }
+    for (uint32_t k = 2; k < n; k += 2u) {
+        if (axes_of(k) == 7u) continue;
+        label(s, 100u, k);
+        leaf(k, w);
+        box(s, w, 7u);
+        if (k + 1u < n) { s += "s_branch "; ref(s, 200u, k + 1u, 'b'); s += "\n"; }
+        else { s += "s_mov_b32 %[i], "; hex(s, n); s += "\n"; s += "s_branch 990f\n"; }
+    }
+    s += "900:\n";
+    s += "s_lshl_b32 s38, %[i], 1\n";
+    s += "s_add_u32 s38, s38, 12\n";
+    s += "s_getpc_b64 s[36:37]\n";
+    s += "s_add_u32 s36, s36, s38\n";
+    s += "s_addc_u32 s37, s37, 0\n";
+    s += "s_setpc_b64 s[36:37]\n";
+    for (uint32_t k = 0; k < n; k += 2u) {
+        s += "s_branch "; ref(s, axes_of(k) == 7u ? 200u : 100u, k, 'b'); s += "\n";
+    }
+    s += "990:\n";
+    out.swap(s);
+    return true;
+}
+
+inline std::string flat_literal_define(const std::string& name, const std::string& asm_text) {
+    std::string d = "#define " + name + " \\\n";
+    size_t a = 0;
+    while (a < asm_text.size()) {
+        size_t b = asm_text.find('\n', a);
+        if (b == std::string::npos) b = asm_text.size();
+        d += "\""; d.append(asm_text, a, b - a); d += "\\n\" \\\n";
+        a = b + 1u;
+    }
+    d += "\"\"\n";
+    return d;
+}
+
+}
diff --git a/tiny-raytracer_amd/csrc/flat_literal_rtc.h b/tiny-raytracer_amd/csrc/flat_literal_rtc.h
--- /dev/null
+++ b/tiny-raytracer_amd/csrc/flat_literal_rtc.h
@@ -0,0 +1,107 @@
+#pragma once
+
+#include <dlfcn.h>
+#include <stdint.h>
+
+#include <string>
+#include <vector>
+
+#include "flat_literal.h"
+
+namespace trt {
+
+struct RtcHeader { const char* name; const char* text; };
+inline const std::vector<RtcHeader>& rtc_project_headers() {
+    static const std::vector<RtcHeader> h = {
+#include "rtc_headers.inc"
+    };
+    return h;
+}
+inline const std::vector<RtcHeader>& rtc_system_headers() {
+    static const std::vector<RtcHeader> h = {
+        {"hip/hip_runtime.h", "#pragma once\n"},
+        {"stdint.h", "#pragma once\n"
+                     "typedef signed char int8_t; typedef unsigned char uint8_t; typedef short int16_t; typedef unsigned short uint16_t;\n"
+                     "typedef int int32_t; typedef unsigned int uint32_t; typedef long int64_t; typedef unsigned long uint64_t;\n"
+                     "typedef unsigned long uintptr_t; typedef long intptr_t;\n"},
+        {"stddef.h", "#pragma once\n#ifndef offsetof\n#define offsetof(t, m) __builtin_offsetof(t, m)\n#endif\n"},
+        {"string.h", "#pragma once\ninline void* memcpy(void* d, const void* s, unsigned long n) { return __builtin_memcpy(d, s, n); }\n"},
+        {"math.h", "#pragma once\n"},
+    };
+    return h;
+}
+
+struct HiprtcApi {
+    typedef void* Program;
+    int (*create)(Program*, const char*, const char*, int, const char* const*, const char* const*) = nullptr;
+    int (*destroy)(Program*) = nullptr;
+    int (*add_name)(Program, const char*) = nullptr;
+    int (*compile)(Program, int, const char* const*) = nullptr;
+    int (*log_size)(Program, size_t*) = nullptr;
+    int (*log)(Program, char*) = nullptr;
+    int (*lowered)(Program, const char*, const char**) = nullptr;
+    int (*code_size)(Program, size_t*) = nullptr;
+    int (*code)(Program, char*) = nullptr;
+    bool ok = false;
+};
+inline const HiprtcApi& hiprtc_api(const void* beside) {
+    static const HiprtcApi api = [beside] {
+        HiprtcApi a;
+        void* h = nullptr;
+        for (const char* name : {"libhiprtc.so", "libhiprtc.so.7", "libhiprtc.so.6"}) {
+            h = dlopen(name, RTLD_NOW | RTLD_LOCAL);
+            if (h) break;
+        }
+        Dl_info info;
+        if (!h && beside && dladdr(beside, &info) && info.dli_fname) {
+            std::string dir(info.dli_fname);
+            const size_t slash = dir.rfind('/');
+            if (slash != std::string::npos) h = dlopen((dir.substr(0, slash + 1) + "libhiprtc.so").c_str(), RTLD_NOW | RTLD_LOCAL);
+        }
+        if (!h) return a;
+        auto sym = [&](auto& fn, const char* name) { fn = reinterpret_cast<std::remove_reference_t<decltype(fn)>>(dlsym(h, name)); return fn != nullptr; };
+        a.ok = sym(a.create, "hiprtcCreateProgram") && sym(a.destroy, "hiprtcDestroyProgram") && sym(a.add_name, "hiprtcAddNameExpression") &&
+               sym(a.compile, "hiprtcCompileProgram") && sym(a.log_size, "hiprtcGetProgramLogSize") && sym(a.log, "hiprtcGetProgramLog") &&
+               sym(a.lowered, "hiprtcGetLoweredName") && sym(a.code_size, "hiprtcGetCodeSize") && sym(a.code, "hiprtcGetCode");
+        return a;
+    }();
+    return api;
+}
+
+struct FlatLiteralBuild {
+    std::vector<char> code;
+    std::string kernel;
+    std::string log;
+};
+
+inline std::string flat_literal_source(const std::string& asm_text) {
+    return flat_literal_define("TRT_FLAT_LITERAL_ASM", asm_text) + "#include \"stream_pool.h\"\n";
+}
+
+inline bool flat_literal_compile(const std::string& source, int minw, const char* arch, const void* beside, FlatLiteralBuild& out) {
+    const HiprtcApi& rtc = hiprtc_api(beside);
+    if (!rtc.ok) { out.log = "hiprtc not found"; return false; }
+    std::vector<const char*> names, texts;
+    for (const auto* set : {&rtc_system_headers(), &rtc_project_headers()})
+        for (const RtcHeader& h : *set) { names.push_back(h.name); texts.push_back(h.text); }
+    HiprtcApi::Program prog = nullptr;
+    if (rtc.create(&prog, source.c_str(), "stream_pool_literal.hip", (int)names.size(), texts.data(), names.data()) != 0) { out.log = "hiprtcCreateProgram failed"; return false; }
+    const std::string expr = "&trt::stream_pool_kernel<1, false, " + std::to_string(minw) + ", 256, 2, true>";
+    const std::string arch_opt = std::string("--offload-arch=") + arch;
+    const char* opts[] = {arch_opt.c_str(), "-O3", "-std=c++17", "-ffp-contract=off", "-fno-fast-math", "-fno-slp-vectorize"};
+    int rc = rtc.add_name(prog, expr.c_str());
+    if (rc == 0) rc = rtc.compile(prog, (int)(sizeof(opts) / sizeof(opts[0])), opts);
+    size_t n = 0;
+    if (rtc.log_size(prog, &n) == 0 && n > 1) { out.log.resize(n); rtc.log(prog, &out.log[0]); }
+    bool ok = rc == 0;
+    const char* lowered = nullptr;
+    if (ok) ok = rtc.lowered(prog, expr.c_str(), &lowered) == 0 && lowered != nullptr;
+    if (ok) out.kernel = lowered;
+    if (ok) ok = rtc.code_size(prog, &n) == 0 && n > 0;
+    if (ok) { out.code.resize(n); ok = rtc.code(prog, out.code.data()) == 0; }
+    if (!ok && out.log.empty()) out.log = "hiprtc failed (" + std::to_string(rc) + ")";
+    rtc.destroy(&prog);
+    return ok;
+}
+
+}
diff --git a/tiny-raytracer_amd/csrc/kernels.h b/tiny-raytracer_amd/csrc/kernels.h
--- a/tiny-raytracer_amd/csrc/kernels.h
+++ b/tiny-raytracer_amd/csrc/kernels.h
@@ -74,6 +74,7 @@
 inline uint32_t scene_lds_bytes(const SceneLayout& L) { return scene_mode(L) == 1 ? L.hot_bytes : 0u; }
 inline size_t q_align16(size_t b) { return (b + 15u) & ~(size_t)15u; }
 
+#ifndef __HIPCC_RTC__
 void timing_mark(hipStream_t stream, bool begin);
 
 hipError_t launch_megakernel(const SceneDev& sc, const CameraDev& cam, const RenderArgs& ra, const trt_tuning& tn, float* d_accum,
@@ -90,9 +91,12 @@
 hipError_t launch_wavefront(const SceneDev& sc, const CameraDev& cam, const RenderArgs& ra, const trt_tuning& tn, void* workspace, float* d_accum,
                             unsigned long long* d_counters, bool stats, hipStream_t stream);
 
+#endif
+#ifndef __HIPCC_RTC__
 uint32_t streamed_chunk_spp(uint32_t width, uint32_t rows, uint32_t radiance_gb);
 size_t streamed_workspace_bytes(uint32_t width, uint32_t rows, uint32_t samples, uint32_t radiance_gb);
 uint32_t streamed_chunk_that_fits(uint32_t width, uint32_t rows, size_t bytes);
+#endif
 struct StreamLaunchPlan {
     int mode, threads, waves_per_simd;
     uint32_t wg_per_cu, slots;
@@ -105,6 +109,7 @@
     bool kernel_pool, kernel_stats;
     const char* kernel_name;
 };
+#ifndef __HIPCC_RTC__
 hipError_t launch_streamed(const SceneDev& sc, const CameraDev& cam, const RenderArgs& ra, const trt_tuning& tn, void* workspace, size_t workspace_bytes,
                            float* d_accum, unsigned long long* d_counters, bool stats, hipStream_t stream);
 hipError_t launch_streamed_moments(const SceneDev& sc, const CameraDev& cam, const RenderArgs& ra, const trt_tuning& tn, void* workspace, size_t workspace_bytes,
@@ -115,5 +120,6 @@
 
 hipError_t launch_sample_batch(const SceneDev& sc, const trt_sample_point* d_in, uint32_t n, trt_sampled_color* d_out,
                                const RenderArgs& ra, unsigned long long* d_counters, bool stats, hipStream_t stream);
+#endif
 
 }
diff --git a/tiny-raytracer_amd/csrc/literal_kernel.h b/tiny-raytracer_amd/csrc/literal_kernel.h
--- /dev/null
+++ b/tiny-raytracer_amd/csrc/literal_kernel.h
@@ -0,0 +1,43 @@
+#pragma once
+
+#include <stdint.h>
+
+#include <condition_variable>
+#include <mutex>
+
+namespace trt {
+
+struct LiteralKernel {
+    enum State { UNTRIED, COMPILING, READY, FAILED };
+    std::mutex mu;
+    std::condition_variable cv;
+    State state = UNTRIED;
+    void* module = nullptr;
+    void* function = nullptr;
+    int minw = 0;
+    void (*unload)(void* module) = nullptr;
+    void release() {
+        if (module && unload) unload(module);
+        module = function = nullptr;
+        state = UNTRIED;
+    }
+};
+
+struct LiteralRequest {
+    LiteralKernel* slot = nullptr;
+    const void* leaf_list = nullptr;
+    uint32_t n_leaves = 0;
+    bool wanted = false;
+    bool empty_source = false;
+};
+inline thread_local const LiteralRequest* t_literal_request = nullptr;
+class LiteralScope {
+  public:
+    explicit LiteralScope(const LiteralRequest* r) { t_literal_request = r; }
+    LiteralScope(const LiteralScope&) = delete;
+    ~LiteralScope() { t_literal_request = nullptr; }
+};
+
+constexpr uint64_t kLiteralAutoSamples = 1ull << 26;
+
+}
diff --git a/tiny-raytracer_amd/csrc/rt_path.h b/tiny-raytracer_amd/csrc/rt_path.h
--- a/tiny-raytracer_amd/csrc/rt_path.h
+++ b/tiny-raytracer_amd/csrc/rt_path.h
@@ -484,6 +484,24 @@
     return stk + ((top - stk_off) >> 3);
 }
 
+#ifdef TRT_FLAT_LITERAL_ASM
+TRT_DEV float2* box_loop_flat_literal(const Trav& tr, const V3& o, uint32_t& i, float2* stk, float2* limit) {
+    const uint32_t stk_off = lds_offset(stk);
+    uint32_t top = stk_off;
+    const uint32_t lim = lds_offset(limit);
+    unsigned long long m;
+    float t0, t1, xe, xx, ye, yx, ze, zx, st, lk;
+    asm volatile(
+        TRT_FLAT_LITERAL_ASM
+        : [i] "+s"(i), [top] "+v"(top), [m] "=&s"(m), [t0] "=&v"(t0), [t1] "=&v"(t1), [xe] "=&v"(xe), [xx] "=&v"(xx),
+          [ye] "=&v"(ye), [yx] "=&v"(yx), [ze] "=&v"(ze), [zx] "=&v"(zx), [st] "=&v"(st), [lk] "=&v"(lk)
+        : [lim] "v"(lim), [ox] "v"(o.x), [oy] "v"(o.y), [oz] "v"(o.z), [ix] "v"(tr.inv.x), [iy] "v"(tr.inv.y),
+          [iz] "v"(tr.inv.z), [tb] "v"(tr.t_best), [tmin] "s"(kTMin)
+        : "vcc", "scc", "memory", "s36", "s37", "s38");
+    return stk + ((top - stk_off) >> 3);
+}
+#endif
+
 struct FlatIntervals {
     float xe, xx, ye, yx, ze, zx;
 };
@@ -519,7 +537,11 @@
     if constexpr (kAsmBoxLoop && !STATS) {
         float2* const lim = stk + 64u * (slots - 2u);
         do {
+#ifdef TRT_FLAT_LITERAL_ASM
+            float2* const top = box_loop_flat_literal(tr, ray.o, i, stk, lim);
+#else
             float2* const top = box_loop_flat(tr, ray.o, leaf_list, i, n, stk, lim, reuse);
+#endif
             TRT_CLK(ctr, 1);
             phase(top);
             TRT_CLK(ctr, 2);
diff --git a/tiny-raytracer_amd/csrc/scene.h b/tiny-raytracer_amd/csrc/scene.h
--- a/tiny-raytracer_amd/csrc/scene.h
+++ b/tiny-raytracer_amd/csrc/scene.h
@@ -2,11 +2,15 @@
 
 #include <stdint.h>
 
+#ifndef __HIPCC_RTC__
 #include <string>
 #include <unordered_map>
 #include <vector>
 
 #include "../../include/tinyrt.h"
+#else
+#include "tinyrt.h"
+#endif
 
 namespace trt {
 
@@ -15,6 +19,7 @@
 enum : uint32_t { PRIM_NONE = 0xFFFFFFFFu, PRIM_QUAD_BIT = 0x40000000u, PRIM_INDEX_MASK = 0x3FFFFFFFu,
                   NODE_INNER_BIT = 0x80000000u };
 
+#ifndef __HIPCC_RTC__
 struct Geometry {
     uint32_t kind;
     uint32_t material;
@@ -26,6 +31,7 @@
     std::vector<trt_material> materials;
     std::unordered_map<std::string, uint32_t> material_index;
 };
+#endif
 
 struct SceneLayout {
     uint32_t n_nodes;
@@ -48,6 +54,7 @@
 constexpr uint32_t kLeafListPad = 4;
 constexpr uint32_t kFlatWalkMaxLeaves = 32;
 
+#ifndef __HIPCC_RTC__
 struct NodeDump {
     std::vector<float> bbox6;
     std::vector<int32_t> prim_geo;
@@ -74,5 +81,6 @@
 void emitter_init_sphere(trt_emitter& out, trt_vec3 centre, float radius, trt_vec3 color);
 
 void tonemap_u8(const float* accum, uint32_t npixels, float gamma, uint8_t* rgb);
+#endif
 
 }
diff --git a/tiny-raytracer_amd/csrc/scene_cache.h b/tiny-raytracer_amd/csrc/scene_cache.h
--- a/tiny-raytracer_amd/csrc/scene_cache.h
+++ b/tiny-raytracer_amd/csrc/scene_cache.h
@@ -10,6 +10,7 @@
 #include <unordered_map>
 #include <vector>
 
+#include "literal_kernel.h"
 #include "scene_query.h"
 
 namespace trt {
@@ -60,6 +61,7 @@
             }
             for (RenderCtx* c : dc.ctx) context_destroy(c);
             for (Cached& u : dc.up) if (u.ptr) (void)hipFree(u.ptr);
+            dc.literal.release();
         }
     }
     void set_cap(size_t bytes) { cap_ = bytes; }
@@ -254,6 +256,7 @@
     }
     uint32_t short_samples(int dev) { std::lock_guard<std::mutex> lock(mu_); return dev_[dev].short_samples; }
     void set_short_samples(int dev, uint32_t samples) { std::lock_guard<std::mutex> lock(mu_); dev_[dev].short_samples = samples; }
+    LiteralKernel* literal_kernel(int dev) { std::lock_guard<std::mutex> lock(mu_); return &dev_[dev].literal; }
   private:
     struct Cached { void* ptr = nullptr; bool busy = false; };
     struct DeviceCache {
@@ -261,6 +264,7 @@
         std::vector<Workspace*> ws;
         std::vector<RenderCtx*> ctx;
         uint32_t short_samples = 0;
+        LiteralKernel literal;
     };
     static bool ws_finished(Workspace* w) {
         if (!w->recorded) return true;
diff --git a/tiny-raytracer_amd/csrc/stream_pool.h b/tiny-raytracer_amd/csrc/stream_pool.h
--- /dev/null
+++ b/tiny-raytracer_amd/csrc/stream_pool.h
@@ -0,0 +1,156 @@
+#pragma once
+
+#include "kernels.h"
+#include "rt_path.h"
+#include "stream_plan.h"
+#include "wave_run.h"
+
+namespace trt {
+
+struct StreamKernargs {
+    SceneDev scd; CameraDev cam; RenderArgs ra;
+    float* colors; uint32_t* batch_counter; unsigned long long* counters;
+    uint32_t tiles_x, n_tiles, n_batches, batch_spp;
+    const float4* leaf_list; const uint4* nodes16;
+};
+struct StreamTileArgs { uint32_t tiles_x, n_tiles, n_batches, batch_spp; };
+template <class T>
+TRT_DEV T kernarg_reload(size_t offset) {
+    static_assert(sizeof(T) % 4 == 0, "whole words");
+    typedef const __attribute__((address_space(4))) uint32_t* WordPtr;
+    WordPtr w = (WordPtr)__builtin_amdgcn_kernarg_segment_ptr() + offset / 4;
+    asm volatile("" : "+s"(w));
+    uint32_t words[sizeof(T) / 4];
+#pragma unroll
+    for (uint32_t i = 0; i < sizeof(T) / 4; i++) words[i] = w[i];
+    T v;
+    __builtin_memcpy(&v, words, sizeof(T));
+    return v;
+}
+
+template <int MODE, bool STATS, int MINW = 1, int THREADS = 256, int WALK = WALK_RUNTIME, bool LAZY = false>
+__global__ __launch_bounds__(THREADS, MINW) void stream_pool_kernel(SceneDev scd, CameraDev cam_entry, RenderArgs ra,
+                                                                           float* __restrict__ colors_entry,
+                                                                           uint32_t* __restrict__ batch_counter_entry,
+                                                                           unsigned long long* __restrict__ counters,
+                                                                           uint32_t tiles_x_entry, uint32_t n_tiles_entry, uint32_t n_batches_entry, uint32_t batch_spp_entry,
+                                                                           const float4* __restrict__ leaf_list,
+                                                                           const uint4* __restrict__ nodes16) {
+    stage_scene_to_lds<MODE>(scd);
+    const FlatReuse flat_reuse = axis_quads_to_lds<MODE, STATS, WALK>(scd, ra.flat_reuse);
+    const SceneAcc<MODE> sc{scd.blob, scd.L};
+    const uint32_t lane = threadIdx.x & 63u;
+    const V3 background = v3(ra.background[0], ra.background[1], ra.background[2]);
+    char* const lds_tail = lds_behind_scene(sc);
+    float2* const leaf_stack = reinterpret_cast<float2*>(lds_tail) + (threadIdx.x >> 6) * (64u * ra.leaf_slots) + lane;
+    uint32_t* const pool = reinterpret_cast<uint32_t*>(lds_tail + (size_t)THREADS * ra.leaf_slots * sizeof(float2)) + (threadIdx.x >> 6) * (64u * kPoolDwords);
+
+    uint32_t tile_x0 = 0, tile_row0 = 0, tile_slot0 = 0, ds0 = 0, items_per_batch = 0, cursor = 0;
+    uint32_t pool_head = 0, pool_count = 0;
+    bool exhausted = false;
+
+    Path p;
+    p.remain = 0u;
+    bool has_path = false;
+    uint32_t out_idx = 0;
+    uint32_t n_samples = 0, n_rays = 0;
+    Counters<STATS> ctr;
+    constexpr bool kResumable = !STATS && (WALK == WALK_COMPACT || WALK == WALK_LDS_STACK);
+    bool walking = false;
+
+    TRT_CLK_START(ctr);
+    for (;;) {
+        for (;;) {
+            const uint64_t need = __builtin_amdgcn_ballot_w64(!has_path);
+            if (need == 0ull) break;
+            if (pool_count == 0u) {
+                if (exhausted) break;
+                const CameraDev cam = kernarg_reload<CameraDev>(offsetof(StreamKernargs, cam));
+                const RenderArgs rr = kernarg_reload<RenderArgs>(offsetof(StreamKernargs, ra));
+                const StreamTileArgs ta = kernarg_reload<StreamTileArgs>(offsetof(StreamKernargs, tiles_x));
+                const uint32_t n_spp = rr.sample_end - rr.sample_begin;
+                if (cursor >= items_per_batch) {
+                    uint32_t* const batch_counter = kernarg_reload<uint32_t*>(offsetof(StreamKernargs, batch_counter));
+                    const uint32_t tiles_x = ta.tiles_x, n_tiles = ta.n_tiles, n_batches = ta.n_batches, batch_spp = ta.batch_spp;
+                    uint32_t b = 0;
+                    if (lane == 0u) b = atomicAdd(batch_counter, 1u);
+                    b = __builtin_amdgcn_readfirstlane(b);
+                    if (b >= n_batches) { exhausted = true; break; }
+                    const uint32_t tile = b % n_tiles;
+                    ds0 = (b / n_tiles) * batch_spp;
+                    tile_x0 = (tile % tiles_x) * 8u;
+                    tile_row0 = (tile / tiles_x) * 8u;
+                    tile_slot0 = tile * n_spp * 64u;
+                    items_per_batch = 64u * (n_spp - ds0 < batch_spp ? n_spp - ds0 : batch_spp);
+                    cursor = 0;
+                }
+                const uint32_t item = cursor + lane;
+                cursor += 64u;
+                const uint32_t ds = ds0 + (item >> 6);
+                const uint32_t x = tile_x0 + (lane & 7u), row = tile_row0 + (lane >> 3);
+                const bool valid = x < cam.width && row < rr.rows_local;
+                const uint64_t vmask = __builtin_amdgcn_ballot_w64(valid);
+                if (valid) {
+                    if constexpr (STATS) { if (first_active_lane()) ctr.w_gen++; }
+                    const uint32_t y = image_row(rr, row);
+                    Rng rng = rng_seed(rr.seed_key, y * cam.width + x, rr.sample_begin + ds);
+                    const Ray ray = primary_ray(cam, x, y, rng);
+                    const uint32_t e = wave_rank(vmask);
+                    pool[0u * 64u + e] = __float_as_uint(ray.o.x); pool[1u * 64u + e] = __float_as_uint(ray.o.y); pool[2u * 64u + e] = __float_as_uint(ray.o.z);
+                    pool[3u * 64u + e] = __float_as_uint(ray.d.x); pool[4u * 64u + e] = __float_as_uint(ray.d.y); pool[5u * 64u + e] = __float_as_uint(ray.d.z);
+                    pool[6u * 64u + e] = rng.s0; pool[7u * 64u + e] = rng.s1;
+                    pool[8u * 64u + e] = tile_slot0 + ds * 64u + lane;
+                }
+                pool_head = 0u;
+                pool_count = (uint32_t)__builtin_popcountll(vmask);
+                if (pool_count == 0u) continue;
+            }
+            const uint32_t rank = wave_rank(need);
+            if (!has_path && rank < pool_count) {
+                const uint32_t e = pool_head + rank;
+                p.ray.o = v3(__uint_as_float(pool[0u * 64u + e]), __uint_as_float(pool[1u * 64u + e]), __uint_as_float(pool[2u * 64u + e]));
+                p.ray.d = v3(__uint_as_float(pool[3u * 64u + e]), __uint_as_float(pool[4u * 64u + e]), __uint_as_float(pool[5u * 64u + e]));
+                p.rng.s0 = pool[6u * 64u + e]; p.rng.s1 = pool[7u * 64u + e];
+                out_idx = pool[8u * 64u + e];
+                p.color = v3(0.0f, 0.0f, 0.0f);
+                p.atten = v3(1.0f, 1.0f, 1.0f);
+                p.remain = ra.max_bounces;
+                has_path = true;
+                n_samples++;
+            }
+            const uint32_t wanted = (uint32_t)__builtin_popcountll(need);
+            const uint32_t taken = wanted < pool_count ? wanted : pool_count;
+            pool_head += taken;
+            pool_count -= taken;
+        }
+        if (__builtin_amdgcn_ballot_w64(has_path) == 0ull) break;
+        TRT_CLK(ctr, 0);
+        if (has_path) {
+            if constexpr (STATS) { if (first_active_lane()) ctr.w_rounds++; }
+            if constexpr (kResumable) {
+                Trav tr = trav_begin<MODE, WALK == WALK_COMPACT>(sc, p.ray, false);
+                if (walking) trav_unpark(leaf_stack, tr); else n_rays++;
+                const uint32_t entered = (uint32_t)__builtin_popcountll(__builtin_amdgcn_ballot_w64(true));
+                walking = !closest_hit_resume<MODE, STATS, WALK>(sc, p.ray, tr, ctr, ra.leaf_slots, leaf_stack, leaf_list, nodes16, ra.stragglers, entered);
+                if (!walking) {
+                    if (shade_hit<MODE, STATS, LAZY>(sc, p, tr.prim_best, tr.t_best, background, ctr)) {
+                        radiance_store(kernarg_reload<float*>(offsetof(StreamKernargs, colors)), out_idx, p.color);
+                        has_path = false;
+                    }
+                }
+            } else {
+                n_rays++;
+                float t;
+                const uint32_t prim = closest_hit<MODE, STATS, WALK>(sc, p.ray, STATS && ra.ref_tree != 0u, t, ctr, ra.leaf_slots, leaf_stack, leaf_list, nodes16, flat_reuse);
+                if (shade_hit<MODE, STATS, LAZY>(sc, p, prim, t, background, ctr)) {
+                    radiance_store(kernarg_reload<float*>(offsetof(StreamKernargs, colors)), out_idx, p.color);
+                    has_path = false;
+                }
+            }
+        }
+        TRT_CLK(ctr, 3);
+    }
+    flush_counters<STATS>(counters, n_samples, n_rays, ctr);
+}
+
+}
diff --git a/tiny-raytracer_amd/csrc/streamed.hip b/tiny-raytracer_amd/csrc/streamed.hip
--- a/tiny-raytracer_amd/csrc/streamed.hip
+++ b/tiny-raytracer_amd/csrc/streamed.hip
@@ -1,9 +1,13 @@
+#include <mutex>
 #include <string>
 
+#include "flat_literal_rtc.h"
 #include "host_stage.h"
 #include "kernels.h"
+#include "literal_kernel.h"
 #include "rt_path.h"
 #include "stream_plan.h"
+#include "stream_pool.h"
 #include "wave_run.h"
 
 namespace trt {
@@ -121,152 +125,6 @@
     flush_counters<STATS>(counters, n_samples, n_rays, ctr);
 }
 
-
-struct StreamKernargs {
-    SceneDev scd; CameraDev cam; RenderArgs ra;
-    float* colors; uint32_t* batch_counter; unsigned long long* counters;
-    uint32_t tiles_x, n_tiles, n_batches, batch_spp;
-    const float4* leaf_list; const uint4* nodes16;
-};
-struct StreamTileArgs { uint32_t tiles_x, n_tiles, n_batches, batch_spp; };
-template <class T>
-TRT_DEV T kernarg_reload(size_t offset) {
-    static_assert(sizeof(T) % 4 == 0, "whole words");
-    typedef const __attribute__((address_space(4))) uint32_t* WordPtr;
-    WordPtr w = (WordPtr)__builtin_amdgcn_kernarg_segment_ptr() + offset / 4;
-    asm volatile("" : "+s"(w));
-    uint32_t words[sizeof(T) / 4];
-#pragma unroll
-    for (uint32_t i = 0; i < sizeof(T) / 4; i++) words[i] = w[i];
-    T v;
-    __builtin_memcpy(&v, words, sizeof(T));
-    return v;
-}
-
-template <int MODE, bool STATS, int MINW = 1, int THREADS = 256, int WALK = WALK_RUNTIME, bool LAZY = false>
-__global__ __launch_bounds__(THREADS, MINW) void stream_pool_kernel(SceneDev scd, CameraDev cam_entry, RenderArgs ra,
-                                                                           float* __restrict__ colors_entry,
-                                                                           uint32_t* __restrict__ batch_counter_entry,
-                                                                           unsigned long long* __restrict__ counters,
-                                                                           uint32_t tiles_x_entry, uint32_t n_tiles_entry, uint32_t n_batches_entry, uint32_t batch_spp_entry,
-                                                                           const float4* __restrict__ leaf_list,
-                                                                           const uint4* __restrict__ nodes16) {
-    stage_scene_to_lds<MODE>(scd);
-    const FlatReuse flat_reuse = axis_quads_to_lds<MODE, STATS, WALK>(scd, ra.flat_reuse);
-    const SceneAcc<MODE> sc{scd.blob, scd.L};
-    const uint32_t lane = threadIdx.x & 63u;
-    const V3 background = v3(ra.background[0], ra.background[1], ra.background[2]);
-    char* const lds_tail = lds_behind_scene(sc);
-    float2* const leaf_stack = reinterpret_cast<float2*>(lds_tail) + (threadIdx.x >> 6) * (64u * ra.leaf_slots) + lane;
-    uint32_t* const pool = reinterpret_cast<uint32_t*>(lds_tail + (size_t)THREADS * ra.leaf_slots * sizeof(float2)) + (threadIdx.x >> 6) * (64u * kPoolDwords);
-
-    uint32_t tile_x0 = 0, tile_row0 = 0, tile_slot0 = 0, ds0 = 0, items_per_batch = 0, cursor = 0;
-    uint32_t pool_head = 0, pool_count = 0;
-    bool exhausted = false;
-
-    Path p;
-    p.remain = 0u;
-    bool has_path = false;
-    uint32_t out_idx = 0;
-    uint32_t n_samples = 0, n_rays = 0;
-    Counters<STATS> ctr;
-    constexpr bool kResumable = !STATS && (WALK == WALK_COMPACT || WALK == WALK_LDS_STACK);
-    bool walking = false;
-
-    TRT_CLK_START(ctr);
-    for (;;) {
-        for (;;) {
-            const uint64_t need = __builtin_amdgcn_ballot_w64(!has_path);
-            if (need == 0ull) break;
-            if (pool_count == 0u) {
-                if (exhausted) break;
-                const CameraDev cam = kernarg_reload<CameraDev>(offsetof(StreamKernargs, cam));
-                const RenderArgs rr = kernarg_reload<RenderArgs>(offsetof(StreamKernargs, ra));
-                const StreamTileArgs ta = kernarg_reload<StreamTileArgs>(offsetof(StreamKernargs, tiles_x));
-                const uint32_t n_spp = rr.sample_end - rr.sample_begin;
-                if (cursor >= items_per_batch) {
-                    uint32_t* const batch_counter = kernarg_reload<uint32_t*>(offsetof(StreamKernargs, batch_counter));
-                    const uint32_t tiles_x = ta.tiles_x, n_tiles = ta.n_tiles, n_batches = ta.n_batches, batch_spp = ta.batch_spp;
-                    uint32_t b = 0;
-                    if (lane == 0u) b = atomicAdd(batch_counter, 1u);
-                    b = __builtin_amdgcn_readfirstlane(b);
-                    if (b >= n_batches) { exhausted = true; break; }
-                    const uint32_t tile = b % n_tiles;
-                    ds0 = (b / n_tiles) * batch_spp;
-                    tile_x0 = (tile % tiles_x) * 8u;
-                    tile_row0 = (tile / tiles_x) * 8u;
-                    tile_slot0 = tile * n_spp * 64u;
-                    items_per_batch = 64u * (n_spp - ds0 < batch_spp ? n_spp - ds0 : batch_spp);
-                    cursor = 0;
-                }
-                const uint32_t item = cursor + lane;
-                cursor += 64u;
-                const uint32_t ds = ds0 + (item >> 6);
-                const uint32_t x = tile_x0 + (lane & 7u), row = tile_row0 + (lane >> 3);
-                const bool valid = x < cam.width && row < rr.rows_local;
-                const uint64_t vmask = __builtin_amdgcn_ballot_w64(valid);
-                if (valid) {
-                    if constexpr (STATS) { if (first_active_lane()) ctr.w_gen++; }
-                    const uint32_t y = image_row(rr, row);
-                    Rng rng = rng_seed(rr.seed_key, y * cam.width + x, rr.sample_begin + ds);
-                    const Ray ray = primary_ray(cam, x, y, rng);
-                    const uint32_t e = wave_rank(vmask);
-                    pool[0u * 64u + e] = __float_as_uint(ray.o.x); pool[1u * 64u + e] = __float_as_uint(ray.o.y); pool[2u * 64u + e] = __float_as_uint(ray.o.z);
-                    pool[3u * 64u + e] = __float_as_uint(ray.d.x); pool[4u * 64u + e] = __float_as_uint(ray.d.y); pool[5u * 64u + e] = __float_as_uint(ray.d.z);
-                    pool[6u * 64u + e] = rng.s0; pool[7u * 64u + e] = rng.s1;
-                    pool[8u * 64u + e] = tile_slot0 + ds * 64u + lane;
-                }
-                pool_head = 0u;
-                pool_count = (uint32_t)__builtin_popcountll(vmask);
-                if (pool_count == 0u) continue;
-            }
-            const uint32_t rank = wave_rank(need);
-            if (!has_path && rank < pool_count) {
-                const uint32_t e = pool_head + rank;
-                p.ray.o = v3(__uint_as_float(pool[0u * 64u + e]), __uint_as_float(pool[1u * 64u + e]), __uint_as_float(pool[2u * 64u + e]));
-                p.ray.d = v3(__uint_as_float(pool[3u * 64u + e]), __uint_as_float(pool[4u * 64u + e]), __uint_as_float(pool[5u * 64u + e]));
-                p.rng.s0 = pool[6u * 64u + e]; p.rng.s1 = pool[7u * 64u + e];
-                out_idx = pool[8u * 64u + e];
-                p.color = v3(0.0f, 0.0f, 0.0f);
-                p.atten = v3(1.0f, 1.0f, 1.0f);
-                p.remain = ra.max_bounces;
-                has_path = true;
-                n_samples++;
-            }
-            const uint32_t wanted = (uint32_t)__builtin_popcountll(need);
-            const uint32_t taken = wanted < pool_count ? wanted : pool_count;
-            pool_head += taken;
-            pool_count -= taken;
-        }
-        if (__builtin_amdgcn_ballot_w64(has_path) == 0ull) break;
-        TRT_CLK(ctr, 0);
-        if (has_path) {
-            if constexpr (STATS) { if (first_active_lane()) ctr.w_rounds++; }
-            if constexpr (kResumable) {
-                Trav tr = trav_begin<MODE, WALK == WALK_COMPACT>(sc, p.ray, false);
-                if (walking) trav_unpark(leaf_stack, tr); else n_rays++;
-                const uint32_t entered = (uint32_t)__builtin_popcountll(__builtin_amdgcn_ballot_w64(true));
-                walking = !closest_hit_resume<MODE, STATS, WALK>(sc, p.ray, tr, ctr, ra.leaf_slots, leaf_stack, leaf_list, nodes16, ra.stragglers, entered);
-                if (!walking) {
-                    if (shade_hit<MODE, STATS, LAZY>(sc, p, tr.prim_best, tr.t_best, background, ctr)) {
-                        radiance_store(kernarg_reload<float*>(offsetof(StreamKernargs, colors)), out_idx, p.color);
-                        has_path = false;
-                    }
-                }
-            } else {
-                n_rays++;
-                float t;
-                const uint32_t prim = closest_hit<MODE, STATS, WALK>(sc, p.ray, STATS && ra.ref_tree != 0u, t, ctr, ra.leaf_slots, leaf_stack, leaf_list, nodes16, flat_reuse);
-                if (shade_hit<MODE, STATS, LAZY>(sc, p, prim, t, background, ctr)) {
-                    radiance_store(kernarg_reload<float*>(offsetof(StreamKernargs, colors)), out_idx, p.color);
-                    has_path = false;
-                }
-            }
-        }
-        TRT_CLK(ctr, 3);
-    }
-    flush_counters<STATS>(counters, n_samples, n_rays, ctr);
-}
 
 struct DualSlot {
     Path p;
@@ -492,6 +350,76 @@
 #undef TRT_FN_DUAL
 static_assert(sizeof(kStreamKernelFns) / sizeof(kStreamKernelFns[0]) == kStreamKernelCount, "one address per shape row");
 
+std::mutex g_literal_mu;
+unsigned long long g_literal_compilations = 0;
+std::string g_literal_diagnostic;
+thread_local std::string t_literal_diagnostic_copy;
+
+void literal_unload(void* module) {
+    (void)hipModuleUnload(static_cast<hipModule_t>(module));
+    (void)hipGetLastError();
+}
+
+bool literal_build(LiteralKernel& slot, const LiteralRequest& rq, const FlatReuse& reuse, int minw, std::string& why) {
+    {
+        std::lock_guard<std::mutex> lock(g_literal_mu);
+        g_literal_compilations++;
+    }
+    int dev = 0;
+    hipDeviceProp_t prop;
+    if (hipGetDevice(&dev) != hipSuccess || hipGetDeviceProperties(&prop, dev) != hipSuccess) { (void)hipGetLastError(); why = "no device properties"; return false; }
+    std::string arch(prop.gcnArchName);
+    arch = arch.substr(0, arch.find(':'));
+    const uint32_t masks[3] = {reuse.x, reuse.y, reuse.z};
+    std::string text, source;
+    if (!rq.empty_source) {
+        if (!flat_literal_asm(rq.leaf_list, rq.n_leaves, masks, text)) { why = "leaf list refused"; return false; }
+        source = flat_literal_source(text);
+    }
+    FlatLiteralBuild built;
+    if (!flat_literal_compile(source, minw, arch.c_str(), reinterpret_cast<const void*>(&hipModuleLoadData), built)) { why = "hiprtc: " + built.log; return false; }
+    hipModule_t mod = nullptr;
+    hipFunction_t fn = nullptr;
+    hipError_t e = hipModuleLoadData(&mod, built.code.data());
+    if (e == hipSuccess) e = hipModuleGetFunction(&fn, mod, built.kernel.c_str());
+    if (e != hipSuccess) {
+        (void)hipGetLastError();
+        if (mod) (void)hipModuleUnload(mod);
+        why = std::string("module load: ") + hipGetErrorString(e);
+        return false;
+    }
+    slot.module = mod; slot.function = fn; slot.minw = minw; slot.unload = &literal_unload;
+    return true;
+}
+
+hipFunction_t literal_kernel_for(const StreamLaunchPlan& pl, const RenderArgs& ra, bool stats) {
+    const LiteralRequest* rq = t_literal_request;
+#ifdef TRT_PHASE_CLOCK
+    return nullptr;
+#endif
+    if (!kAsmBoxLoop) return nullptr;
+    if (!rq || !rq->slot || stats || !pl.specialised || !pl.pool || pl.dual || pl.walk != WALK_FLAT || pl.mode != MODE_LDS || ra.ref_tree ||
+        pl.kernel_walk != WALK_FLAT || pl.threads != 256 || pl.lds_bytes > 48u * 1024u || rq->n_leaves > kFlatLiteralMaxLeaves) return nullptr;
+    LiteralKernel& slot = *rq->slot;
+    std::unique_lock<std::mutex> lock(slot.mu);
+    while (slot.state == LiteralKernel::COMPILING) slot.cv.wait(lock);
+    if (slot.state == LiteralKernel::UNTRIED && rq->wanted) {
+        slot.state = LiteralKernel::COMPILING;
+        lock.unlock();
+        std::string why;
+        const bool ok = literal_build(slot, *rq, ra.flat_reuse, pl.kernel_minw, why);
+        if (!ok) {
+            std::lock_guard<std::mutex> g(g_literal_mu);
+            g_literal_diagnostic = "lock-step kernel not compiled for its scene, the built-in kernel runs: " + why;
+        }
+        lock.lock();
+        slot.state = ok ? LiteralKernel::READY : LiteralKernel::FAILED;
+        slot.cv.notify_all();
+    }
+    if (slot.state != LiteralKernel::READY || slot.minw != pl.kernel_minw) return nullptr;
+    return static_cast<hipFunction_t>(slot.function);
+}
+
 }
 
 static hipError_t launch_streamed_folds(const SceneDev& sc, const CameraDev& cam, const RenderArgs& ra_all, const trt_tuning& tn, void* workspace, size_t workspace_bytes,
@@ -515,6 +443,7 @@
     const StreamLaunchPlan pl = streamed_launch_plan(sc.L, ra_all, tn, stats);
     if (pl.kernel_index < 0 || (size_t)pl.kernel_index >= kStreamKernelCount) return hipErrorInvalidDeviceFunction;
     const void* const kernel = kStreamKernelFns[pl.kernel_index];
+    const hipFunction_t literal = literal_kernel_for(pl, ra_all, stats);
     const LdsLayout lds = plan_lds_layout(pl);
     if (lds.total() != pl.lds_bytes || !lds.fits(1u) || pl.kernel_threads != pl.threads || (pl.pool && !pl.lds_stack) ||
         (pl.flat && pl.slots < 2u) || (pl.kernel_pool != pl.pool)) return hipErrorInvalidConfiguration;
@@ -549,7 +478,8 @@
         if (e != hipSuccess) return e;
         void* args[] = {&scd, &camd, &ra, &colors, &batch_counter, &d_counters, &tiles_x, &n_tiles, &n_batches, &batch_spp, &leaf_list, &nodes16};
         timing_mark(stream, true);
-        e = hipLaunchKernel(kernel, dim3(grid_x), dim3((uint32_t)pl.threads), args, pl.lds_bytes, stream);
+        if (literal) e = hipModuleLaunchKernel(literal, grid_x, 1u, 1u, (uint32_t)pl.threads, 1u, 1u, (uint32_t)pl.lds_bytes, stream, args, nullptr);
+        else e = hipLaunchKernel(kernel, dim3(grid_x), dim3((uint32_t)pl.threads), args, pl.lds_bytes, stream);
         timing_mark(stream, false);
         if (e != hipSuccess) return e;
         const uint32_t fold_blocks = (n_tiles + 3u) / 4u;
@@ -599,6 +529,16 @@
     const hipError_t e = trt::launch_variance(d_accum, d_moment2, npixels, samples_per_pixel, d_variance, static_cast<hipStream_t>(stream));
     if (e != hipSuccess) return trt::query_fail_hip(e, "variance launch");
     return TRT_OK;
+}
+
+uint64_t trt_flat_literal_compilations(void) {
+    std::lock_guard<std::mutex> lock(trt::g_literal_mu);
+    return trt::g_literal_compilations;
+}
+const char* trt_flat_literal_diagnostic(void) {
+    std::lock_guard<std::mutex> lock(trt::g_literal_mu);
+    trt::t_literal_diagnostic_copy = trt::g_literal_diagnostic;
+    return trt::t_literal_diagnostic_copy.c_str();
 }
 
 int trt_variance(const float* accum, const float* moment2, uint32_t npixels, uint32_t samples_per_pixel, float* variance) {
```
